# CouncilmanJeremyJamm/path_tracer

Measured on AMD Instinct MI355X. Metric: Mray/s at 1920x1080, 256 spp; achieved HBM GB/s in traversal kernel, higher is better.
Workload: dtype f32; 1 GPU; Cornell box (36 triangles, 6 BLAS) 1920x1080, 256 spp, depth 8, NEE+MIS; parallelism=rows/1, bvh_in_lds=True, scene_bytes=4208

## Files before the change

### include/pt_api.h

```cpp
#ifndef PT_API_H
#define PT_API_H
#include <stdint.h>
#ifdef __cplusplus
extern "C" {
#endif

typedef struct pt_ctx pt_ctx;

enum pt_status
{
    PT_OK = 0,
    PT_ERR_ARG = -1,
    PT_ERR_HIP = -2,
    PT_ERR_STATE = -3,
    PT_ERR_NONRIGID = -4,
    PT_ERR_LIMIT = -5,
    PT_ERR_IO = -6,
    PT_ERR_PARSE = -7,
    PT_ERR_NCCL = -8
};

enum pt_material_kind
{
    PT_LAMBERTIAN = 0,
    PT_EMISSIVE = 1,
    PT_SPECULAR = 2,
    PT_GGX_METAL = 3,
    PT_GGX_DIELECTRIC = 4,
    PT_DIELECTRIC = 5
};

typedef struct pt_material_desc
{
    int32_t kind;
    float colour[3];
    float roughness;
    float ior;
    int32_t has_volume;
    float vol_absorption[3];
    float vol_k, vol_c, vol_g;
} pt_material_desc;

typedef struct pt_config
{
    uint32_t width, height;
    uint32_t max_bounces;
    uint32_t n_sobol;
    uint32_t enable_nee;
    uint64_t seed;
    uint32_t rank, world_size, strip_rows;
    uint32_t batch_spp;
    int32_t device;
    uint32_t flags;
    uint32_t stack_lds_levels;
    uint32_t queue_slack;
    uint32_t pipelines;
    uint32_t reserved;
} pt_config;

enum
{
    PT_FLAG_TIMING = 1u,
    PT_FLAG_NO_LDS_SCENE = 2u,
    PT_FLAG_TIMING_ALL = 4u,
    PT_FLAG_NO_PRIMARY_CULL = 8u,
    PT_FLAG_GENERAL_WALK = 16u,
    PT_FLAG_ADAPTIVE = 32u
};

pt_ctx* pt_create(const pt_config* cfg);
void pt_destroy(pt_ctx* ctx);
const char* pt_last_error(pt_ctx* ctx);
int pt_set_config(pt_ctx* ctx, const pt_config* cfg);

int pt_add_material(pt_ctx* ctx, const pt_material_desc* desc);
int pt_add_model(pt_ctx* ctx, const float* positions_xyz, const float* normals_xyz, uint32_t n_tris, int material,
                 const float* affine3x4_rowmajor, uint32_t n_instances);
int pt_add_model_obj(pt_ctx* ctx, const char* path, int material, const float* affine3x4_rowmajor, uint32_t n_instances);
int pt_model_vertices(pt_ctx* ctx, int model, float* positions_xyz, float* normals_xyz, uint32_t cap_tris, uint32_t* n_tris);
int pt_build(pt_ctx* ctx);
int pt_set_instances(pt_ctx* ctx, int model, const float* affine3x4_rowmajor, uint32_t n_instances);
typedef struct pt_scene_info
{
    uint64_t blas_builds;
    uint64_t tlas_builds;
    uint64_t uploads_full;
    uint64_t uploads_patched;
    uint64_t last_upload_bytes;
    uint64_t scene_bytes;
    uint64_t reserved[2];
} pt_scene_info;
int pt_get_scene_info(pt_ctx* ctx, pt_scene_info* out);

int pt_add_texture(pt_ctx* ctx, uint32_t w, uint32_t h, const float* rgb_linear);
int pt_set_material_texture(pt_ctx* ctx, int material, int texture);
int pt_set_model_uvs(pt_ctx* ctx, int model, const float* uv, uint32_t n_tris);
int pt_model_uvs(pt_ctx* ctx, int model, float* uv, uint32_t cap_tris, uint32_t* n_tris);
int pt_surface_colour(pt_ctx* ctx, int on_device, uint32_t n, const uint32_t* instance, const uint32_t* prim, const float* u, const float* v,
                      float* rgb);

int pt_set_camera(pt_ctx* ctx, const float eye[3], const float target[3], float fov_y_deg, float aspect);
enum pt_event { PT_EV_MOUSE_MOTION = 0, PT_EV_KEY_W = 1, PT_EV_KEY_S = 2, PT_EV_KEY_A = 3, PT_EV_KEY_D = 4 };
int pt_camera_input(pt_ctx* ctx, int event, float a, float b, float dt);
int pt_camera_angles(pt_ctx* ctx, float pitch_yaw[2]);
int pt_camera_matrices(pt_ctx* ctx, float cam_to_world_3x4[12], float inv_proj_4x4_colmajor[16]);
int pt_set_environment(pt_ctx* ctx, uint32_t width, uint32_t height, const float* rgb_linear);
int pt_create_ray(pt_ctx* ctx, float s, float t, float o[3], float d[3]);

int pt_set_lens(pt_ctx* ctx, float aperture, float focus);
int pt_primary_ray(pt_ctx* ctx, uint32_t pixel, uint32_t sample, float o[3], float d[3], uint32_t* draws);

enum pt_projection_kind { PT_PROJ_PERSPECTIVE = 0, PT_PROJ_PANORAMA = 1, PT_PROJ_ORTHOGRAPHIC = 2 };
typedef struct pt_projection {
    uint32_t kind;
    float span_x_deg, span_y_deg;
    float ortho_height;
    uint32_t reserved[4];
} pt_projection;
int pt_set_projection(pt_ctx* ctx, const pt_projection* projection);
int pt_get_projection(pt_ctx* ctx, pt_projection* out);

int pt_render(pt_ctx* ctx, uint32_t first_sample, uint32_t n_samples, float* data_rgba, float* position_xyzt, uint32_t* id);
int pt_active_pixels(pt_ctx* ctx, uint32_t rect[4], float root_box[6]);
int pt_render_device(pt_ctx* ctx, uint32_t first_sample, uint32_t n_samples);
int pt_reset_accumulation(pt_ctx* ctx);
int pt_accum_device_ptr(pt_ctx* ctx, void** dev_ptr, uint64_t* n_pixels);
int pt_read_accumulation(pt_ctx* ctx, float* data_rgba);
int pt_read_frame(pt_ctx* ctx, float* data_rgba, float* position_xyzt, uint32_t* id);
int pt_write_accumulation(pt_ctx* ctx, const float* data_rgba, const float* position_xyzt, const uint32_t* id);
int pt_render_samples(pt_ctx* ctx, uint32_t first_sample, uint32_t n_samples, float* samples_rgba);
typedef struct pt_adaptive
{
    float rel_error;
    float abs_floor;
    uint32_t min_samples;
    uint32_t max_samples;
} pt_adaptive;
int pt_render_adaptive(pt_ctx* ctx, const pt_adaptive* crit, uint32_t n_samples, uint32_t* n_active);
int pt_adaptive_mask(pt_ctx* ctx, const pt_adaptive* crit, uint8_t* mask, uint32_t* n_active);
int pt_read_moments(pt_ctx* ctx, float* sumsq);
int pt_write_moments(pt_ctx* ctx, const float* sumsq);

int pt_local_rows(pt_ctx* ctx, uint32_t* n_rows, uint32_t* rows, uint32_t cap);
int pt_set_stream(pt_ctx* ctx, void* hip_stream);
int pt_synchronize(pt_ctx* ctx);

int pt_frame(pt_ctx* ctx, uint32_t frame_index, const float* last_inv_projection, float* data_rgba, float* position_xyzt, uint32_t* id);
int pt_inv_projection(pt_ctx* ctx, float out16_colmajor[16]);
int pt_frame_moving(pt_ctx* ctx, uint32_t frame_index, const float* last_inv_projection, float* data_rgba, float* position_xyzt, uint32_t* id);
int pt_present(pt_ctx* ctx, float* rgba);
int pt_present_rgb8(pt_ctx* ctx, uint8_t* rgb);
int pt_write_image(pt_ctx* ctx, const char* path);
int pt_post_velocity(pt_ctx* ctx, uint32_t w, uint32_t h, const float* position, const float* last_inv_projection, float* velocity);
int pt_post_reproject(pt_ctx* ctx, uint32_t w, uint32_t h, const float* input, const float* accum, const float* velocity, const uint32_t* id,
                      float* output);
int pt_post_motion(pt_ctx* ctx, uint32_t w, uint32_t h, const float* position_xyzt, const uint32_t* instance, uint32_t n_instances,
                   const float* matrix12, const float* inv_matrix12, const float* prev_matrix12, const uint8_t* has_prev, float* x_prev_xyzt);
int pt_post_tonemap(pt_ctx* ctx, uint32_t w, uint32_t h, const float* accum, float* out);
int pt_post_rgb8(pt_ctx* ctx, uint32_t w, uint32_t h, const float* accum, uint8_t* rgb);

int pt_render_guides(pt_ctx* ctx, uint32_t sample);
int pt_read_guides(pt_ctx* ctx, float* position_xyzt, float* normal_xyz, uint32_t* model);
int pt_read_guide_instances(pt_ctx* ctx, uint32_t* instance);
int pt_read_guide_albedo(pt_ctx* ctx, float* rgb);
typedef struct pt_denoise_params
{
    uint32_t iterations;
    float sigma_luminance;
    uint32_t sigma_normal;
    float sigma_plane;
} pt_denoise_params;
int pt_denoise(pt_ctx* ctx, const pt_denoise_params* p, float* rgba);
int pt_write_denoised_image(pt_ctx* ctx, const char* path);
int pt_post_denoise(pt_ctx* ctx, uint32_t w, uint32_t h, const pt_denoise_params* p, const float* accum_rgba, const float* position_xyzt,
                    const float* normal_xyz, const uint32_t* model, const float* sumsq, float* out_rgba);

int pt_accumulate_albedo(pt_ctx* ctx, uint32_t first_sample, uint32_t n_samples);
int pt_reset_albedo(pt_ctx* ctx);
int pt_read_albedo(pt_ctx* ctx, float* rgbn);
enum { PT_ALBEDO_GUIDE = 1, PT_ALBEDO_MEAN = 2 };
int pt_denoise_albedo(pt_ctx* ctx, const pt_denoise_params* p, uint32_t albedo_source, float* rgba);
int pt_post_denoise_albedo(pt_ctx* ctx, uint32_t w, uint32_t h, const pt_denoise_params* p, const float* accum_rgba, const float* position_xyzt,
                           const float* normal_xyz, const uint32_t* model, const float* albedo_rgb, const float* sumsq, float* out_rgba);

typedef struct pt_rays_params
{
    uint32_t draws_consumed;
    uint32_t batch_rays;
    uint32_t reserved[2];
} pt_rays_params;
int pt_integrate_rays(pt_ctx* ctx, uint64_t n, const float* o_xyz, const float* d_xyz, const uint32_t* key, const uint32_t* sample,
                      const pt_rays_params* p, float* radiance_rgba, float* position_xyzt, uint8_t* id);
int pt_integrate_rays_device(pt_ctx* ctx, uint64_t n, const float* o_xyz, const float* d_xyz, const uint32_t* key, const uint32_t* sample,
                             const pt_rays_params* p, float* radiance_rgba, float* position_xyzt, uint8_t* id);

typedef struct pt_probe_params
{
    uint32_t first_sample, n_samples;
    uint32_t key_base;
    uint32_t reserved;
} pt_probe_params;
int pt_bake_probes(pt_ctx* ctx, uint32_t n_probes, const float* position_xyz, const pt_probe_params* p, float* sh27);
int pt_probe_ray(pt_ctx* ctx, uint32_t key, uint32_t sample, float d[3], float y9[9]);

int pt_trace_closest(pt_ctx* ctx, int which, uint32_t n, const float* o_xyz, const float* d_xyz, const float* t_max, float* t,
                     float* u, float* v, uint32_t* inst, uint32_t* prim);
int pt_trace_any(pt_ctx* ctx, int which, uint32_t n, const float* o_xyz, const float* d_xyz, const float* t_max, uint8_t* hit);
int pt_ss_sobol(pt_ctx* ctx, uint32_t n_points, uint32_t n, const uint32_t* index, const uint32_t* seed, float* out_xy);
int pt_math_batch(pt_ctx* ctx, int fn, uint32_t n, const float* a, const float* b, float* out0, float* out1);
int pt_material_eval(pt_ctx* ctx, int material, uint32_t n, const float* incoming_xyz, const float* normal_xyz, const uint8_t* front,
                     const uint32_t* pixel, const uint32_t* sample, uint32_t draws_consumed, float* out9);
int pt_volume_eval(pt_ctx* ctx, int material, uint32_t n, const float* incoming_xyz, const float* t_max, const float* dist,
                   const uint32_t* pixel, const uint32_t* sample, uint32_t draws_consumed, float* out9);

int pt_blas_count(pt_ctx* ctx);
int pt_blas_dump(pt_ctx* ctx, int blas, uint32_t* n_nodes, uint32_t* root, float* boxes6, uint32_t* kind, uint32_t* a, uint32_t* b,
                 uint32_t* n_prim_ids, uint32_t* prim_ids, uint32_t cap_nodes, uint32_t cap_ids);
int pt_tlas_dump(pt_ctx* ctx, int which, uint32_t* n_nodes, uint32_t* root, float* boxes6, uint32_t* kind, uint32_t* a, uint32_t* b,
                 uint32_t cap_nodes);
int pt_tlas_instances(pt_ctx* ctx, int which, uint32_t* n, float* matrix12, float* inv_matrix12, uint32_t cap);
int pt_instance_materials(pt_ctx* ctx, int which, uint32_t* n, uint32_t* material, uint32_t* blas, uint32_t cap);
int pt_light_cdf(pt_ctx* ctx, uint32_t* n, float* pdf, float* cdf, uint32_t* blas, uint32_t* prim, float* max_weight, uint32_t cap);
int pt_triangle_dump(pt_ctx* ctx, int blas, uint32_t prim, float out36[36]);

typedef struct pt_multi pt_multi;
pt_multi* pt_multi_create(const pt_config* cfg, const int32_t* devices, uint32_t n_devices);
void pt_multi_destroy(pt_multi* m);
const char* pt_multi_last_error(pt_multi* m);
pt_ctx* pt_multi_ctx(pt_multi* m, uint32_t rank);
int pt_multi_render(pt_multi* m, uint32_t first_sample, uint32_t n_samples, float* data_rgba);
int pt_multi_framebuffer_device_ptr(pt_multi* m, void** dev_ptr);
int pt_multi_reset_accumulation(pt_multi* m);
int pt_multi_write_image(pt_multi* m, const char* path);
int pt_multi_used_rccl(pt_multi* m);

typedef struct pt_stats
{
    uint64_t rays_closest;
    uint64_t rays_any;
    uint64_t rays_light_closest;
    uint64_t paths;
    uint64_t launches_trace_closest;
    double ms_trace_closest;
    double ms_trace_any, ms_trace_light, ms_shade, ms_generate, ms_accumulate;
    double ms_total;
    uint64_t scene_bytes;
    uint32_t lds_scene;
    uint32_t stack_entries;
    uint64_t state_bytes;
    uint64_t rays_light_closest_traced;
    uint64_t rays_primary_culled;
    uint32_t ident_tlas;
    uint32_t reserved_stats;
} pt_stats;
int pt_get_stats(pt_ctx* ctx, pt_stats* out);
int pt_multi_get_stats(pt_multi* m, pt_stats* sum);
int pt_last_batch_counters(pt_ctx* ctx, uint32_t* rows16, uint32_t cap_rows, uint32_t* n_rows);
int pt_last_batch_shade_pids(pt_ctx* ctx, uint32_t qclass, uint32_t first, uint32_t count, uint32_t* pids);
int pt_last_batch_step_stats(pt_ctx* ctx, uint32_t* rows8, uint32_t cap_rows, uint32_t* n_rows);
int pt_reset_stats(pt_ctx* ctx);

#ifdef __cplusplus
}
#endif
#endif
```

### path_tracer_amd/api.py

```python
from __future__ import annotations

import ctypes as C
import os
from typing import Optional

import numpy as np

from . import build as _build
from .scene_desc import CameraDesc, SceneDesc

PT_OK = 0
FLAG_TIMING = 1
FLAG_NO_LDS_SCENE = 2
FLAG_TIMING_ALL = 4
FLAG_NO_PRIMARY_CULL = 8
FLAG_GENERAL_WALK = 16
FLAG_ADAPTIVE = 32
DEFAULT_SEED = 0x5EED5EED

EXPORTS = [
    "pt_create", "pt_destroy", "pt_last_error", "pt_set_config", "pt_add_material", "pt_add_model", "pt_add_model_obj", "pt_model_vertices", "pt_build", "pt_set_camera",
    "pt_camera_matrices", "pt_set_environment", "pt_create_ray", "pt_set_lens", "pt_primary_ray", "pt_render", "pt_render_device", "pt_reset_accumulation", "pt_accum_device_ptr",
    "pt_read_accumulation", "pt_read_frame", "pt_write_accumulation", "pt_render_samples", "pt_render_adaptive", "pt_adaptive_mask", "pt_read_moments", "pt_write_moments", "pt_active_pixels", "pt_local_rows", "pt_set_stream", "pt_synchronize", "pt_camera_input", "pt_camera_angles", "pt_frame", "pt_inv_projection", "pt_present", "pt_post_velocity", "pt_post_reproject", "pt_post_tonemap", "pt_post_rgb8", "pt_present_rgb8", "pt_write_image", "pt_trace_closest", "pt_trace_any",
    "pt_ss_sobol", "pt_math_batch", "pt_material_eval", "pt_volume_eval", "pt_blas_count", "pt_blas_dump", "pt_tlas_dump", "pt_tlas_instances", "pt_instance_materials", "pt_light_cdf",
    "pt_triangle_dump", "pt_get_stats", "pt_reset_stats", "pt_last_batch_counters", "pt_last_batch_shade_pids", "pt_last_batch_step_stats",
    "pt_multi_create", "pt_multi_destroy", "pt_multi_last_error", "pt_multi_ctx", "pt_multi_render", "pt_multi_framebuffer_device_ptr",
    "pt_multi_reset_accumulation", "pt_multi_get_stats", "pt_multi_used_rccl", "pt_multi_write_image",
    "pt_render_guides", "pt_read_guides", "pt_denoise", "pt_write_denoised_image", "pt_post_denoise",
    "pt_integrate_rays", "pt_integrate_rays_device", "pt_bake_probes", "pt_probe_ray",
    "pt_set_instances", "pt_get_scene_info", "pt_read_guide_instances", "pt_frame_moving", "pt_post_motion",
    "pt_add_texture", "pt_set_material_texture", "pt_set_model_uvs", "pt_model_uvs", "pt_surface_colour", "pt_read_guide_albedo",
    "pt_accumulate_albedo", "pt_reset_albedo", "pt_read_albedo", "pt_denoise_albedo", "pt_post_denoise_albedo",
    "pt_set_projection", "pt_get_projection",
]


ALBEDO_GUIDE, ALBEDO_MEAN = 1, 2
PROJ_PERSPECTIVE, PROJ_PANORAMA, PROJ_ORTHOGRAPHIC = range(3)
EV_MOUSE_MOTION, EV_KEY_W, EV_KEY_S, EV_KEY_A, EV_KEY_D = range(5)


class MaterialDesc(C.Structure):
    _fields_ = [("kind", C.c_int32), ("colour", C.c_float * 3), ("roughness", C.c_float), ("ior", C.c_float), ("has_volume", C.c_int32),
                ("vol_absorption", C.c_float * 3), ("vol_k", C.c_float), ("vol_c", C.c_float), ("vol_g", C.c_float)]


class Projection(C.Structure):
    _fields_ = [("kind", C.c_uint32), ("span_x_deg", C.c_float), ("span_y_deg", C.c_float), ("ortho_height", C.c_float), ("reserved", C.c_uint32 * 4)]


class Config(C.Structure):
    _fields_ = [("width", C.c_uint32), ("height", C.c_uint32), ("max_bounces", C.c_uint32), ("n_sobol", C.c_uint32),
                ("enable_nee", C.c_uint32), ("seed", C.c_uint64), ("rank", C.c_uint32), ("world_size", C.c_uint32),
                ("strip_rows", C.c_uint32), ("batch_spp", C.c_uint32), ("device", C.c_int32), ("flags", C.c_uint32),
                ("stack_lds_levels", C.c_uint32), ("queue_slack", C.c_uint32), ("pipelines", C.c_uint32), ("reserved", C.c_uint32)]


class Stats(C.Structure):
    _fields_ = [("rays_closest", C.c_uint64), ("rays_any", C.c_uint64), ("rays_light_closest", C.c_uint64), ("paths", C.c_uint64),
                ("launches_trace_closest", C.c_uint64), ("ms_trace_closest", C.c_double), ("ms_trace_any", C.c_double),
                ("ms_trace_light", C.c_double), ("ms_shade", C.c_double), ("ms_generate", C.c_double), ("ms_accumulate", C.c_double),
                ("ms_total", C.c_double), ("scene_bytes", C.c_uint64), ("lds_scene", C.c_uint32), ("stack_entries", C.c_uint32),
                ("state_bytes", C.c_uint64), ("rays_light_closest_traced", C.c_uint64), ("rays_primary_culled", C.c_uint64),
                ("ident_tlas", C.c_uint32), ("reserved_stats", C.c_uint32)]

    def as_dict(self):
        return {n: getattr(self, n) for n, _ in self._fields_}

    @property
    def rays(self):
        return self.rays_closest + self.rays_any + self.rays_light_closest


class Adaptive(C.Structure):
    _fields_ = [("rel_error", C.c_float), ("abs_floor", C.c_float), ("min_samples", C.c_uint32), ("max_samples", C.c_uint32)]


class DenoiseParams(C.Structure):
    _fields_ = [("iterations", C.c_uint32), ("sigma_luminance", C.c_float), ("sigma_normal", C.c_uint32), ("sigma_plane", C.c_float)]


class RaysParams(C.Structure):
    _fields_ = [("draws_consumed", C.c_uint32), ("batch_rays", C.c_uint32), ("reserved", C.c_uint32 * 2)]


class ProbeParams(C.Structure):
    _fields_ = [("first_sample", C.c_uint32), ("n_samples", C.c_uint32), ("key_base", C.c_uint32), ("reserved", C.c_uint32)]


class SceneInfo(C.Structure):
    _fields_ = [("blas_builds", C.c_uint64), ("tlas_builds", C.c_uint64), ("uploads_full", C.c_uint64), ("uploads_patched", C.c_uint64),
                ("last_upload_bytes", C.c_uint64), ("scene_bytes", C.c_uint64), ("reserved", C.c_uint64 * 2)]

    def as_dict(self):
        return {n: getattr(self, n) for n, _ in self._fields_ if n != "reserved"}


class PtError(RuntimeError):
    def __init__(self, code, msg):
        super().__init__(f"libptmi error {code}: {msg}")
        self.code = code


_lib = None


def lib():
    global _lib
    if _lib is None:
        path = os.environ.get("PTMI_LIB")
        if not path:
            path = _build.LIB_PATH
            if _build.is_stale():
                path = _build.build()
        try:
            import torch
        except ImportError:
            pass
        L = C.CDLL(path)
        vp, u32, f32p = C.c_void_p, C.c_uint32, C.c_void_p
        L.pt_create.restype = vp
        L.pt_create.argtypes = [C.POINTER(Config)]
        L.pt_destroy.argtypes = [vp]
        L.pt_last_error.restype = C.c_char_p
        L.pt_last_error.argtypes = [vp]
        L.pt_set_config.argtypes = [vp, C.POINTER(Config)]
        L.pt_add_material.argtypes = [vp, C.POINTER(MaterialDesc)]
        L.pt_add_model.argtypes = [vp, f32p, f32p, u32, C.c_int, f32p, u32]
        L.pt_add_model_obj.argtypes = [vp, C.c_char_p, C.c_int, f32p, u32]
        L.pt_model_vertices.argtypes = [vp, C.c_int, f32p, f32p, u32, C.POINTER(u32)]
        L.pt_build.argtypes = [vp]
        L.pt_set_camera.argtypes = [vp, C.POINTER(C.c_float), C.POINTER(C.c_float), C.c_float, C.c_float]
        L.pt_camera_matrices.argtypes = [vp, vp, vp]
        L.pt_set_environment.argtypes = [vp, u32, u32, vp]
        L.pt_create_ray.argtypes = [vp, C.c_float, C.c_float, vp, vp]
        L.pt_set_lens.argtypes = [vp, C.c_float, C.c_float]
        L.pt_primary_ray.argtypes = [vp, u32, u32, vp, vp, C.POINTER(u32)]
        L.pt_set_projection.argtypes = [vp, C.POINTER(Projection)]
        L.pt_get_projection.argtypes = [vp, C.POINTER(Projection)]
        L.pt_render.argtypes = [vp, u32, u32, vp, vp, vp]
        L.pt_render_device.argtypes = [vp, u32, u32]
        L.pt_active_pixels.argtypes = [vp, vp, vp]
        L.pt_reset_accumulation.argtypes = [vp]
        L.pt_accum_device_ptr.argtypes = [vp, C.POINTER(vp), C.POINTER(C.c_uint64)]
        L.pt_read_accumulation.argtypes = [vp, vp]
        L.pt_write_accumulation.argtypes = [vp, vp, vp, vp]
        L.pt_read_frame.argtypes = [vp, vp, vp, vp]
        L.pt_render_samples.argtypes = [vp, u32, u32, vp]
        L.pt_render_adaptive.argtypes = [vp, C.POINTER(Adaptive), u32, C.POINTER(u32)]
        L.pt_adaptive_mask.argtypes = [vp, C.POINTER(Adaptive), vp, C.POINTER(u32)]
        L.pt_read_moments.argtypes = [vp, vp]
        L.pt_write_moments.argtypes = [vp, vp]
        L.pt_local_rows.argtypes = [vp, C.POINTER(u32), vp, u32]
        L.pt_set_stream.argtypes = [vp, vp]
        L.pt_synchronize.argtypes = [vp]
        L.pt_frame.argtypes = [vp, u32, vp, vp, vp, vp]
        L.pt_camera_input.argtypes = [vp, C.c_int, C.c_float, C.c_float, C.c_float]
        L.pt_camera_angles.argtypes = [vp, vp]
        L.pt_inv_projection.argtypes = [vp, vp]
        L.pt_present.argtypes = [vp, vp]
        L.pt_multi_create.restype = vp
        L.pt_multi_create.argtypes = [C.POINTER(Config), vp, u32]
        L.pt_multi_destroy.argtypes = [vp]
        L.pt_multi_last_error.restype = C.c_char_p
        L.pt_multi_last_error.argtypes = [vp]
        L.pt_multi_ctx.restype = vp
        L.pt_multi_ctx.argtypes = [vp, u32]
        L.pt_multi_render.argtypes = [vp, u32, u32, vp]
        L.pt_multi_framebuffer_device_ptr.argtypes = [vp, C.POINTER(vp)]
        L.pt_multi_reset_accumulation.argtypes = [vp]
        L.pt_multi_get_stats.argtypes = [vp, C.POINTER(Stats)]
        L.pt_multi_used_rccl.argtypes = [vp]
        L.pt_multi_write_image.argtypes = [vp, C.c_char_p]
        L.pt_post_velocity.argtypes = [vp, u32, u32, vp, vp, vp]
        L.pt_post_reproject.argtypes = [vp, u32, u32, vp, vp, vp, vp, vp]
        L.pt_post_tonemap.argtypes = [vp, u32, u32, vp, vp]
        L.pt_post_rgb8.argtypes = [vp, u32, u32, vp, vp]
        L.pt_present_rgb8.argtypes = [vp, vp]
        L.pt_write_image.argtypes = [vp, C.c_char_p]
        L.pt_trace_closest.argtypes = [vp, C.c_int, u32] + [vp] * 8
        L.pt_trace_any.argtypes = [vp, C.c_int, u32] + [vp] * 4
        L.pt_ss_sobol.argtypes = [vp, u32, u32, vp, vp, vp]
        L.pt_math_batch.argtypes = [vp, C.c_int, u32, vp, vp, vp, vp]
        L.pt_material_eval.argtypes = [vp, C.c_int, u32, vp, vp, vp, vp, vp, u32, vp]
        L.pt_volume_eval.argtypes = [vp, C.c_int, u32, vp, vp, vp, vp, vp, u32, vp]
        L.pt_blas_count.argtypes = [vp]
        L.pt_blas_dump.argtypes = [vp, C.c_int] + [vp] * 8 + [u32, u32]
        L.pt_tlas_dump.argtypes = [vp, C.c_int] + [vp] * 6 + [u32]
        L.pt_tlas_instances.argtypes = [vp, C.c_int, vp, vp, vp, u32]
        L.pt_instance_materials.argtypes = [vp, C.c_int, vp, vp, vp, u32]
        L.pt_light_cdf.argtypes = [vp] + [vp] * 6 + [u32]
        L.pt_triangle_dump.argtypes = [vp, C.c_int, u32, vp]
        L.pt_get_stats.argtypes = [vp, C.POINTER(Stats)]
        L.pt_reset_stats.argtypes = [vp]
        L.pt_last_batch_counters.argtypes = [vp, vp, u32, C.POINTER(u32)]
        L.pt_last_batch_shade_pids.argtypes = [vp, u32, u32, u32, vp]
        L.pt_render_guides.argtypes = [vp, u32]
        L.pt_read_guides.argtypes = [vp, vp, vp, vp]
        L.pt_denoise.argtypes = [vp, C.POINTER(DenoiseParams), vp]
        L.pt_write_denoised_image.argtypes = [vp, C.c_char_p]
        L.pt_post_denoise.argtypes = [vp, u32, u32, C.POINTER(DenoiseParams), vp, vp, vp, vp, vp, vp]
        L.pt_integrate_rays.argtypes = [vp, C.c_uint64, vp, vp, vp, vp, C.POINTER(RaysParams), vp, vp, vp]
        L.pt_integrate_rays_device.argtypes = [vp, C.c_uint64, vp, vp, vp, vp, C.POINTER(RaysParams), vp, vp, vp]
        L.pt_bake_probes.argtypes = [vp, u32, vp, C.POINTER(ProbeParams), vp]
        L.pt_probe_ray.argtypes = [vp, u32, u32, vp, vp]
        L.pt_set_instances.argtypes = [vp, C.c_int, f32p, u32]
        L.pt_get_scene_info.argtypes = [vp, C.POINTER(SceneInfo)]
        L.pt_read_guide_instances.argtypes = [vp, vp]
        L.pt_frame_moving.argtypes = [vp, u32, vp, vp, vp, vp]
        L.pt_post_motion.argtypes = [vp, u32, u32, vp, vp, u32, vp, vp, vp, vp, vp]
        L.pt_add_texture.argtypes = [vp, u32, u32, vp]
        L.pt_set_material_texture.argtypes = [vp, C.c_int, C.c_int]
        L.pt_set_model_uvs.argtypes = [vp, C.c_int, vp, u32]
        L.pt_model_uvs.argtypes = [vp, C.c_int, vp, u32, C.POINTER(u32)]
        L.pt_surface_colour.argtypes = [vp, C.c_int, u32, vp, vp, vp, vp, vp]
        L.pt_read_guide_albedo.argtypes = [vp, vp]
        L.pt_accumulate_albedo.argtypes = [vp, u32, u32]
        L.pt_reset_albedo.argtypes = [vp]
        L.pt_read_albedo.argtypes = [vp, vp]
        L.pt_denoise_albedo.argtypes = [vp, C.POINTER(DenoiseParams), u32, vp]
        L.pt_post_denoise_albedo.argtypes = [vp, u32, u32, C.POINTER(DenoiseParams), vp, vp, vp, vp, vp, vp, vp]
        _lib = L
    return _lib


def _p(a):
    return a.ctypes.data_as(C.c_void_p) if a is not None else None


def _f3(v):
    return (C.c_float * 3)(*[float(x) for x in v])


class Renderer:

    def __init__(self, scene: SceneDesc, width: int, height: int, max_bounces: int = 8, n_sobol: int = 512, enable_nee: bool = True,
                 seed: int = DEFAULT_SEED, rank: int = 0, world_size: int = 1, strip_rows: int = 4, batch_spp: int = 0, device: int = -1,
                 flags: int = 0, stack_lds_levels: int = 0, queue_slack: int = 0, pipelines: int = 0):
        self.L = lib()
        self.cfg = Config(width, height, max_bounces, n_sobol, int(enable_nee), seed, rank, world_size, strip_rows, batch_spp, device, flags,
                          stack_lds_levels, queue_slack, pipelines, 0)
        self.ctx = C.c_void_p(self.L.pt_create(C.byref(self.cfg)))
        if not self.ctx:
            raise PtError(-1, "pt_create failed (bad configuration)")
        self.desc = scene
        self._materials = []
        self._textures = []
        for mod in scene.models:
            self.add_model(mod)
        self.rebuild()
        if scene.camera is not None:
            self.set_camera(scene.camera)

    def _material_index(self, m) -> int:
        if m not in self._materials:
            d = MaterialDesc()
            d.kind = m.kind
            d.colour[:] = m.colour
            d.roughness, d.ior = m.roughness, m.ior
            if m.volume is not None:
                d.has_volume = 1
                d.vol_absorption[:] = m.volume.absorption
                d.vol_k, d.vol_c, d.vol_g = m.volume.k, m.volume.c, m.volume.g
            mi = self._chk(self.L.pt_add_material(self.ctx, C.byref(d)), allow_positive=True)
            self._materials.append(m)
            if getattr(m, "texture", None) is not None:
                self.set_material_texture(mi, self._texture_index(m.texture))
        return self._materials.index(m)

    def _texture_index(self, t) -> int:
        for i, have in enumerate(self._textures):
            if have is t:
                return i
        self.add_texture(t.data)
        self._textures[-1] = t
        return len(self._textures) - 1

    def add_model(self, mod) -> int:
        mi = self._material_index(mod.material)
        if getattr(mod, "obj_path", None):
            r = self._chk(self.L.pt_add_model_obj(self.ctx, mod.obj_path.encode(), mi, _p(mod.matrices), mod.matrices.shape[0]), allow_positive=True)
        else:
            r = self._chk(self.L.pt_add_model(self.ctx, _p(mod.positions), _p(mod.normals), mod.positions.shape[0], mi, _p(mod.matrices),
                                              mod.matrices.shape[0]), allow_positive=True)
        if getattr(mod, "uvs", None) is not None:
            self.set_model_uvs(r, mod.uvs)
        return r

# ... 380 lines not shown
                                                _p(out)))
        return out

    def integrate_rays(self, o, d, key, sample, draws_consumed=1, batch_rays=0):
        if type(o).__module__.startswith("torch"):
            return self._integrate_rays_device(o, d, key, sample, draws_consumed, batch_rays)
        o = np.ascontiguousarray(o, np.float32).reshape(-1, 3)
        d = np.ascontiguousarray(d, np.float32).reshape(-1, 3)
        key = np.ascontiguousarray(key, np.uint32).reshape(-1)
        sample = np.ascontiguousarray(sample, np.uint32).reshape(-1)
        n = o.shape[0]
        if d.shape[0] != n or key.size != n or sample.size != n:
            raise PtError(-1, "integrate_rays: o, d, key and sample do not describe the same number of rays")
        rad = np.zeros((n, 4), np.float32); pos = np.zeros((n, 4), np.float32); idb = np.zeros(n, np.uint8)
        prm = RaysParams(draws_consumed, batch_rays)
        self._chk(self.L.pt_integrate_rays(self.ctx, n, _p(o), _p(d), _p(key), _p(sample), C.byref(prm), _p(rad), _p(pos), _p(idb)))
        return rad, pos, idb

    def _integrate_rays_device(self, o, d, key, sample, draws_consumed, batch_rays):
        import torch
        n = o.shape[0]
        ts = (o, d, key, sample)
        if not all(t.is_cuda and t.is_contiguous() for t in ts) or o.dtype != torch.float32 or d.dtype != torch.float32 or \
                key.dtype not in (torch.int32, torch.uint32) or sample.dtype not in (torch.int32, torch.uint32):
            raise PtError(-1, "integrate_rays: device rays are contiguous GPU tensors, o and d float32, key and sample 32-bit integers")
        if o.numel() != 3 * n or d.numel() != 3 * n or key.numel() != n or sample.numel() != n:
            raise PtError(-1, "integrate_rays: o, d, key and sample do not describe the same number of rays")
        rad = torch.zeros((n, 4), dtype=torch.float32, device=o.device); pos = torch.zeros((n, 4), dtype=torch.float32, device=o.device)
        idb = torch.zeros(n, dtype=torch.uint8, device=o.device)
        torch.cuda.synchronize(o.device)
        prm = RaysParams(draws_consumed, batch_rays)
        ptr = lambda t: C.c_void_p(t.data_ptr())
        self._chk(self.L.pt_integrate_rays_device(self.ctx, n, ptr(o), ptr(d), ptr(key), ptr(sample), C.byref(prm), ptr(rad), ptr(pos), ptr(idb)))
        return rad, pos, idb

    def bake_probes(self, positions, n_samples, first_sample=0, key_base=0, sh=None):
        pos = np.ascontiguousarray(positions, np.float32).reshape(-1, 3)
        n = pos.shape[0]
        out = np.zeros((n, 9, 3), np.float32) if sh is None else np.ascontiguousarray(sh, np.float32)
        if out.size != n * 27:
            raise PtError(-1, "bake_probes: sh does not hold 27 values per probe")
        prm = ProbeParams(first_sample, n_samples, key_base, 0)
        self._chk(self.L.pt_bake_probes(self.ctx, n, _p(pos), C.byref(prm), _p(out)))
        return out.reshape(n, 9, 3)

    def probe_ray(self, key: int, sample: int):
        d = np.zeros(3, np.float32); y = np.zeros(9, np.float32)
        self._chk(self.L.pt_probe_ray(self.ctx, key, sample, _p(d), _p(y)))
        return d, y

    def trace_closest(self, o, d, tmax=None, which=0):
        o = np.ascontiguousarray(o, np.float32)
        d = np.ascontiguousarray(d, np.float32)
        n = o.shape[0]
        tm = None if tmax is None else np.ascontiguousarray(tmax, np.float32)
        t = np.zeros(n, np.float32); u = np.zeros(n, np.float32); v = np.zeros(n, np.float32)
        inst = np.zeros(n, np.uint32); prim = np.zeros(n, np.uint32)
        self._chk(self.L.pt_trace_closest(self.ctx, which, n, _p(o), _p(d), _p(tm), _p(t), _p(u), _p(v), _p(inst), _p(prim)))
        return dict(t=t, u=u, v=v, inst=inst, prim=prim)

    def trace_any(self, o, d, tmax, which=0):
        o = np.ascontiguousarray(o, np.float32)
        d = np.ascontiguousarray(d, np.float32)
        tm = np.ascontiguousarray(tmax, np.float32)
        hit = np.zeros(o.shape[0], np.uint8)
        self._chk(self.L.pt_trace_any(self.ctx, which, o.shape[0], _p(o), _p(d), _p(tm), _p(hit)))
        return hit

    def ss_sobol(self, n_points, index, seed):
        index = np.ascontiguousarray(index, np.uint32)
        seed = np.ascontiguousarray(seed, np.uint32)
        out = np.zeros((index.size, 2), np.float32)
        self._chk(self.L.pt_ss_sobol(self.ctx, n_points, index.size, _p(index), _p(seed), _p(out)))
        return out

    def math_batch(self, fn, a, b=None):
        a = np.ascontiguousarray(a, np.float32)
        b = None if b is None else np.ascontiguousarray(b, np.float32)
        o0 = np.zeros_like(a)
        o1 = np.zeros_like(a)
        self._chk(self.L.pt_math_batch(self.ctx, fn, a.size, _p(a), _p(b), _p(o0), _p(o1)))
        return o0, o1

    def material_eval(self, material, incoming, normal, front, pixel, sample, draws_consumed=0):
        i = np.ascontiguousarray(incoming, np.float32); n = np.ascontiguousarray(normal, np.float32)
        f = np.ascontiguousarray(front, np.uint8); px = np.ascontiguousarray(pixel, np.uint32); sm = np.ascontiguousarray(sample, np.uint32)
        out = np.zeros((i.shape[0], 9), np.float32)
        self._chk(self.L.pt_material_eval(self.ctx, material, i.shape[0], _p(i), _p(n), _p(f), _p(px), _p(sm), draws_consumed, _p(out)))
        return out

    def volume_eval(self, material, incoming, t_max, dist, pixel, sample, draws_consumed=0):
        i = np.ascontiguousarray(incoming, np.float32); tm = np.ascontiguousarray(t_max, np.float32); d = np.ascontiguousarray(dist, np.float32)
        px = np.ascontiguousarray(pixel, np.uint32); sm = np.ascontiguousarray(sample, np.uint32)
        out = np.zeros((i.shape[0], 9), np.float32)
        self._chk(self.L.pt_volume_eval(self.ctx, material, i.shape[0], _p(i), _p(tm), _p(d), _p(px), _p(sm), draws_consumed, _p(out)))
        return out

    def model_vertices(self, model):
        n = C.c_uint32()
        self._chk(self.L.pt_model_vertices(self.ctx, model, None, None, 0, C.byref(n)))
        p = np.zeros((n.value, 3, 3), np.float32)
        nr = np.zeros((n.value, 3, 3), np.float32)
        self._chk(self.L.pt_model_vertices(self.ctx, model, _p(p), _p(nr), n.value, C.byref(n)))
        return p, nr

    def blas_count(self):
        return self._chk(self.L.pt_blas_count(self.ctx), allow_positive=True)

    def blas_dump(self, blas, cap=1 << 20):
        nn = C.c_uint32(); root = C.c_uint32(); nids = C.c_uint32()
        boxes = np.zeros((cap, 6), np.float32); kind = np.zeros(cap, np.uint32); a = np.zeros(cap, np.uint32); b = np.zeros(cap, np.uint32)
        ids = np.zeros(cap, np.uint32)
        self._chk(self.L.pt_blas_dump(self.ctx, blas, C.byref(nn), C.byref(root), _p(boxes), _p(kind), _p(a), _p(b), C.byref(nids), _p(ids), cap, cap))
        n = nn.value
        return dict(root=root.value, boxes=boxes[:n].copy(), kind=kind[:n].copy(), a=a[:n].copy(), b=b[:n].copy(), prim_ids=ids[:nids.value].copy())

    def tlas_dump(self, which=0, cap=1 << 16):
        nn = C.c_uint32(); root = C.c_uint32()
        boxes = np.zeros((cap, 6), np.float32); kind = np.zeros(cap, np.uint32); a = np.zeros(cap, np.uint32); b = np.zeros(cap, np.uint32)
        self._chk(self.L.pt_tlas_dump(self.ctx, which, C.byref(nn), C.byref(root), _p(boxes), _p(kind), _p(a), _p(b), cap))
        n = nn.value
        return dict(root=root.value, boxes=boxes[:n].copy(), kind=kind[:n].copy(), a=a[:n].copy(), b=b[:n].copy())

    def tlas_instances(self, which=0, cap=1 << 16):
        n = C.c_uint32()
        m = np.zeros((cap, 3, 4), np.float32); inv = np.zeros((cap, 3, 4), np.float32)
        self._chk(self.L.pt_tlas_instances(self.ctx, which, C.byref(n), _p(m), _p(inv), cap))
        return dict(matrix=m[:n.value].copy(), inv_matrix=inv[:n.value].copy())

    def instance_materials(self, which=0, cap=1 << 16):
        n = C.c_uint32()
        mat = np.zeros(cap, np.uint32); bl = np.zeros(cap, np.uint32)
        self._chk(self.L.pt_instance_materials(self.ctx, which, C.byref(n), _p(mat), _p(bl), cap))
        return dict(material=mat[:n.value].copy(), blas=bl[:n.value].copy())

    def light_cdf(self, cap=1 << 20):
        n = C.c_uint32(); mx = C.c_float()
        pdf = np.zeros(cap, np.float32); cdf = np.zeros(cap, np.float32); bl = np.zeros(cap, np.uint32); pr = np.zeros(cap, np.uint32)
        self._chk(self.L.pt_light_cdf(self.ctx, C.byref(n), _p(pdf), _p(cdf), _p(bl), _p(pr), C.byref(mx), cap))
        k = n.value
        return dict(pdf=pdf[:k].copy(), cdf=cdf[:k].copy(), blas=bl[:k].copy(), prim=pr[:k].copy(), max=mx.value)

    def triangle(self, blas, prim):
        out = np.zeros(36, np.float32)
        self._chk(self.L.pt_triangle_dump(self.ctx, blas, prim, _p(out)))
        return out

    def stats(self) -> Stats:
        s = Stats()
        self._chk(self.L.pt_get_stats(self.ctx, C.byref(s)))
        return s

    def last_batch_counters(self):
        rows = np.zeros((self.cfg.max_bounces + 2, 16), np.uint32)
        n = C.c_uint32()
        self._chk(self.L.pt_last_batch_counters(self.ctx, _p(rows), rows.shape[0], C.byref(n)))
        return rows[: n.value]

    def last_batch_shade_pids(self, qclass, first, count):
        out = np.zeros(count, np.uint32)
        self._chk(self.L.pt_last_batch_shade_pids(self.ctx, qclass, first, count, _p(out)))
        return out

    def last_batch_step_stats(self):
        rows = np.zeros((self.cfg.max_bounces + 2, 8), np.uint32)
        n = C.c_uint32()
        self._chk(self.L.pt_last_batch_step_stats(self.ctx, _p(rows), rows.shape[0], C.byref(n)))
        return rows[: n.value]

    def reset_stats(self):
        self._chk(self.L.pt_reset_stats(self.ctx))


class MultiRenderer:

    def __init__(self, scene: SceneDesc, width: int, height: int, devices, **kw):
        self.L = lib()
        devices = [int(d) for d in devices]
        kw.setdefault("strip_rows", 4)
        cfg = Config(width, height, kw.get("max_bounces", 8), kw.get("n_sobol", 512), int(kw.get("enable_nee", True)), kw.get("seed", DEFAULT_SEED), 0, 1,
                     kw["strip_rows"], kw.get("batch_spp", 0), -1, kw.get("flags", 0), 0, 0, kw.get("pipelines", 0), 0)
        arr = (C.c_int32 * len(devices))(*devices)
        self.m = C.c_void_p(self.L.pt_multi_create(C.byref(cfg), arr, len(devices)))
        if not self.m:
            raise PtError(-1, "pt_multi_create failed")
        self.width, self.height, self.n = width, height, len(devices)
        self.rank0 = Renderer.attach(self.L.pt_multi_ctx(self.m, 0), cfg)
        for mod in scene.models:
            self.rank0.add_model(mod)
        self.rank0.rebuild()
        if scene.camera is not None:
            self.rank0.set_camera(scene.camera)

    def _chk(self, r):
        if r != 0:
            raise PtError(r, self.L.pt_multi_last_error(self.m).decode())

    def render(self, first_sample: int, n_samples: int, download=True):
        out = np.zeros((self.height, self.width, 4), np.float32) if download else None
        self._chk(self.L.pt_multi_render(self.m, first_sample, n_samples, _p(out)))
        return out

    def reset_accumulation(self):
        self._chk(self.L.pt_multi_reset_accumulation(self.m))

    def write_image(self, path):
        self._chk(self.L.pt_multi_write_image(self.m, str(path).encode()))

    def used_rccl(self) -> bool:
        return bool(self.L.pt_multi_used_rccl(self.m))

    def stats(self) -> Stats:
        s = Stats()
        self._chk(self.L.pt_multi_get_stats(self.m, C.byref(s)))
        return s

    def close(self):
# ... 11 lines not shown
```

### path_tracer_amd/csrc/pt_api.cpp

```cpp
#include "../../include/pt_api.h"

#include <hip/hip_runtime.h>

#include <algorithm>
#include <chrono>
#include <cmath>
#include <cstdio>
#include <cstdlib>
#include <cstring>
#include <mutex>
#include <string>
#include <utility>
#include <vector>

#include "pt_batch_plan.h"
#include "pt_kernels.h"
#include "pt_png.h"
#include "pt_probe.h"
#include "pt_scene.h"

using namespace pt;

#ifndef PT_SHADE_BLOCKS_PER_CU
#define PT_SHADE_BLOCKS_PER_CU 16
// ... 24 lines not shown
#endif

namespace {

enum TimeCat { T_GEN = 0, T_WORLD, T_ANY, T_LIGHT, T_SHADE, T_ACCUM, T_COUNT };

template <class T, auto Release>
struct Owned
{
    T p{};
    Owned() = default;
    Owned(Owned&& o) noexcept : p(std::exchange(o.p, T{})) {}
    ~Owned() { reset(); }
    void reset() { if (p) (void)Release(p); p = T{}; }
    T* out() { reset(); return &p; }
    operator T() const { return p; }
};
using StreamHandle = Owned<hipStream_t, hipStreamDestroy>;
using EventHandle = Owned<hipEvent_t, hipEventDestroy>;
template <class T> using Pinned = Owned<T*, hipHostFree>;

struct DevBuf : Owned<void*, hipFree>
{
    size_t bytes = 0;
    DevBuf() = default;
    DevBuf(DevBuf&& o) noexcept : Owned(std::move(o)), bytes(std::exchange(o.bytes, 0)) {}
    void reset() { Owned::reset(); bytes = 0; }
};

}

struct pt_ctx
{
    pt_config cfg{};
    HostScene scene;
    std::string err;
    std::mutex mu;

    bool dev_ready = false;
    int device = 0;
    int n_cus = 256;
    StreamHandle own_stream;
    hipStream_t stream = nullptr;
    EventHandle ev_start;

    struct Pipe
    {
        StreamHandle own_stream, side_stream;
        EventHandle ev_fork, ev_join, ev_done;
        size_t cap_paths = 0, cap_slots = 0, cap_slots_term = 0;
        uint32_t cap_rows = 0;
        std::vector<DevBuf> pool;
        WavefrontBuffers wb{};
        Pinned<Counters> h_counters;
        Pinned<uint32_t> h_heads;
        struct Ev { EventHandle a, b; int cat; };
        std::vector<Ev> ev_pool;
        size_t ev_used = 0;
        uint32_t slack_cfg = 0;
        uint32_t pixels_cfg = 0;
        size_t state_bytes = 0;
        DevBuf ray_pos, ray_id;
        bool busy = false;
        uint32_t busy_rows = 0;
        uint64_t busy_paths = 0, busy_culled = 0;
    };
    static constexpr int kMaxPipes = (int)kMaxPipelines;
    Pipe pipe[kMaxPipes];
    hipStream_t pipe_stream(int i) const { return i == 0 ? stream : pipe[i].own_stream; }

    bool scene_uploaded = false;
    DevBuf d_spill;
    size_t spill_region_words = 0;
    DevBuf d_blob, d_tri_shade, d_tri_pos, d_tri_orig, d_materials, d_lights, d_env;
    DevBuf d_tri_uv, d_tex_table, d_tex_texels;
    TexView tex{};
    bool textured = false;
    std::vector<f4> h_env;
    uint32_t env_w = 0, env_h = 0;
    bool env_uploaded = false;
    SceneView sv{};
    bool lds_scene = false;
    uint32_t ident_tlas = 0;
    uint32_t block_threads = 256, trace_blocks = 1024;
    bool class_present[Q_COUNT] = {true, false, false, false, false};
    bool resident_valid = false;
    uint64_t resident_epoch = 0;
    size_t resident_blob_bytes = 0;
    std::vector<uint8_t> h_patch;
    EventHandle ev_patch;
    uint64_t uploads_full = 0, uploads_patched = 0, last_upload_bytes = 0;

    std::vector<uint32_t> rows;
    uint32_t local_pixels = 0;
    uint32_t pad_rows = 0;
    uint64_t scene_version = 0;
    DevBuf d_accum, d_position, d_id;
    DevBuf d_input, d_velocity, d_output;

    DevBuf d_moments, d_list, d_select;
    bool moments_valid = true;
    const uint2* cur_list = nullptr;
    uint32_t cur_list_n = 0;

    DevBuf d_gpos, d_gnrm, d_gmodel, d_ginst, d_galbedo, d_gray_a, d_gray_b, d_ghits, d_ghead;
    bool guides_valid = false;
    uint64_t guides_scene_version = 0, guides_config_version = 0;
    uint32_t guides_sample = 0;
    uint64_t config_version = 0;
    DevBuf d_dn_a, d_dn_b, d_dn_nv, d_dn_out;
    DevBuf d_albedo_sum, d_dn_k;
    bool albedo_valid = false;
    uint64_t albedo_scene_version = 0, albedo_config_version = 0;

    std::vector<std::vector<xf34>> snap;
    bool snap_valid = false;
    uint64_t snap_build = 0;
    DevBuf d_motion, d_xprev;
    bool denoised_valid = false;

    DevBuf d_ray_keys;

    pt_stats stats{};
    int last_pipe = 0;
};

namespace {

int fail(pt_ctx* c, int code, const std::string& msg)
{
    c->err = msg;
    return code;
}

#define HIPCHK(c, call)                                                                                       \
    do {                                                                                                      \
        hipError_t e__ = (call);                                                                              \
        if (e__ != hipSuccess) return fail((c), PT_ERR_HIP, std::string(#call) + ": " + hipGetErrorString(e__)); \
    } while (0)

int dev_alloc(pt_ctx* c, DevBuf& b, size_t bytes)
{
    if (b.bytes >= bytes && b.p) return PT_OK;
    b.reset();
    bytes = std::max<size_t>(bytes, 16);
    HIPCHK(c, hipMalloc(&b.p, bytes));
    b.bytes = bytes;
    return PT_OK;
}

struct Staging
{
    pt_ctx* c;
    int err = PT_OK;
    std::vector<DevBuf> bufs;
    explicit Staging(pt_ctx* c_) : c(c_) {}
    void* in(const void* src, size_t bytes)
    {
        DevBuf b;
        if (err || (err = dev_alloc(c, b, bytes))) return nullptr;
        const hipError_t e = src ? hipMemcpy(b.p, src, bytes, hipMemcpyHostToDevice) : hipSuccess;
        if (e != hipSuccess) { err = fail(c, PT_ERR_HIP, hipGetErrorString(e)); return nullptr; }
        bufs.push_back(std::move(b));
        return bufs.back().p;
    }
    void* out(size_t bytes) { return in(nullptr, bytes); }
// ... 10 lines not shown
    const pt_config& g = c->cfg;
    c->rows.clear();
    const uint32_t world = std::max(1u, g.world_size), strip = std::max(1u, g.strip_rows);
    for (uint32_t y = 0; y < g.height; ++y)
        if ((y / strip) % world == g.rank) c->rows.push_back(y);
    c->local_pixels = (uint32_t)c->rows.size() * g.width;
    uint32_t r0 = 0;
    for (uint32_t y = 0; y < g.height; ++y) r0 += ((y / strip) % world == 0u) ? 1u : 0u;
    c->pad_rows = r0;
}

int normalise_config(pt_ctx* c, const pt_config* in)
{
    pt_config g = *in;
    if (g.width == 0 || g.height == 0) return fail(c, PT_ERR_ARG, "width/height must be non-zero");
    if (g.n_sobol == 0) g.n_sobol = 512;
    if (g.world_size == 0) g.world_size = 1;
    if (g.strip_rows == 0) g.strip_rows = 4;
    if (g.rank >= g.world_size) return fail(c, PT_ERR_ARG, "rank >= world_size");
    if ((uint64_t)g.width * g.height > 0x7fffffffull) return fail(c, PT_ERR_ARG, "image too large");
    c->cfg = g;
    compute_rows(c);
    return PT_OK;
}

int ensure_device(pt_ctx* c)
{
    if (c->dev_ready)
    {
        HIPCHK(c, hipSetDevice(c->device));
        return PT_OK;
    }
    int n = 0;
    hipError_t e = hipGetDeviceCount(&n);
    if (e != hipSuccess || n == 0) return fail(c, PT_ERR_HIP, "no HIP device available (libptmi has no CPU path)");
    if (c->cfg.device >= 0) HIPCHK(c, hipSetDevice(c->cfg.device));
    HIPCHK(c, hipGetDevice(&c->device));
    hipDeviceProp_t prop;
    HIPCHK(c, hipGetDeviceProperties(&prop, c->device));
    c->n_cus = prop.multiProcessorCount > 0 ? prop.multiProcessorCount : 256;
    HIPCHK(c, hipStreamCreateWithFlags(c->own_stream.out(), hipStreamNonBlocking));
    HIPCHK(c, hipEventCreateWithFlags(c->ev_start.out(), hipEventDisableTiming));
    for (int i = 0; i < pt_ctx::kMaxPipes; ++i)
    {
        pt_ctx::Pipe& pp = c->pipe[i];
        if (i > 0) HIPCHK(c, hipStreamCreateWithFlags(pp.own_stream.out(), hipStreamNonBlocking));
        HIPCHK(c, hipStreamCreateWithFlags(pp.side_stream.out(), hipStreamNonBlocking));
        HIPCHK(c, hipEventCreateWithFlags(pp.ev_fork.out(), hipEventDisableTiming));
        HIPCHK(c, hipEventCreateWithFlags(pp.ev_join.out(), hipEventDisableTiming));
        HIPCHK(c, hipEventCreateWithFlags(pp.ev_done.out(), hipEventDisableTiming));
    }
    if (!c->stream) c->stream = c->own_stream;
    c->dev_ready = true;
    return PT_OK;
}

int derive_scene_view(pt_ctx* c, const FlatScene& f, size_t blob_bytes)
{
    int r;
    const size_t nb = f.nodes.size() * sizeof(DNode), tb = f.tri_isect.size() * sizeof(DTriIsect);
    SceneView& sv = c->sv;
    uint8_t* base = (uint8_t*)c->d_blob.p;
    sv.nodes = (const DNode*)base;
    sv.tri_isect = (const DTriIsect*)(base + nb);
    sv.instances = (const DInstance*)(base + nb + tb);
    sv.tri_shade = (const DTriVerts*)c->d_tri_shade.p;
    sv.tri_pos = (const DTriVerts*)c->d_tri_pos.p;
    sv.tri_orig = (const uint32_t*)c->d_tri_orig.p;
    sv.materials = (const DMaterial*)c->d_materials.p;
    sv.lights = (const DLight*)c->d_lights.p;
    sv.n_nodes = (uint32_t)f.nodes.size();
    sv.n_tris = (uint32_t)f.tri_isect.size();
    sv.n_instances = (uint32_t)f.instances.size();
    sv.n_materials = (uint32_t)f.materials.size();
    sv.n_lights = (uint32_t)f.lights.size();
    sv.world_root = f.world_root;
    sv.lights_root = f.lights_root;
    sv.prim_bits = f.prim_bits;
    sv.light_weight_sum = f.light_weight_sum;
    sv.blob_bytes = (uint32_t)blob_bytes;
    sv.stack_entries = f.stack_entries;
    sv.has_volumes = f.has_volumes ? 1u : 0u;
    c->ident_tlas = f.ident_tlas;

    c->lds_scene = blob_bytes <= 48 * 1024 && !(c->cfg.flags & PT_FLAG_NO_LDS_SCENE);
    uint32_t threads = 256;
#ifndef PT_STACK_LDS_LEVELS
#define PT_STACK_LDS_LEVELS 14
#endif
    sv.stack_lds = std::min<uint32_t>(sv.stack_entries, c->cfg.stack_lds_levels ? c->cfg.stack_lds_levels : PT_STACK_LDS_LEVELS);
    auto lds_need = [&](uint32_t t) { return trace_lds_bytes(c->lds_scene, sv.blob_bytes, sv.stack_lds, t); };
    while (threads > 64 && lds_need(threads) > 64 * 1024) threads >>= 1;
    if (lds_need(threads) > 160 * 1024) return fail(c, PT_ERR_LIMIT, "BVH too deep for the LDS traversal stack");
    c->block_threads = threads;
    const size_t lds = lds_need(threads);
    uint32_t per_cu = (uint32_t)std::min<size_t>((160 * 1024) / std::max<size_t>(lds, 1), 2048 / threads);
    per_cu = std::max(1u, std::min(per_cu, (uint32_t)PT_TRACE_BLOCKS_PER_CU_MAX));
    c->trace_blocks = (uint32_t)c->n_cus * per_cu;
    sv.stack_spill = nullptr;
    if (sv.stack_entries > sv.stack_lds)
    {
        const size_t lanes = (size_t)c->trace_blocks * threads;
        c->spill_region_words = (size_t)(sv.stack_entries - sv.stack_lds) * lanes;
        if ((r = dev_alloc(c, c->d_spill, 2 * pt_ctx::kMaxPipes * c->spill_region_words * 8))) return r;
        sv.stack_spill = (uint64_t*)c->d_spill.p;
    }

    for (uint32_t q = 0; q < Q_COUNT; ++q) c->class_present[q] = (q == Q_TERMINAL);
    for (const DInstance& in : f.instances) c->class_present[in.qclass & 0xffu] = true;
    c->stats.scene_bytes = blob_bytes;
    c->stats.lds_scene = c->lds_scene;
    c->stats.stack_entries = sv.stack_entries;
    return PT_OK;
}

int upload_scene(pt_ctx* c)
{
    if (c->scene_uploaded) return ensure_device(c);
    if (!c->scene.built) return fail(c, PT_ERR_STATE, "pt_build has not been called");
    int r = ensure_device(c);
    if (r) return r;
    const FlatScene& f = c->scene.flat;
    const size_t nb = f.nodes.size() * sizeof(DNode), tb = f.tri_isect.size() * sizeof(DTriIsect), ib = f.instances.size() * sizeof(DInstance);
    const size_t lb = (f.big_leaves.size() * 4 + 15) / 16 * 16;
    const size_t blob_bytes = nb + tb + ib + lb;

    if (c->resident_valid && c->resident_epoch == c->scene.layout_epoch && c->resident_blob_bytes == blob_bytes && c->d_blob.p)
    {
        const size_t tlas_nodes = c->scene.world.nodes.size() + c->scene.lights.nodes.size();
        const size_t pn = tlas_nodes * sizeof(DNode);
        if (pn > nb) return fail(c, PT_ERR_STATE, "internal: TLAS nodes exceed the node array");
        HIPCHK(c, hipStreamSynchronize(c->stream));
        if (!c->ev_patch.p) HIPCHK(c, hipEventCreateWithFlags(c->ev_patch.out(), hipEventDisableTiming));
        for (int i = 1; i < pt_ctx::kMaxPipes; ++i)
        {
            HIPCHK(c, hipEventRecord(c->ev_patch, c->pipe_stream(i)));
            HIPCHK(c, hipStreamWaitEvent(c->stream, c->ev_patch, 0));
        }
        c->h_patch.resize(pn + ib);
        if (pn) std::memcpy(c->h_patch.data(), f.nodes.data(), pn);
        if (ib) std::memcpy(c->h_patch.data() + pn, f.instances.data(), ib);
        uint8_t* base = (uint8_t*)c->d_blob.p;
        if (pn) HIPCHK(c, hipMemcpyAsync(base, c->h_patch.data(), pn, hipMemcpyHostToDevice, c->stream));
        if (ib) HIPCHK(c, hipMemcpyAsync(base + nb + tb, c->h_patch.data() + pn, ib, hipMemcpyHostToDevice, c->stream));
        if ((r = derive_scene_view(c, f, blob_bytes))) { c->resident_valid = false; return r; }
        c->scene_uploaded = true;
        c->uploads_patched++;
        c->last_upload_bytes = pn + ib;
        return PT_OK;
    }

    c->resident_valid = false;
    std::vector<uint8_t> blob(blob_bytes);
    std::memcpy(blob.data(), f.nodes.data(), nb);
    std::memcpy(blob.data() + nb, f.tri_isect.data(), tb);
    std::memcpy(blob.data() + nb + tb, f.instances.data(), ib);
    if (lb) std::memcpy(blob.data() + nb + tb + ib, f.big_leaves.data(), f.big_leaves.size() * 4);
    if ((r = dev_alloc(c, c->d_blob, blob.size()))) return r;
    HIPCHK(c, hipMemcpy(c->d_blob.p, blob.data(), blob.size(), hipMemcpyHostToDevice));
    uint64_t copied = blob.size();
    auto up = [&](DevBuf& b, const void* src, size_t bytes) -> int {
        int rr = dev_alloc(c, b, bytes);
        if (rr) return rr;
        if (bytes) HIPCHK(c, hipMemcpy(b.p, src, bytes, hipMemcpyHostToDevice));
        copied += bytes;
        return PT_OK;
    };
    if ((r = up(c->d_tri_shade, f.tri_shade.data(), f.tri_shade.size() * sizeof(DTriVerts)))) return r;
    if ((r = up(c->d_tri_pos, f.tri_pos.data(), f.tri_pos.size() * sizeof(DTriVerts)))) return r;
    if ((r = up(c->d_tri_orig, f.tri_orig.data(), f.tri_orig.size() * 4))) return r;
    if ((r = up(c->d_materials, f.materials.data(), f.materials.size() * sizeof(DMaterial)))) return r;
    if ((r = up(c->d_lights, f.lights.data(), f.lights.size() * sizeof(DLight)))) return r;
    c->textured = f.has_textures;
    c->tex = TexView{};
    if (f.has_textures)
    {
        if ((r = up(c->d_tri_uv, f.tri_uv.data(), f.tri_uv.size() * sizeof(DTriUV)))) return r;
        if ((r = up(c->d_tex_table, f.tex_table.data(), f.tex_table.size() * sizeof(DTexture)))) return r;
        if ((r = up(c->d_tex_texels, f.tex_texels.data(), f.tex_texels.size() * sizeof(f4)))) return r;
        c->tex = TexView{(const f4*)c->d_tex_texels.p, (const DTexture*)c->d_tex_table.p, (const DTriUV*)c->d_tri_uv.p};
    }
    if ((r = derive_scene_view(c, f, blob_bytes))) return r;
    c->scene_uploaded = true;
    c->resident_valid = true;
    c->resident_epoch = c->scene.layout_epoch;
    c->resident_blob_bytes = blob_bytes;
    c->uploads_full++;
    c->last_upload_bytes = copied;
    return PT_OK;
}

TraceLaunch trace_launch(pt_ctx* c, int pipe = 0, bool side_stream = false)
{
    TraceLaunch tl;
    tl.scene = c->sv;
    if (tl.scene.stack_spill) tl.scene.stack_spill += (size_t)(2 * pipe + (side_stream ? 1 : 0)) * c->spill_region_words;
    tl.blob = c->d_blob.p;
    tl.lds_scene = c->lds_scene;
    tl.ident_tlas = (c->cfg.flags & PT_FLAG_GENERAL_WALK) ? 0u : c->ident_tlas;
    tl.grid_blocks = c->trace_blocks;
    tl.n_cus = (uint32_t)c->n_cus;
    tl.block_threads = c->block_threads;
    tl.tex = c->textured ? &c->tex : nullptr;
    return tl;
}

struct ActiveRect { uint32_t x0, w, ly0, rows; };
ActiveRect active_rect(pt_ctx* c)
{
    const uint32_t W = c->cfg.width, H = c->cfg.height, local_rows = (uint32_t)c->rows.size();
    const ActiveRect full{0u, W, 0u, local_rows};
    if ((c->cfg.flags & PT_FLAG_NO_PRIMARY_CULL) || c->env_w || !c->scene.built || !c->scene.camera.set) return full;
    if (c->scene.camera.proj_kind != PROJ_PERSPECTIVE) return full;
    const FlatScene& f = c->scene.flat;
    if (f.world_root == MISS_ID || f.world_root >= f.nodes.size()) return full;
    const DNode& root = f.nodes[f.world_root];
    double m[16], inv[16];
    for (int i = 0; i < 16; ++i) m[i] = c->scene.camera.ray_matrix[i];
    {
        double a[4][8];
        for (int r = 0; r < 4; ++r)
            for (int k = 0; k < 4; ++k) { a[r][k] = m[k * 4 + r]; a[r][4 + k] = r == k ? 1.0 : 0.0; }
        for (int col = 0; col < 4; ++col)
        {
            int piv = col;
            for (int r = col + 1; r < 4; ++r)
                if (std::fabs(a[r][col]) > std::fabs(a[piv][col])) piv = r;
            if (std::fabs(a[piv][col]) < 1e-300) return full;
            for (int k = 0; k < 8; ++k) std::swap(a[col][k], a[piv][k]);
            const double d = a[col][col];
            for (int k = 0; k < 8; ++k) a[col][k] /= d;
            for (int r = 0; r < 4; ++r)
                if (r != col)
                {
                    const double fct = a[r][col];
                    for (int k = 0; k < 8; ++k) a[r][k] -= fct * a[col][k];
                }
        }
        for (int r = 0; r < 4; ++r)
            for (int k = 0; k < 4; ++k) inv[k * 4 + r] = a[r][4 + k];
    }
    const double eye[3] = {c->scene.camera.matrix.t.x, c->scene.camera.matrix.t.y, c->scene.camera.matrix.t.z};
    double ctr[4];
    for (int r = 0; r < 4; ++r) ctr[r] = m[12 + r];
    if (!(std::fabs(ctr[3]) > 1e-300)) return full;
    double fwd[3] = {ctr[0] / ctr[3] - eye[0], ctr[1] / ctr[3] - eye[1], ctr[2] / ctr[3] - eye[2]};
    const double fl = std::sqrt(fwd[0] * fwd[0] + fwd[1] * fwd[1] + fwd[2] * fwd[2]);
    if (!(fl > 0.0) || !std::isfinite(fl)) return full;
    double ext = 0.0;
    for (int k = 0; k < 3; ++k) { fwd[k] /= fl; ext = std::max(ext, std::fabs((double)root.mx[k] - (double)root.mn[k])); }
    const LensView lens = c->scene.lens_view();
    const double lens_r = lens.radius;
    double px_lo = 1e300, px_hi = -1e300, py_lo = 1e300, py_hi = -1e300;
    for (int corner = 0; corner < 8; ++corner)
    {
        const double X[3] = {corner & 1 ? root.mx[0] : root.mn[0], corner & 2 ? root.mx[1] : root.mn[1], corner & 4 ? root.mx[2] : root.mn[2]};
        if (!std::isfinite(X[0]) || !std::isfinite(X[1]) || !std::isfinite(X[2])) return full;
        const double depth = (X[0] - eye[0]) * fwd[0] + (X[1] - eye[1]) * fwd[1] + (X[2] - eye[2]) * fwd[2];
        if (!(depth > 1e-3 * ext + 1e-6)) return full;
        for (int lc = 0; lc < (lens_r > 0.0 ? 4 : 1); ++lc)
        {
            double P[3] = {X[0], X[1], X[2]};
            if (lens_r > 0.0)
            {
                const double sa = lc & 1 ? lens_r : -lens_r, sb = lc & 2 ? lens_r : -lens_r;
                double L[3], z = 0.0;
                for (int k = 0; k < 3; ++k) { L[k] = eye[k] + sa * lens.c0[k] + sb * lens.c1[k]; z += (X[k] - L[k]) * fwd[k]; }
                if (!(z > 1e-3 * ext + 1e-6)) return full;
                for (int k = 0; k < 3; ++k) P[k] = L[k] + (X[k] - L[k]) * ((double)lens.focus / z);
            }
            double q[4];
            for (int r = 0; r < 4; ++r) q[r] = inv[r] * P[0] + inv[4 + r] * P[1] + inv[8 + r] * P[2] + inv[12 + r];
            if (!(std::fabs(q[3]) > 1e-300)) return full;
            const double nx = q[0] / q[3], ny = q[1] / q[3];
            if (!std::isfinite(nx) || !std::isfinite(ny)) return full;
            const double px = (nx + 1.0) * 0.5 * W, py = (ny + 1.0) * 0.5 * H;
            px_lo = std::min(px_lo, px); px_hi = std::max(px_hi, px);
            py_lo = std::min(py_lo, py); py_hi = std::max(py_hi, py);
        }
    }
    const double margin = 3.0;
    const double gx0 = std::floor(px_lo - 0.5 - margin), gx1 = std::ceil(px_hi + 0.5 + margin) + 1.0;
// ... 2056 lines not shown
    {
        for (uint32_t i = 0; i < n; ++i) { t[i] = __builtin_inff(); u[i] = v[i] = 0; inst[i] = prim[i] = MISS_ID; }
        return PT_OK;
    }
    Staging st(c);
    RayQueue q;
    uint32_t* dh = upload_rays(st, n, o, d, tmax, q);
    f4* dhit = (f4*)st.out((size_t)n * 16);
    if (st.err) return st.err;
    launch_trace_rays_closest(c->stream, trace_launch(c), root, q, n, dh, dhit);
    std::vector<f4> h(n);
    if ((r = st.download(h.data(), dhit, (size_t)n * 16))) return r;
    const FlatScene& f = c->scene.flat;
    const uint32_t mask = (1u << f.prim_bits) - 1u;
    for (uint32_t i = 0; i < n; ++i)
    {
        const uint32_t id = bits(h[i].w);
        t[i] = h[i].x; u[i] = h[i].y; v[i] = h[i].z;
        if (id == MISS_ID) { inst[i] = prim[i] = MISS_ID; t[i] = __builtin_inff(); u[i] = v[i] = 0; }
        else
        {
            inst[i] = (id >> f.prim_bits) - f.inst_base[which ? 1 : 0];
            prim[i] = f.tri_orig[id & mask];
        }
    }
    return PT_OK;
}

int pt_trace_any(pt_ctx* c, int which, uint32_t n, const float* o, const float* d, const float* tmax, uint8_t* hit)
{
    if (!c || !o || !d || !tmax || !hit) return PT_ERR_ARG;
    std::lock_guard<std::mutex> lk(c->mu);
    int r;
    if ((r = upload_scene(c))) return r;
    if (n == 0) return PT_OK;
    const uint32_t root = which ? c->sv.lights_root : c->sv.world_root;
    if (root == MISS_ID) { std::memset(hit, 0, n); return PT_OK; }
    Staging st(c);
    RayQueue q;
    uint32_t* dh = upload_rays(st, n, o, d, tmax, q);
    uint32_t* docc = (uint32_t*)st.out((size_t)n * 4);
    if (st.err) return st.err;
    launch_trace_rays_any(c->stream, trace_launch(c), root, q, n, dh, docc);
    std::vector<uint32_t> h(n);
    if ((r = st.download(h.data(), docc, (size_t)n * 4))) return r;
    for (uint32_t i = 0; i < n; ++i) hit[i] = h[i] ? 1 : 0;
    return PT_OK;
}

int pt_ss_sobol(pt_ctx* c, uint32_t n_points, uint32_t n, const uint32_t* index, const uint32_t* seed, float* out)
{
    if (!c || !index || !seed || !out || n_points == 0) return PT_ERR_ARG;
    std::lock_guard<std::mutex> lk(c->mu);
    int r;
    if ((r = ensure_device(c))) return r;
    Staging t(c);
    const uint32_t* di = (const uint32_t*)t.in(index, (size_t)n * 4);
    const uint32_t* ds = (const uint32_t*)t.in(seed, (size_t)n * 4);
    float* dout = (float*)t.out((size_t)n * 8);
    if (t.err) return t.err;
    launch_sobol_probe(c->stream, n_points, n, di, ds, dout);
    return t.download(out, dout, (size_t)n * 8);
}

int pt_math_batch(pt_ctx* c, int fn, uint32_t n, const float* a, const float* b, float* o0, float* o1)
{
    if (!c || !a || !o0) return PT_ERR_ARG;
    std::lock_guard<std::mutex> lk(c->mu);
    int r;
    if ((r = ensure_device(c))) return r;
    Staging t(c);
    const float* da = (const float*)t.in(a, (size_t)n * 4);
    float* db = (float*)t.in(b, (size_t)n * 4);
    float* d0 = (float*)t.out((size_t)n * 4);
    float* d1 = (float*)t.out((size_t)n * 4);
    if (t.err) return t.err;
    if (!b) HIPCHK(c, hipMemsetAsync(db, 0, (size_t)n * 4, c->stream));
    HIPCHK(c, hipMemsetAsync(d1, 0, (size_t)n * 4, c->stream));
    launch_math_probe(c->stream, fn, n, da, db, d0, d1, c->cfg.seed);
    if ((r = t.download(o0, d0, (size_t)n * 4))) return r;
    return o1 ? t.download(o1, d1, (size_t)n * 4) : PT_OK;
}

int pt_material_eval(pt_ctx* c, int material, uint32_t n, const float* incoming, const float* normal, const uint8_t* front, const uint32_t* pixel,
                     const uint32_t* sample, uint32_t draws, float* out9)
{
    if (!c || !incoming || !normal || !front || !pixel || !sample || !out9) return PT_ERR_ARG;
    std::lock_guard<std::mutex> lk(c->mu);
    if (material < 0 || material >= (int)c->scene.materials.size()) return fail(c, PT_ERR_ARG, "material index");
    int r;
    if ((r = upload_scene(c))) return r;
    Staging t(c);
    const float* di = (const float*)t.in(incoming, (size_t)n * 12);
    const float* dn = (const float*)t.in(normal, (size_t)n * 12);
    const uint8_t* df = (const uint8_t*)t.in(front, n);
    const uint32_t* dp = (const uint32_t*)t.in(pixel, (size_t)n * 4);
    const uint32_t* ds = (const uint32_t*)t.in(sample, (size_t)n * 4);
    float* dout = (float*)t.out((size_t)n * 36);
    if (t.err) return t.err;
    launch_material_probe(c->stream, c->sv, material, n, di, dn, df, dp, ds, draws, c->cfg.seed, dout);
    return t.download(out9, dout, (size_t)n * 36);
}

int pt_volume_eval(pt_ctx* c, int material, uint32_t n, const float* incoming, const float* t_max, const float* dist, const uint32_t* pixel,
                   const uint32_t* sample, uint32_t draws, float* out9)
{
    if (!c || !incoming || !t_max || !dist || !pixel || !sample || !out9) return PT_ERR_ARG;
    std::lock_guard<std::mutex> lk(c->mu);
    if (material < 0 || material >= (int)c->scene.materials.size()) return fail(c, PT_ERR_ARG, "material index");
    if (n == 0) return PT_OK;
    int r;
    if ((r = upload_scene(c))) return r;
    Staging t(c);
    const float* di = (const float*)t.in(incoming, (size_t)n * 12);
    const float* dt = (const float*)t.in(t_max, (size_t)n * 4);
    const float* dd = (const float*)t.in(dist, (size_t)n * 4);
    const uint32_t* dp = (const uint32_t*)t.in(pixel, (size_t)n * 4);
    const uint32_t* ds = (const uint32_t*)t.in(sample, (size_t)n * 4);
    float* dout = (float*)t.out((size_t)n * 36);
    if (t.err) return t.err;
    launch_volume_probe(c->stream, c->sv, material, n, di, dt, dd, dp, ds, draws, c->cfg.seed, dout);
    return t.download(out9, dout, (size_t)n * 36);
}

int pt_blas_count(pt_ctx* c) { return (c && c->scene.built) ? (int)c->scene.blas.size() : PT_ERR_STATE; }

int pt_blas_dump(pt_ctx* c, int blas, uint32_t* n_nodes, uint32_t* root, float* boxes6, uint32_t* kind, uint32_t* a, uint32_t* b,
                 uint32_t* n_prim_ids, uint32_t* prim_ids, uint32_t cap_nodes, uint32_t cap_ids)
{
    if (!c || !c->scene.built) return PT_ERR_STATE;
    if (blas < 0 || blas >= (int)c->scene.blas.size()) return PT_ERR_ARG;
    const HostBlas& bl = c->scene.blas[blas];
    *n_nodes = (uint32_t)bl.nodes.size();
    *root = bl.root;
    *n_prim_ids = (uint32_t)bl.prim_ids.size();
    if (bl.nodes.size() > cap_nodes || bl.prim_ids.size() > cap_ids) return PT_ERR_ARG;
    for (size_t i = 0; i < bl.nodes.size(); ++i)
    {
        std::memcpy(boxes6 + i * 6, &bl.nodes[i].box, 24);
        kind[i] = bl.nodes[i].kind == NODE_BRANCH ? 0 : 1;
        a[i] = bl.nodes[i].a;
        b[i] = bl.nodes[i].b;
    }
    std::memcpy(prim_ids, bl.prim_ids.data(), bl.prim_ids.size() * 4);
    return PT_OK;
}

int pt_tlas_dump(pt_ctx* c, int which, uint32_t* n_nodes, uint32_t* root, float* boxes6, uint32_t* kind, uint32_t* a, uint32_t* b, uint32_t cap)
{
    if (!c || !c->scene.built) return PT_ERR_STATE;
    const HostTlas& t = which ? c->scene.lights : c->scene.world;
    *n_nodes = (uint32_t)t.nodes.size();
    *root = t.root;
    if (t.nodes.size() > cap) return PT_ERR_ARG;
    for (size_t i = 0; i < t.nodes.size(); ++i)
    {
        std::memcpy(boxes6 + i * 6, &t.nodes[i].box, 24);
        kind[i] = t.nodes[i].kind == NODE_BRANCH ? 0 : 1;
        a[i] = t.nodes[i].a;
        b[i] = t.nodes[i].b;
    }
    return PT_OK;
}

int pt_tlas_instances(pt_ctx* c, int which, uint32_t* n, float* matrix12, float* inv_matrix12, uint32_t cap)
{
    if (!c || !c->scene.built || !n) return PT_ERR_STATE;
    const HostTlas& t = which ? c->scene.lights : c->scene.world;
    *n = (uint32_t)t.instances.size();
    if (t.instances.size() > cap || !matrix12 || !inv_matrix12) return PT_ERR_ARG;
    for (size_t i = 0; i < t.instances.size(); ++i) { xf_rows(t.instances[i].fwd, matrix12 + 12 * i); xf_rows(t.instances[i].inv, inv_matrix12 + 12 * i); }
    return PT_OK;
}

int pt_instance_materials(pt_ctx* c, int which, uint32_t* n, uint32_t* material, uint32_t* blas, uint32_t cap)
{
    if (!c || !c->scene.built || !n) return PT_ERR_STATE;
    const FlatScene& f = c->scene.flat;
    const uint32_t b = f.inst_base[which ? 1 : 0], e = which ? (uint32_t)f.instances.size() : f.inst_base[1];
    *n = e - b;
    if (e - b > cap || !material || !blas) return PT_ERR_ARG;
    for (uint32_t i = b; i < e; ++i) { material[i - b] = f.instances[i].material; blas[i - b] = f.instances[i].blas; }
    return PT_OK;
}

int pt_light_cdf(pt_ctx* c, uint32_t* n, float* pdf, float* cdf, uint32_t* blas, uint32_t* prim, float* max_weight, uint32_t cap)
{
    if (!c || !c->scene.built) return PT_ERR_STATE;
    const auto& L = c->scene.light_items;
    *n = (uint32_t)L.size();
    *max_weight = c->scene.light_weight_sum;
    if (L.size() > cap) return PT_ERR_ARG;
    for (size_t i = 0; i < L.size(); ++i) { pdf[i] = L[i].pdf; cdf[i] = L[i].cdf; blas[i] = L[i].blas; prim[i] = L[i].prim; }
    return PT_OK;
}

int pt_triangle_dump(pt_ctx* c, int blas, uint32_t prim, float out36[36])
{
    if (!c || !c->scene.built) return PT_ERR_STATE;
    if (blas < 0 || blas >= (int)c->scene.blas.size() || prim >= c->scene.blas[blas].tris.size()) return PT_ERR_ARG;
    const HostTriangle& t = c->scene.blas[blas].tris[prim];
    std::memcpy(out36, &t.n0, 16);
    std::memcpy(out36 + 4, &t.n1, 16);
    std::memcpy(out36 + 8, &t.n2, 16);
    std::memcpy(out36 + 12, t.p, 36);
    std::memcpy(out36 + 21, t.n, 36);
    for (int i = 30; i < 36; ++i) out36[i] = 0;
    return PT_OK;
}

}

#include <dlfcn.h>
#include <rccl/rccl.h>
#include <thread>

namespace {
struct Rccl
{
    void* lib = nullptr;
    ncclResult_t (*CommInitAll)(ncclComm_t*, int, const int*) = nullptr;
    ncclResult_t (*CommDestroy)(ncclComm_t) = nullptr;
    ncclResult_t (*GroupStart)() = nullptr;
    ncclResult_t (*GroupEnd)() = nullptr;
    ncclResult_t (*Gather)(const void*, void*, size_t, ncclDataType_t, int, ncclComm_t, hipStream_t) = nullptr;
    const char* (*GetErrorString)(ncclResult_t) = nullptr;
    bool load(std::string* err)
    {
        if (lib) return true;
        for (const char* name : {"librccl.so", "librccl.so.1", "/opt/rocm/lib/librccl.so"})
            if ((lib = dlopen(name, RTLD_NOW | RTLD_LOCAL))) break;
        if (!lib) { *err = std::string("librccl.so cannot be loaded: ") + dlerror(); return false; }
        CommInitAll = (decltype(CommInitAll))dlsym(lib, "ncclCommInitAll");
        CommDestroy = (decltype(CommDestroy))dlsym(lib, "ncclCommDestroy");
        GroupStart = (decltype(GroupStart))dlsym(lib, "ncclGroupStart");
        GroupEnd = (decltype(GroupEnd))dlsym(lib, "ncclGroupEnd");
        Gather = (decltype(Gather))dlsym(lib, "ncclGather");
        GetErrorString = (decltype(GetErrorString))dlsym(lib, "ncclGetErrorString");
        if (!CommInitAll || !CommDestroy || !GroupStart || !GroupEnd || !Gather || !GetErrorString) { *err = "librccl.so lacks an expected symbol"; return false; }
        return true;
    }
};
Rccl g_rccl;
std::mutex g_rccl_mu;
}

struct pt_multi
{
    std::vector<pt_ctx*> ctx;
    std::vector<int> devices;
    std::string err;
    bool distinct = true;
    std::vector<ncclComm_t> comms;
    uint64_t replicated_version = ~0ull;
    DevBuf d_parts, d_full;
    bool used_rccl = false;
};

namespace {
int mfail(pt_multi* m, int code, const std::string& msg)
{
    m->err = msg;
    return code;
}
#define MHIPCHK(m, call)                                                                                      \
// ... 324 lines not shown
```

### path_tracer_amd/csrc/pt_kernels.hip

```cpp
#include "pt_kernels.h"
#include "pt_camera.h"
#include "pt_probe.h"
#include "pt_materials.h"

#include <algorithm>
#include <mutex>
#include <type_traits>
#include <vector>

namespace pt {
namespace {

#ifndef PT_STEPS_PER_ROUND
#define PT_STEPS_PER_ROUND 8
#endif
#ifndef PT_REFILL_BELOW
#define PT_REFILL_BELOW 40
#endif
#ifndef PT_STEPS_PER_ROUND_GLOBAL_BVH
#define PT_STEPS_PER_ROUND_GLOBAL_BVH 4
#endif
#ifndef PT_REFILL_BELOW_GLOBAL_BVH
#define PT_REFILL_BELOW_GLOBAL_BVH 56
#endif
// ... 5 lines not shown
#endif
#ifndef PT_WAVES_LDS_BVH
#define PT_WAVES_LDS_BVH 5
#endif
#ifndef PT_WAVES_LDS_BVH_ANY
#define PT_WAVES_LDS_BVH_ANY 5
#endif
#ifndef PT_WAVES_GLOBAL_BVH
#define PT_WAVES_GLOBAL_BVH 5
#endif
#ifndef PT_WAVES_GLOBAL_BVH_ANY
#define PT_WAVES_GLOBAL_BVH_ANY 5
#endif
#ifndef PT_TRACE_WAVES_LDS_IDENT
#define PT_TRACE_WAVES_LDS_IDENT 6
#endif
constexpr uint32_t trace_waves_cap(bool lds, bool ident) { return lds && ident ? PT_TRACE_WAVES_LDS_IDENT : 0; }
#ifndef PT_BRANCH_LEVELS
#define PT_BRANCH_LEVELS 4
#endif
#ifndef PT_BRANCH_LEVELS_ANY
#define PT_BRANCH_LEVELS_ANY 4
#endif
#ifndef PT_BRANCH_LEVELS_INLINE
#define PT_BRANCH_LEVELS_INLINE 6
#endif
#ifndef PT_ACC_QUAD_BELOW
#define PT_ACC_QUAD_BELOW (1u << 30)
#endif
#ifndef PT_STEP_STATS
#define PT_STEP_STATS 0
#endif
#ifndef PT_WAVE_TIMES
#define PT_WAVE_TIMES 0
#endif
#ifndef PT_MIN_GENERATIONS
#define PT_MIN_GENERATIONS 1
#endif
#ifndef PT_STRIPE_DIV
#define PT_STRIPE_DIV 64
#endif
#ifndef PT_REGIONS_PER_STRIPE
#define PT_REGIONS_PER_STRIPE 256
#endif
#ifndef PT_REGION_DIV
#define PT_REGION_DIV 16
#endif
#ifndef PT_TAPER
#define PT_TAPER 2
#endif
#ifndef PT_TAPER_ANY
#define PT_TAPER_ANY 0
#endif
#ifndef PT_RESERVICE
#define PT_RESERVICE 1
#endif
#ifndef PT_CLAIM_AHEAD
#define PT_CLAIM_AHEAD 0
#endif
#ifndef PT_SHADE_WAVES
#define PT_SHADE_WAVES 5
#endif
#ifndef PT_SHADE_WAVES_DIEL
#define PT_SHADE_WAVES_DIEL 5
#endif
#ifndef PT_SHADE_WAVES_GGX
#define PT_SHADE_WAVES_GGX 5
#endif
#ifndef PT_SHADE_WAVES_VOLUMES
#define PT_SHADE_WAVES_VOLUMES 4
#endif
constexpr int shade_waves(uint32_t qclass, bool volumes)
{
    return volumes ? PT_SHADE_WAVES_VOLUMES : (qclass == Q_GGX ? PT_SHADE_WAVES_GGX : (qclass == Q_DIELECTRIC ? PT_SHADE_WAVES_DIEL : PT_SHADE_WAVES));
}
#ifndef PT_INLINE_SHADOW
#define PT_INLINE_SHADOW 1
#endif
#ifndef PT_IDENT_SHADE
#define PT_IDENT_SHADE 1
#endif
#ifndef PT_SHADE_WAVES_INLINE
#define PT_SHADE_WAVES_INLINE 5
#endif
#ifndef PT_SHADE_THREADS
#define PT_SHADE_THREADS 256
#endif
#ifndef PT_CHUNK_MAX
#define PT_CHUNK_MAX 1024
#endif
#ifndef PT_CHUNK_DIV
#define PT_CHUNK_DIV 4
#endif
#ifndef PT_CHUNK_DIV_GLOBAL_BVH
#define PT_CHUNK_DIV_GLOBAL_BVH 16
#endif
template <bool LDS_SCENE> struct Refill
{
    static constexpr int kSteps = LDS_SCENE ? PT_STEPS_PER_ROUND : PT_STEPS_PER_ROUND_GLOBAL_BVH;
    static constexpr int kStepsAny = LDS_SCENE ? PT_STEPS_ANY : PT_STEPS_PER_ROUND_GLOBAL_BVH;
    static constexpr int kBelow = LDS_SCENE ? PT_REFILL_BELOW : PT_REFILL_BELOW_GLOBAL_BVH;
    static constexpr int kBelowAny = LDS_SCENE ? PT_REFILL_BELOW_ANY : PT_REFILL_BELOW_GLOBAL_BVH;
};

__device__ __forceinline__ uint32_t fastdiv(uint32_t n, const FastDiv& f)
{
    const uint32_t q = __umulhi(f.magic, n);
    const uint32_t t = ((n - q) >> 1) + q;
    return f.one ? n : (t >> f.shift);
}
__device__ __forceinline__ uint32_t lane_id() { return threadIdx.x & 63u; }
__device__ __forceinline__ uint32_t mbcnt64(uint64_t m)
{
    return __builtin_amdgcn_mbcnt_hi((uint32_t)(m >> 32), __builtin_amdgcn_mbcnt_lo((uint32_t)m, 0u));
}
struct FetchPlan
{
    uint32_t n;
    uint32_t chunk;
    uint32_t n_static;
    uint32_t psize;
    uint32_t lvl;
    uint32_t blocks;
};
__device__ __forceinline__ bool chunk_of(const FetchPlan& pl, uint32_t i, uint32_t& start, uint32_t& len)
{
    uint32_t rem = pl.psize, base = 0u;
    const uint32_t e64 = min(rem, pl.lvl); rem -= e64;
    const uint32_t e128 = min(rem, 2u * pl.lvl); rem -= e128;
    const uint32_t e256 = min(rem, 4u * pl.lvl); rem -= e256;
    const uint32_t e512 = min(rem, 8u * pl.lvl); rem -= e512;
    const uint32_t e1024 = rem;
#define PT_LEVEL(E, C)                                                                                     \
    {                                                                                                      \
        const uint32_t c = min((uint32_t)(C), pl.chunk), cnt = ((E) + c - 1u) / c;                          \
        if (i < cnt) { start = base + i * c; len = min(c, (E) - i * c); return true; }                      \
        i -= cnt;                                                                                          \
        base += (E);                                                                                       \
    }
    PT_LEVEL(e1024, 1024u) PT_LEVEL(e512, 512u) PT_LEVEL(e256, 256u) PT_LEVEL(e128, 128u) PT_LEVEL(e64, 64u)
#undef PT_LEVEL
    return false;
}
__device__ __forceinline__ FetchPlan fetch_plan(uint32_t n, uint32_t chunk_div, uint32_t taper)
{
    FetchPlan pl;
    const uint32_t wpb = blockDim.x >> 6;
    const uint32_t need_waves = (n + 63u) >> 6;
    pl.blocks = min(gridDim.x, (need_waves + wpb * (uint32_t)PT_MIN_GENERATIONS - 1u) / (wpb * (uint32_t)PT_MIN_GENERATIONS));
    const uint32_t waves = max(pl.blocks, 1u) * wpb;
    uint32_t c = n / (waves * chunk_div);
    c = c < 64u ? 64u : (c > (uint32_t)PT_CHUNK_MAX ? (uint32_t)PT_CHUNK_MAX : c);
    pl.chunk = (c + 63u) & ~63u;
    pl.n = n;
    const uint64_t st = (uint64_t)waves * pl.chunk;
    pl.n_static = st >= n ? n : (uint32_t)st;
    const uint32_t units = (n - pl.n_static + 63u) >> 6;
    pl.psize = ((units + kQueueHeads - 1u) / kQueueHeads) << 6;
    pl.lvl = taper ? ((taper * waves * 64u / kQueueHeads + 63u) & ~63u) : 0u;
    return pl;
}
struct WaveRange
{
    uint32_t cur, end;
    uint32_t home;
    bool drained;
// ... 274 lines not shown
__device__ __forceinline__ bool tri_in_range(const TriEval& e, float t_min, float t_mx) { return !sign_differs(e.td - e.det * t_min, e.det * t_mx - e.td); }

struct Blob
{
    const uint4* nodes;
    const uint4* tris;
    const uint4* inst;
    const uint2* leaves;
};
__device__ __forceinline__ void leaf_range(const Blob& bl, uint32_t kind, uint32_t payload, uint32_t& first, uint32_t& count)
{
    if (kind == NODE_TRIS) { first = payload & LEAF_FIRST_MASK; count = (payload >> LEAF_FIRST_BITS) + 1u; }
    else { const uint2 lf = bl.leaves[payload]; first = lf.x; count = lf.y; }
}

struct LaneRay { f3 o, d, inv; };

__device__ __forceinline__ void pin(uint4& v) { asm volatile("" : "+v"(v.x), "+v"(v.y), "+v"(v.z), "+v"(v.w)); }
template <bool EAGER, bool ROOT_BOX>
__device__ __forceinline__ LaneRay to_object(const Blob& bl, uint32_t inst, const LaneRay& w, bool ray_finite, uint4& root0, uint4& root1)
{
    const uint4* ip = bl.inst + INST_WORDS * inst;
    uint4 r0, r1, r2;
    if (EAGER)
    {
        r0 = ip[0]; r1 = ip[1]; r2 = ip[2];
    }
    const uint4 meta = ip[INST_META_WORD];
    if (ROOT_BOX) { root0 = ip[INST_ROOT_WORD]; root1 = ip[INST_ROOT_WORD + 1u]; }
    else root0.w = reinterpret_cast<const uint32_t*>(ip + INST_ROOT_WORD)[3];
    if (EAGER) { pin(r0); pin(r1); pin(r2); }
    LaneRay r;
    if ((meta.w & INSTANCE_IDENTITY) != 0u && ray_finite)
    {
        const uint32_t so = asu(w.o.x) & asu(w.o.y) & asu(w.o.z) & 0x80000000u;
        const uint32_t sd = asu(w.d.x) & asu(w.d.y) & asu(w.d.z) & 0x80000000u;
        r.o.x = w.o.x != 0.0f ? w.o.x : asf(so);
        r.o.y = w.o.y != 0.0f ? w.o.y : asf(so);
        r.o.z = w.o.z != 0.0f ? w.o.z : asf(so);
        r.d.x = w.d.x != 0.0f ? w.d.x : asf(sd);
        r.d.y = w.d.y != 0.0f ? w.d.y : asf(sd);
        r.d.z = w.d.z != 0.0f ? w.d.z : asf(sd);
        r.inv.x = w.d.x != 0.0f ? w.inv.x : asf(sd | 0x7f800000u);
        r.inv.y = w.d.y != 0.0f ? w.inv.y : asf(sd | 0x7f800000u);
        r.inv.z = w.d.z != 0.0f ? w.inv.z : asf(sd | 0x7f800000u);
        return r;
    }
    if (!EAGER) { r0 = ip[0]; r1 = ip[1]; r2 = ip[2]; }
    r.o.x = ((asf(r0.x) * w.o.x + asf(r0.y) * w.o.y) + asf(r0.z) * w.o.z) + asf(r0.w);
    r.o.y = ((asf(r1.x) * w.o.x + asf(r1.y) * w.o.y) + asf(r1.z) * w.o.z) + asf(r1.w);
    r.o.z = ((asf(r2.x) * w.o.x + asf(r2.y) * w.o.y) + asf(r2.z) * w.o.z) + asf(r2.w);
    r.d.x = (asf(r0.x) * w.d.x + asf(r0.y) * w.d.y) + asf(r0.z) * w.d.z;
    r.d.y = (asf(r1.x) * w.d.x + asf(r1.y) * w.d.y) + asf(r1.z) * w.d.z;
    r.d.z = (asf(r2.x) * w.d.x + asf(r2.y) * w.d.y) + asf(r2.z) * w.d.z;
    r.inv = rcp3(r.d);
    return r;
}

__device__ __forceinline__ LaneRay ident_ray(const LaneRay& w)
{
    const uint32_t so = asu(w.o.x) & asu(w.o.y) & asu(w.o.z) & 0x80000000u;
    const uint32_t sd = asu(w.d.x) & asu(w.d.y) & asu(w.d.z) & 0x80000000u;
    LaneRay r;
    r.o.x = w.o.x != 0.0f ? w.o.x : asf(so);
    r.o.y = w.o.y != 0.0f ? w.o.y : asf(so);
    r.o.z = w.o.z != 0.0f ? w.o.z : asf(so);
    r.d.x = w.d.x != 0.0f ? w.d.x : asf(sd);
    r.d.y = w.d.y != 0.0f ? w.d.y : asf(sd);
    r.d.z = w.d.z != 0.0f ? w.d.z : asf(sd);
    r.inv = w.inv;
    return r;
}
__device__ __forceinline__ uint32_t ray_signs(const LaneRay& w)
{
    return (asu(w.o.x) >> 31) | ((asu(w.o.y) >> 31) << 1) | ((asu(w.o.z) >> 31) << 2) |
           ((asu(w.d.x) >> 31) << 3) | ((asu(w.d.y) >> 31) << 4) | ((asu(w.d.z) >> 31) << 5);
}
__device__ __forceinline__ f3 with_signs(const f3 v, uint32_t bits)
{
    return f3{asf((asu(v.x) & 0x7fffffffu) | ((bits & 1u) << 31)), asf((asu(v.y) & 0x7fffffffu) | (((bits >> 1) & 1u) << 31)),
              asf((asu(v.z) & 0x7fffffffu) | (((bits >> 2) & 1u) << 31))};
}

__device__ __forceinline__ Blob blob_at(const SceneView& sv, const uint4* base)
{
    Blob b;
    b.nodes = base;
    b.tris = base + 2u * sv.n_nodes;
    b.inst = base + 2u * sv.n_nodes + 3u * sv.n_tris;
    b.leaves = reinterpret_cast<const uint2*>(base + 2u * sv.n_nodes + 3u * sv.n_tris + INST_WORDS * sv.n_instances);
    return b;
}
template <bool LDS_SCENE>
__device__ __forceinline__ Blob stage_scene(const SceneView& sv, const uint4* __restrict__ gblob, uint4* smem, uint32_t& words)
{
    const uint4* base = gblob;
    words = 0;
    if (LDS_SCENE)
    {
        words = sv.blob_bytes >> 4;
        for (uint32_t i = threadIdx.x; i < words; i += blockDim.x) smem[i] = gblob[i];
        __syncthreads();
        base = smem;
    }
    return blob_at(sv, base);
}

enum { CLOSEST_WORLD = 0, CLOSEST_LIGHTS = 1, CLOSEST_HOOK = 2, CLOSEST_PRIMARY = 3, CLOSEST_PRIMARY_LENS = 4 };
constexpr bool closest_is_primary(int mode) { return mode == CLOSEST_PRIMARY || mode == CLOSEST_PRIMARY_LENS; }

struct ClosestOut
{
    f4* hits;
    f4* q_base;
    uint32_t q_stride, q_class_slot;
    uint2* q_term;
    uint32_t* n_shade;
    uint4* wave_times;
    uint32_t* tails;
    uint32_t cap_shade, cap_term;
    uint32_t class_mask;
    uint32_t* overflow;
    uint32_t world_root;
    uint8_t* occl;
    f3 eye;
    f4* radiance;
    f4* first_pos;
    uint32_t* first_id;
    uint32_t keep_s_id, keep_s_pos, blk_log, n_blk, blk_last, act_pixels;
    FastDiv div_blk_paths, div_blk_last;
    uint32_t finalize_miss;
    const DPathRec* rec;
    uint32_t enable_nee;
};

template <bool SPILL>
struct Stack8;
template <>
struct Stack8<false>
{
    char* base;
    uint32_t bottom, step;
    __device__ __forceinline__ static Stack8 make(uint4* smem, uint32_t blob_words, const SceneView&)
    {
        return Stack8{reinterpret_cast<char*>(smem), blob_words * 16u + threadIdx.x * 8u, blockDim.x * 8u};
    }
    __device__ __forceinline__ uint32_t empty() const { return bottom; }
    __device__ __forceinline__ uint32_t up(uint32_t sp) const { return sp + step; }
    __device__ __forceinline__ uint32_t down(uint32_t sp) const { return sp - step; }
    __device__ __forceinline__ uint2 get(uint32_t sp) const { return *reinterpret_cast<const uint2*>(base + sp); }
    __device__ __forceinline__ void put(uint32_t sp, uint2 v) const { *reinterpret_cast<uint2*>(base + sp) = v; }
};
template <>
struct Stack8<true>
{
    uint2* lds;
    uint2* spill;
    uint32_t stride, lds_levels, spill_stride;
    __device__ __forceinline__ static Stack8 make(uint4* smem, uint32_t blob_words, const SceneView& sv)
    {
        return Stack8{reinterpret_cast<uint2*>(smem + blob_words) + threadIdx.x,
                      reinterpret_cast<uint2*>(sv.stack_spill) + (blockIdx.x * blockDim.x + threadIdx.x), blockDim.x, sv.stack_lds, gridDim.x * blockDim.x};
    }
    __device__ __forceinline__ uint32_t empty() const { return 0u; }
    __device__ __forceinline__ uint32_t up(uint32_t sp) const { return sp + 1u; }
    __device__ __forceinline__ uint32_t down(uint32_t sp) const { return sp - 1u; }
// ... 48 lines not shown
    }
};
struct WaveTimes
{
#if PT_WAVE_TIMES
    uint32_t start = (uint32_t)wall_clock64(), first = 0u, drained = 0u;
#endif
    __device__ __forceinline__ void check_drained(bool no_more)
    {
#if PT_WAVE_TIMES
        if (no_more && drained == 0u) drained = (uint32_t)wall_clock64() | 1u;
#endif
    }
    __device__ __forceinline__ void check_first(uint32_t take)
    {
#if PT_WAVE_TIMES
        if (first == 0u && take != 0u) first = (uint32_t)wall_clock64() | 1u;
#endif
    }
    __device__ __forceinline__ void write(uint4* times)
    {
#if PT_WAVE_TIMES
        if (lane_id() == 0u && times)
        {
            const uint32_t end = (uint32_t)wall_clock64();
            if (drained == 0u) drained = end;
            if (first == 0u) first = start;
            const uint32_t w = blockIdx.x * (blockDim.x >> 6) + (threadIdx.x >> 6);
            if (w < kWaveTimeSlots) times[w] = make_uint4(start, first, drained, end | 1u);
        }
#endif
    }
};
#if PT_WAVE_TIMES
__device__ uint4* g_any_times = nullptr;
#else
constexpr uint4* g_any_times = nullptr;
#endif

template <typename Radiance>
__device__ __forceinline__ void apply_shadow(DPathRec* rec, bool ends, bool blocked, Radiance&& radiance)
{
    if (ends)
    {
        const f3 e = blocked ? f3{0.0f, 0.0f, 0.0f} : xyz(rec->nee_e);
        const f3 acc = xyz(rec->acc) + xyz(rec->nee_pw) * (e + f3{0.0f, 0.0f, 0.0f});
        radiance() = f4{acc.x, acc.y, acc.z, 0.0f};
    }
    else if (blocked)
    {
        float* e = reinterpret_cast<float*>(&rec->nee_e);
        e[0] = 0.0f; e[1] = 0.0f; e[2] = 0.0f;
    }
}

struct ClosestKArgs
{
    SceneView sv;
    const uint4* gblob;
    const f4* ra;
    const f4* rb;
    const uint32_t* n_ptr;
    uint32_t* heads;
    uint32_t root, cap_in;
    ClosestOut out;
};
typedef const __attribute__((address_space(4))) ClosestKArgs* ClosestKArgsPtr;
typedef const __attribute__((address_space(4))) ClosestOut* ClosestOutPtr;
__device__ __forceinline__ ClosestOutPtr launder_args(ClosestOutPtr p)
{
    asm volatile("" : "+s"(p));
    return p;
}
template <int BVH, int MODE, bool SPILL, bool IDENT>
__device__ __forceinline__ void closest_body(const SceneView& sv, const Blob& bl, const uint32_t blob_words, uint4* smem, const uint32_t root, const f4* __restrict__ ra,
                                             const f4* __restrict__ rb, const uint32_t* __restrict__ n_ptr, const uint32_t cap_in,
                                             uint32_t* __restrict__ heads, const ClosestOutPtr outp)
{
    constexpr bool LDS_SCENE = BVH != 0;
    const FetchPlan plan = fetch_plan(min(*n_ptr, cap_in), LDS_SCENE ? (uint32_t)PT_CHUNK_DIV : (uint32_t)PT_CHUNK_DIV_GLOBAL_BVH, (uint32_t)PT_TAPER);
    if (blockIdx.x >= plan.blocks) return;
    const Stack8<SPILL> stk = Stack8<SPILL>::make(smem, blob_words, sv);
    const uint32_t prim_bits = sv.prim_bits;

    bool active = false, pending = false, ray_finite = false;
    uint32_t ray_idx = 0, pid = 0;
    LaneRay w{}, ob{};
    uint32_t w_signs = 0u;
    float t_max = 0.0f, bt = 0.0f;
    float hud = 0.0f, hvd = 0.0f, hdet = 1.0f;
    uint32_t bid = MISS_ID, sp = stk.empty(), blas_base = 0, inst = 0;
    bool in_blas = false;
    bool any_phase = false;
    uint32_t chain_code = 0u;
    WaveRange wr = first_range(plan, heads);
    uint32_t light_hits = 0, valid_rays = 0;
    StepStats ss;
    WaveTimes wt;
    Region bin_region[Q_COUNT];
#pragma unroll
    for (uint32_t c = 0; c < Q_COUNT; ++c) bin_region[c] = Region{0u, 0u};
    const uint32_t lights_world_root = MODE == CLOSEST_LIGHTS ? outp->world_root : 0u;
    const uint32_t rsize = outp->finalize_miss != 0u ? 64u : region_size(plan.n, plan.blocks * (blockDim.x >> 6), 64u);
    const Stripes stripes = stripes_for(plan.n);
    uint32_t stripe_rot = blockIdx.x * (blockDim.x >> 6) + __builtin_amdgcn_readfirstlane(threadIdx.x >> 6);

    for (;;)
    {
        uint64_t act = __ballot(active);
        const bool no_more = wr.drained && wr.cur >= wr.end;
        wt.check_drained(no_more);
        const bool service = no_more ? (act == 0ull) : (__popcll(act) <= Refill<LDS_SCENE>::kBelow);
        if (service)
        {
            const ClosestOutPtr out = launder_args(outp);
            const uint64_t pm = __ballot(pending);
            if (pm != 0ull)
            {
                if (MODE == CLOSEST_WORLD || closest_is_primary(MODE))
                {
                    if (IDENT && pending) { w.o = with_signs(ob.o, w_signs); w.d = with_signs(ob.d, w_signs >> 3); }
                    uint64_t qm = pm;
                    if (closest_is_primary(MODE))
                    {
                        const bool missed = pending && bid == MISS_ID && out->finalize_miss != 0u;
                        if (pending) out->occl[ray_idx] = missed ? (uint8_t)PRIMARY_MISS : (uint8_t)0u;
                        if (!missed && pending && bid == MISS_ID)
                        {
                            const FastDiv dbp{out->div_blk_paths.magic, out->div_blk_paths.shift, out->div_blk_paths.one, out->div_blk_paths.d};
                            const FastDiv dbl{out->div_blk_last.magic, out->div_blk_last.shift, out->div_blk_last.one, out->div_blk_last.d};
                            const uint32_t b = fastdiv(ray_idx, dbp), rem = ray_idx - b * (out->act_pixels << out->blk_log);
                            const bool short_blk = b + 1u == out->n_blk;
                            const uint32_t k = short_blk ? fastdiv(rem, dbl) : (rem >> out->blk_log);
                            const uint32_t sl = (b << out->blk_log) + (rem - k * (short_blk ? out->blk_last : (1u << out->blk_log)));
                            if (sl >= out->keep_s_id) out->first_id[(sl - out->keep_s_id) * out->act_pixels + k] = 255u;
                            if (sl == out->keep_s_pos)
                            {
                                const f3 far = fma3(w.d, bc3(1e5f), w.o);
                                out->first_pos[k] = f4{far.x, far.y, far.z, 1e5f};
                            }
                        }
                        qm = __ballot(pending && !missed);
                        pending = pending && !missed;
                    }
                    if (MODE == CLOSEST_WORLD)
                    {
                        bool ends = false, emissive = false;
                        uint32_t mat_id = 0;
                        if (pending)
                        {
                            if (bid == MISS_ID) ends = out->finalize_miss != 0u;
                            else
                            {
                                const uint4 meta = bl.inst[INST_WORDS * (bid >> prim_bits) + INST_META_WORD];
                                emissive = ends = (meta.w & 0xffu) == (uint32_t)Q_TERMINAL;
                                mat_id = meta.z;
                            }
                        }
                        if (ends)
                        {
                            const DPathRec& rec = out->rec[pid];
                            const f4 acc4 = rec.acc;
                            const uint32_t flags = asu(acc4.w);
                            if (!(flags & FLAG_BSDF_CAST))
                            {
                                f3 acc = xyz(acc4);
// ... 49 lines not shown
                    if (pending)
                    {
                        out->occl[pid] = (uint8_t)chain_code;
                        if (chain_code == 0u) out->hits[ray_idx] = f4{bt, hud / hdet, hvd / hdet, asf(bid)};
                    }
                }
                else
                {
                    if (pending) out->hits[ray_idx] = f4{bt, hud / hdet, hvd / hdet, asf(bid)};
                }
                pending = false;
            }
            if (no_more) break;
            const uint64_t idle = ~act;
            uint32_t first;
            const uint32_t take = claim_rays(wr, heads, plan, (uint32_t)__popcll(idle), first);
            const uint32_t rank = mbcnt64(idle);
            if (!active && rank < take)
            {
                const uint32_t mine = first + rank;
                const f4 b = rb[mine];
                ray_idx = mine;
                pid = asu(b.w);
                if (pid != HOLE) {
                valid_rays += 1u;
                if (MODE == CLOSEST_PRIMARY)
                {
                    w.o = f3{out->eye.x, out->eye.y, out->eye.z};
                    t_max = asf(0x7f800000u);
                }
                else
                {
                    const f4 a = ra[mine];
                    w.o = xyz(a);
                    t_max = a.w;
                }
                w.d = xyz(b);
                w.inv = rcp3(w.d);
                ray_finite = finite3(w.o) && finite3(w.d);
                if (IDENT) { ob = ident_ray(w); w_signs = ray_signs(w); }
                bid = MISS_ID;
                any_phase = false;
                chain_code = 2u;
                bt = asf(0x7f800000u);
                hud = 0.0f;
                hvd = 0.0f;
                hdet = 1.0f;
                in_blas = false;
                sp = stk.empty();
                float te;
                const uint4 root0 = bl.nodes[2u * root];
                const bool ok = (t_max == t_max) && (!IDENT || ray_finite) && slab(root0, bl.nodes[2u * root + 1u], IDENT ? ob.o : w.o, w.inv, t_max, te);
                if (ok)
                {
                    stk.put(sp, make_uint2(root0.w, 0u));
                    sp = stk.up(sp);
                    active = true;
                }
                else { pending = true; }
                }
            }
            wt.check_first(take);
            act = __ballot(active);
            if (act == 0ull) continue;
            if (PT_RESERVICE && take < (uint32_t)__popcll(idle) && !wr.drained && (uint32_t)__popcll(act) <= (uint32_t)Refill<LDS_SCENE>::kBelow) continue;
        }

#pragma unroll 1
        for (int it = 0; it < Refill<LDS_SCENE>::kSteps; ++it)
        {
            ss.step(active);
            if (!active) continue;
            if (!IDENT && in_blas && sp == blas_base) in_blas = false;
            if (MODE == CLOSEST_LIGHTS && any_phase)
            {
                if (sp == stk.empty()) { active = false; pending = true; chain_code = 0u; continue; }
                sp = stk.down(sp);
                const uint2 e = stk.get(sp);
                uint32_t link = e.x;
                float t_enter = asf(e.y);
                if ((link >> NODE_KIND_SHIFT) == NODE_INSTANCE)
                {
                    uint4 r0, r1;
                    if (IDENT)
                    {
                        const uint4* ip = bl.inst + INST_WORDS * (link & NODE_PAYLOAD_MASK) + INST_ROOT_WORD;
                        r0 = ip[0]; r1 = ip[1];
                    }
                    else
                    {
                        ob = to_object<!LDS_SCENE, true>(bl, link & NODE_PAYLOAD_MASK, w, ray_finite, r0, r1);
                        in_blas = true;
                        blas_base = sp;
                    }
                    if (!slab(r0, r1, ob.o, ob.inv, t_max, t_enter)) continue;
                    link = r0.w;
                }
                const uint32_t kkind = link >> NODE_KIND_SHIFT, kpay = link & NODE_PAYLOAD_MASK;
                if (kkind == NODE_BRANCH)
                {
                    const uint4* cp = bl.nodes + 2u * kpay;
                    const uint4 l0 = cp[0], l1 = cp[1], r0 = cp[2], r1 = cp[3];
                    const f3 so = (IDENT || in_blas) ? ob.o : w.o, sinv = (IDENT || in_blas) ? ob.inv : w.inv;
                    float tl, tr;
                    const bool hl = slab(l0, l1, so, sinv, t_max, tl);
                    const bool hr = slab(r0, r1, so, sinv, t_max, tr);
                    if (hl) { stk.put(sp, make_uint2(l0.w, asu(tl))); sp = stk.up(sp); }
                    if (hr) { stk.put(sp, make_uint2(r0.w, asu(tr))); sp = stk.up(sp); }
                }
                else
                {
                    uint32_t first, count;
                    leaf_range(bl, kkind, kpay, first, count);
                    for (uint32_t k = 0; k < count; ++k)
                    {
                        const uint4* tp = bl.tris + 3u * (first + k);
                        float td, ud, vd, det;
                        if (tri_planes(tp[0], tp[1], tp[2], ob.o, ob.d, t_max, t_enter, td, ud, vd, det))
                        {
                            active = false;
                            pending = true;
                            chain_code = 1u;
                            break;
                        }
                    }
                }
                continue;
            }
            if (sp == stk.empty())
            {
                if (MODE == CLOSEST_LIGHTS && bid != MISS_ID)
                {
                    light_hits += 1u;
                    any_phase = true;
                    in_blas = false;
                    t_max = bt * (1.0f - PT_EPSILON);
                    float te = 0.0f;
                    const uint4 wr0 = bl.nodes[2u * lights_world_root];
                    if (t_max == t_max && slab(wr0, bl.nodes[2u * lights_world_root + 1u], IDENT ? ob.o : w.o, IDENT ? ob.inv : w.inv, t_max, te)) { stk.put(sp, make_uint2(wr0.w, asu(te))); sp = stk.up(sp); }
                    else { active = false; pending = true; chain_code = 0u; }
                    continue;
                }
                active = false;
                pending = true;
                continue;
            }
            sp = stk.down(sp);
            const uint2 e = stk.get(sp);
            if (asf(e.y) > t_max) continue;
            uint32_t link = e.x;
            float t_est = asf(e.y);
            ss.section(StepStats::INST, (link >> NODE_KIND_SHIFT) == NODE_INSTANCE);
            if ((link >> NODE_KIND_SHIFT) == NODE_INSTANCE)
            {
                uint4 root0, root1;
                inst = link & NODE_PAYLOAD_MASK;
                if (IDENT) root0.w = reinterpret_cast<const uint32_t*>(bl.inst + INST_WORDS * inst + INST_ROOT_WORD)[3];
                else
                {
                    ob = to_object<!LDS_SCENE, false>(bl, inst, w, ray_finite, root0, root1);
                    in_blas = true;
                    blas_base = sp;
                }
                if (0.0f > t_max) continue;
                link = root0.w;
                t_est = 0.0f;
            }
            uint32_t kind = link >> NODE_KIND_SHIFT, payload = link & NODE_PAYLOAD_MASK;
            ss.section(StepStats::BRANCH, kind == NODE_BRANCH);
#pragma unroll 1
            for (int lvl = 0; lvl < PT_BRANCH_LEVELS && kind == NODE_BRANCH; ++lvl)
            {
                const uint4* cp = bl.nodes + 2u * payload;
                const uint4 l0 = cp[0], l1 = cp[1], r0 = cp[2], r1 = cp[3];
                const f3 o = (IDENT || in_blas) ? ob.o : w.o, inv = (IDENT || in_blas) ? ob.inv : w.inv;
                float tl, tr;
                const bool hl = slab(l0, l1, o, inv, t_max, tl);
                const bool hr = slab(r0, r1, o, inv, t_max, tr);
                const bool left_near = tl < tr;
                const uint2 le = make_uint2(l0.w, asu(tl)), re = make_uint2(r0.w, asu(tr));
                if (hl && hr) { stk.put(sp, left_near ? re : le); sp = stk.up(sp); }
                kind = NODE_INSTANCE;
                if (hl || hr)
                {
                    const uint2 near = (hl && (left_near || !hr)) ? le : re;
                    const uint32_t nk = near.x >> NODE_KIND_SHIFT;
                    if ((nk & 1u) != 0u || (nk == NODE_BRANCH && lvl + 1 < PT_BRANCH_LEVELS))
                    {
                        kind = nk;
                        payload = near.x & NODE_PAYLOAD_MASK;
                        t_est = asf(near.y);
                    }
                    else { stk.put(sp, near); sp = stk.up(sp); }
                }
            }
            ss.section(StepStats::LEAF, (kind & 1u) != 0u);
            if (kind & 1u)
            {
                uint32_t first, count;
                leaf_range(bl, kind, payload, first, count);
                const f3 mo = fma3(ob.d, bc3(t_est), ob.o);
                const float t_min = PT_EPSILON - t_est;
                auto accept = [&](const TriEval& e, uint32_t tri) {
                    if (e.uv_ok && tri_in_range(e, t_min, t_max - t_est))
                    {
                        bt = e.td / e.det + t_est;
                        hud = e.ud;
                        hvd = e.vd;
                        hdet = e.det;
                        t_max = bt;
                        bid = (inst << prim_bits) | tri;
                    }
                };
                for (uint32_t k = 0; k < count; ++k) accept(tri_eval(bl.tris + 3u * (first + k), mo, ob.d), first + k);
                if (bt != bt) { sp = stk.empty(); in_blas = false; }
            }
        }
    }
    if (MODE == CLOSEST_WORLD || closest_is_primary(MODE))
    {
        const ClosestOutPtr out = launder_args(outp);
        const f4 hole{0.0f, 0.0f, 0.0f, asf(HOLE)};
        for (uint32_t i = bin_region[Q_TERMINAL].cur + lane_id(); i < bin_region[Q_TERMINAL].end; i += 64u) out->q_term[i] = make_uint2(HOLE, 0u);
#pragma unroll
        for (uint32_t c = 1; c < Q_COUNT; ++c)
        {
            f4* const qa = out->q_base + (size_t)(3u * ((out->q_class_slot >> (4u * c)) & 0xfu)) * out->q_stride;
            for (uint32_t i = bin_region[c].cur + lane_id(); i < bin_region[c].end; i += 64u) qa[i] = hole;
        }
    }
    wt.write(outp->wave_times);
    ss.flush(heads);
    if (MODE != CLOSEST_HOOK) add_tally(heads, valid_rays, HEAD_TALLY0);
    if (MODE == CLOSEST_LIGHTS) add_tally(heads, light_hits, HEAD_TALLY1);
}
template <int BVH, int MODE, bool SPILL, bool IDENT = false>
__global__ void __launch_bounds__(256, BVH != 0 ? PT_WAVES_LDS_BVH : PT_WAVES_GLOBAL_BVH) k_closest(const ClosestKArgs a)
{
    constexpr bool LDS_SCENE = BVH != 0;
    extern __shared__ uint4 smem[];
    if (blockIdx.x >= fetch_plan(min(*a.n_ptr, a.cap_in), LDS_SCENE ? (uint32_t)PT_CHUNK_DIV : (uint32_t)PT_CHUNK_DIV_GLOBAL_BVH, (uint32_t)PT_TAPER).blocks) return;
    uint32_t blob_words;
    const Blob bl = stage_scene<LDS_SCENE>(a.sv, a.gblob, smem, blob_words);
    const ClosestOutPtr outp = &((ClosestKArgsPtr)__builtin_amdgcn_kernarg_segment_ptr())->out;
    closest_body<BVH, MODE, SPILL, IDENT>(a.sv, bl, blob_words, smem, a.root, a.ra, a.rb, a.n_ptr, a.cap_in, a.heads, outp);
}

enum { ANY_SHADOW = 0, ANY_HOOK = 2 };

template <int BVH, int MODE, bool SPILL, bool IDENT>
__device__ __forceinline__ void any_body(const SceneView& sv, const Blob& bl, const uint32_t blob_words, uint4* smem, const uint32_t root, const f4* __restrict__ ra,
                                         const f4* __restrict__ rb, const uint32_t* __restrict__ n_ptr, const uint32_t cap_in,
                                         uint32_t* __restrict__ heads, uint32_t* __restrict__ occluded,
                                         f4* __restrict__ radiance)
{
    constexpr bool LDS_SCENE = BVH != 0;
    const FetchPlan plan = fetch_plan(min(*n_ptr, cap_in), LDS_SCENE ? (uint32_t)PT_CHUNK_DIV : (uint32_t)PT_CHUNK_DIV_GLOBAL_BVH, (uint32_t)PT_TAPER_ANY);
    if (blockIdx.x >= plan.blocks) return;
    const Stack8<SPILL> stk = Stack8<SPILL>::make(smem, blob_words, sv);

    bool active = false, ray_finite = false;
    uint32_t out_idx = 0, valid_rays = 0;
    LaneRay w{}, ob{};
    float t_max = 0.0f;
    uint32_t sp = stk.empty(), blas_base = 0;
    bool path_ends = false;
    auto put_result_at = [&](uint32_t idx, bool ends, uint32_t v) {
        if (MODE == ANY_SHADOW) apply_shadow(reinterpret_cast<DPathRec*>(occluded) + idx, ends, v != 0u, [&]() -> f4& { return radiance[idx]; });
        else occluded[idx] = v;
    };
    auto put_result = [&](uint32_t v) { put_result_at(out_idx, path_ends, v); };
    bool in_blas = false;
    WaveTimes wt;
    StepStats ss;
    WaveRange wr = first_range(plan, heads);

    for (;;)
    {
        uint64_t act = __ballot(active);
        const bool no_more = wr.drained && wr.cur >= wr.end;
        wt.check_drained(no_more);
        const bool service = no_more ? (act == 0ull) : (__popcll(act) <= Refill<LDS_SCENE>::kBelowAny);
        if (service)
        {
            if (no_more) break;
            const uint64_t idle = ~act;
            uint32_t first;
            const uint32_t take = claim_rays(wr, heads, plan, (uint32_t)__popcll(idle), first);
            const uint32_t rank = mbcnt64(idle);
            if (!active && rank < take)
            {
                const uint32_t mine = first + rank;
                const f4 a = ra[mine], b = rb[mine];
                const uint32_t tag = asu(b.w);
                if (tag != HOLE) {
                valid_rays += 1u;
                path_ends = MODE == ANY_SHADOW && (tag & PATH_ENDS) != 0u;
                out_idx = (MODE == ANY_HOOK) ? mine : (tag & ~PATH_ENDS);
                w.o = xyz(a);
                w.d = xyz(b);
                w.inv = rcp3(w.d);
                ray_finite = finite3(w.o) && finite3(w.d);
                if (IDENT) ob = ident_ray(w);
                t_max = a.w;
                in_blas = false;
                sp = stk.empty();
                float te;
                const uint4 root0 = bl.nodes[2u * root];
                const bool ok = (t_max == t_max) && (!IDENT || ray_finite) && slab(root0, bl.nodes[2u * root + 1u], IDENT ? ob.o : w.o, w.inv, t_max, te);
                if (ok)
                {
                    stk.put(sp, make_uint2(root0.w, asu(te)));
                    sp = stk.up(sp);
                    active = true;
                }
                else put_result(0u);
                }
            }
            act = __ballot(active);
            if (act == 0ull) continue;
            if (PT_RESERVICE && take < (uint32_t)__popcll(idle) && !wr.drained && (uint32_t)__popcll(act) <= (uint32_t)Refill<LDS_SCENE>::kBelowAny) continue;
        }

#pragma unroll 1
        for (int it = 0; it < Refill<LDS_SCENE>::kStepsAny; ++it)
        {
            ss.step(active);
            if (!active) continue;
            if (!IDENT && in_blas && sp == blas_base) in_blas = false;
            if (sp == stk.empty())
            {
                active = false;
                put_result(0u);
                continue;
            }
            sp = stk.down(sp);
            const uint2 e = stk.get(sp);
            uint32_t link = e.x;
            float t_enter = asf(e.y);
            ss.section(StepStats::INST, (link >> NODE_KIND_SHIFT) == NODE_INSTANCE);
            if ((link >> NODE_KIND_SHIFT) == NODE_INSTANCE)
            {
                uint4 r0, r1;
                if (IDENT)
                {
                    const uint4* ip = bl.inst + INST_WORDS * (link & NODE_PAYLOAD_MASK) + INST_ROOT_WORD;
                    r0 = ip[0]; r1 = ip[1];
                }
                else
                {
                    ob = to_object<!LDS_SCENE, true>(bl, link & NODE_PAYLOAD_MASK, w, ray_finite, r0, r1);
                    in_blas = true;
                    blas_base = sp;
                }
                if (!slab(r0, r1, ob.o, ob.inv, t_max, t_enter)) continue;
                link = r0.w;
            }
            uint32_t kind = link >> NODE_KIND_SHIFT, payload = link & NODE_PAYLOAD_MASK;
            ss.section(StepStats::BRANCH, kind == NODE_BRANCH);
#pragma unroll 1
            for (int lvl = 0; lvl < PT_BRANCH_LEVELS_ANY && kind == NODE_BRANCH; ++lvl)
            {
                const uint4* cp = bl.nodes + 2u * payload;
                const uint4 l0 = cp[0], l1 = cp[1], r0 = cp[2], r1 = cp[3];
                const f3 o = (IDENT || in_blas) ? ob.o : w.o, inv = (IDENT || in_blas) ? ob.inv : w.inv;
                float tl, tr;
                const bool hl = slab(l0, l1, o, inv, t_max, tl);
                const bool hr = slab(r0, r1, o, inv, t_max, tr);
                if (hl && hr) { stk.put(sp, make_uint2(l0.w, asu(tl))); sp = stk.up(sp); }
                kind = NODE_INSTANCE;
                if (hl || hr)
                {
                    const uint2 next = hr ? make_uint2(r0.w, asu(tr)) : make_uint2(l0.w, asu(tl));
                    const uint32_t nk = next.x >> NODE_KIND_SHIFT;
                    if ((nk & 1u) != 0u || (nk == NODE_BRANCH && lvl + 1 < PT_BRANCH_LEVELS_ANY))
                    {
                        kind = nk;
                        payload = next.x & NODE_PAYLOAD_MASK;
                        t_enter = asf(next.y);
                    }
                    else { stk.put(sp, next); sp = stk.up(sp); }
                }
            }
            ss.section(StepStats::LEAF, (kind & 1u) != 0u);
            if (kind & 1u)
            {
                uint32_t first, count;
                leaf_range(bl, kind, payload, first, count);
                for (uint32_t k = 0; k < count; ++k)
                {
                    const uint4* tp = bl.tris + 3u * (first + k);
                    float td, ud, vd, det;
                    if (tri_planes(tp[0], tp[1], tp[2], ob.o, ob.d, t_max, t_enter, td, ud, vd, det))
                    {
                        active = false;
                        put_result(1u);
                        break;
                    }
                }
            }
        }
    }
    if (MODE == ANY_SHADOW)
    {
        ss.flush(heads);
        add_tally(heads, valid_rays, HEAD_TALLY0);
        wt.write(g_any_times);
    }
}
template <int BVH, int MODE, bool SPILL, bool IDENT = false>
__global__ void __launch_bounds__(256, BVH != 0 ? PT_WAVES_LDS_BVH_ANY : PT_WAVES_GLOBAL_BVH_ANY) k_any(const SceneView sv, const uint4* __restrict__ gblob, const uint32_t root, const f4* __restrict__ ra,
                                              const f4* __restrict__ rb, const uint32_t* __restrict__ n_ptr, const uint32_t cap_in,
                                              uint32_t* __restrict__ heads, uint32_t* __restrict__ occluded,
                                              f4* __restrict__ radiance)
{
    constexpr bool LDS_SCENE = BVH != 0;
    extern __shared__ uint4 smem[];
    if (blockIdx.x >= fetch_plan(min(*n_ptr, cap_in), LDS_SCENE ? (uint32_t)PT_CHUNK_DIV : (uint32_t)PT_CHUNK_DIV_GLOBAL_BVH, (uint32_t)PT_TAPER_ANY).blocks) return;
    uint32_t blob_words;
    const Blob bl = stage_scene<LDS_SCENE>(sv, gblob, smem, blob_words);
    any_body<BVH, MODE, SPILL, IDENT>(sv, bl, blob_words, smem, root, ra, rb, n_ptr, cap_in, heads, occluded, radiance);
}

struct FusedArgs
{
    const f4 *wa, *wb;
    const uint32_t* wn;
    uint32_t* wheads;
    const f4 *la, *lb;
    const uint32_t* ln;
    uint32_t* lheads;
    uint32_t world_root, lights_root, cap_in;
};
struct FusedKArgs
{
    SceneView sv;
    const uint4* gblob;
    FusedArgs fa;
    ClosestOut wout, lout;
// ... 187 lines not shown
            const DInstance& in = sv.instances[inst];
            const DMaterial& lm = sv.materials[in.material];
            const f3 emitted{lm.colour[0], lm.colour[1], lm.colour[2]};
            const DTriIsect ti = sv.tri_isect[tri];
            const float area = 0.5f * len3(xyz(ti.n0));
            const float sample_pdf = (area * len3(emitted) / sv.light_weight_sum) / area;
            const f3 dir = xyz(io.rq_lchain_prev.b[slot]);
            bool ff;
            const f3 ln = hit_normal(sv, inst, tri, lh.y, lh.z, dir, ff);
            const float cosine = fabsf(dot3(dir, ln));
            const float light_pdf = sample_pdf * (lh.x * lh.x / cosine);
            const float weight = mis2(pw4.w, light_pdf);
            s = emitted * weight * b4.w * xyz(b4) / pw4.w;
        }
    }
    acc = acc + xyz(pw4) * (e + s);
    flags &= ~(FLAG_NEE_PENDING | FLAG_BSDF_CAST);
}

template <bool LENS = false>
__global__ void __launch_bounds__(256) k_shade_terminal(const SceneView sv, const RenderParams rp, const ShadeIO io, const uint32_t bounce)
{
    const uint32_t n = min(io.ctr->n_shade[Q_TERMINAL], io.cap_slots_term);
    for (uint32_t idx = blockIdx.x * blockDim.x + threadIdx.x; idx < n; idx += gridDim.x * blockDim.x)
    {
        const uint2 e2 = io.entries[idx];
        const uint32_t entry = e2.x, pid = e2.y;
        if (entry == HOLE) continue;
        const bool dead = (entry & ENTRY_DEAD) != 0u;
        f4 ra{}, rb{}, hit{};
        if (!dead)
        {
            hit = io.hits[entry];
            if (asu(hit.w) != MISS_ID)
            {
                ra = (!LENS && bounce == 0u) ? io.primary_a : io.rq_in.a[entry];
                rb = io.rq_in.b[entry];
            }
            else if (io.env.w != 0u) rb = io.rq_in.b[entry];
        }
        f3 acc{0.0f, 0.0f, 0.0f};
        uint32_t flags = 0u;
        if (bounce != 0u)
        {
            const DPathRec& rec = io.st.rec[pid];
            const f4 acc4 = rec.acc;
            acc = xyz(acc4);
            flags = asu(acc4.w);
            resolve_nee(sv, io, pid, rec, acc, flags);
        }
        if (!dead)
        {
            const f3 pw = bounce == 0u ? f3{1.0f, 1.0f, 1.0f} : xyz(io.st.rec[pid].pw);
            const uint32_t hid = asu(hit.w);
            if (hid == MISS_ID)
            {
                if (io.env.w != 0u) acc = acc + env_lookup(io.env, xyz(rb)) * pw;
                else acc = acc + f3{0.006f, 0.006f, 0.006f} * pw;
            }
            else
            {
                const uint32_t inst = hid >> sv.prim_bits;
                const DInstance& in = sv.instances[inst];
                if (bounce == 0u)
                {
                    const PidParts pp = pid_split(rp, pid);
                    if (pp.s == rp.keep_s_pos)
                    {
                        const f3 p = fma3(xyz(rb), bc3(hit.x), xyz(ra));
                        io.st.first_pos[pp.k] = f4{p.x, p.y, p.z, hit.x};
                    }
                    if (pp.s >= rp.keep_s_id) io.st.first_id[(pp.s - rp.keep_s_id) * rp.act_pixels + pp.k] = in.blas & 0xffu;
                }
                const DMaterial& m = sv.materials[in.material];
                if (!rp.enable_nee || (flags & FLAG_LAST_DELTA) || bounce == 0u)
                    acc = fma3(f3{m.colour[0], m.colour[1], m.colour[2]}, pw, acc);
            }
        }
        io.st.radiance[pid] = f4{acc.x, acc.y, acc.z, 0.0f};
    }
}

template <bool IDENT>
__device__ __forceinline__ bool inline_any(const Blob& bl, const Stack8<false>& stk, const uint32_t root, const f4 ra, const f4 rb, const bool want)
{
    bool active = false, blocked = false, in_blas = false, ray_finite = false;
    LaneRay w{}, ob{};
    const float t_max = ra.w;
    uint32_t sp = stk.empty(), blas_base = 0u;
    if (want)
    {
        w.o = xyz(ra);
        w.d = xyz(rb);
        w.inv = rcp3(w.d);
        ray_finite = finite3(w.o) && finite3(w.d);
        if (IDENT) ob = ident_ray(w);
        float te;
        const uint4 root0 = bl.nodes[2u * root];
        if ((t_max == t_max) && (!IDENT || ray_finite) && slab(root0, bl.nodes[2u * root + 1u], IDENT ? ob.o : w.o, w.inv, t_max, te))
        {
            stk.put(sp, make_uint2(root0.w, asu(te)));
            sp = stk.up(sp);
            active = true;
        }
    }
    while (__ballot(active) != 0ull)
    {
        if (!active) continue;
        if (!IDENT && in_blas && sp == blas_base) in_blas = false;
        if (sp == stk.empty()) { active = false; continue; }
        sp = stk.down(sp);
        const uint2 e = stk.get(sp);
        uint32_t link = e.x;
        float t_enter = asf(e.y);
        if ((link >> NODE_KIND_SHIFT) == NODE_INSTANCE)
        {
            uint4 r0, r1;
            if (IDENT)
            {
                const uint4* ip = bl.inst + INST_WORDS * (link & NODE_PAYLOAD_MASK) + INST_ROOT_WORD;
                r0 = ip[0]; r1 = ip[1];
            }
            else
            {
                ob = to_object<false, true>(bl, link & NODE_PAYLOAD_MASK, w, ray_finite, r0, r1);
                in_blas = true;
                blas_base = sp;
            }
            if (!slab(r0, r1, ob.o, ob.inv, t_max, t_enter)) continue;
            link = r0.w;
        }
        uint32_t kind = link >> NODE_KIND_SHIFT, payload = link & NODE_PAYLOAD_MASK;
#pragma unroll 1
        for (int lvl = 0; lvl < PT_BRANCH_LEVELS_INLINE && kind == NODE_BRANCH; ++lvl)
        {
            const uint4* cp = bl.nodes + 2u * payload;
            const uint4 l0 = cp[0], l1 = cp[1], r0 = cp[2], r1 = cp[3];
            const f3 o = (IDENT || in_blas) ? ob.o : w.o, inv = (IDENT || in_blas) ? ob.inv : w.inv;
            float tl, tr;
            const bool hl = slab(l0, l1, o, inv, t_max, tl);
            const bool hr = slab(r0, r1, o, inv, t_max, tr);
            if (hl && hr) { stk.put(sp, make_uint2(l0.w, asu(tl))); sp = stk.up(sp); }
            kind = NODE_INSTANCE;
            if (hl || hr)
            {
                const uint2 next = hr ? make_uint2(r0.w, asu(tr)) : make_uint2(l0.w, asu(tl));
                const uint32_t nk = next.x >> NODE_KIND_SHIFT;
                if ((nk & 1u) != 0u || (nk == NODE_BRANCH && lvl + 1 < PT_BRANCH_LEVELS_INLINE))
                {
                    kind = nk;
                    payload = next.x & NODE_PAYLOAD_MASK;
                    t_enter = asf(next.y);
                }
                else { stk.put(sp, next); sp = stk.up(sp); }
            }
        }
        if (kind & 1u)
        {
            uint32_t first, count;
            leaf_range(bl, kind, payload, first, count);
            for (uint32_t k = 0; k < count; ++k)
            {
                const uint4* tp = bl.tris + 3u * (first + k);
                float td, ud, vd, det;
                if (tri_planes(tp[0], tp[1], tp[2], ob.o, ob.d, t_max, t_enter, td, ud, vd, det))
                {
                    active = false;
                    blocked = true;
                    break;
                }
            }
        }
    }
    return blocked;
}

struct ShadeKArgs { SceneView sv; RenderParams rp; ShadeIO io; uint32_t bounce; const uint4* gblob; uint32_t world_root; };
typedef const __attribute__((address_space(4))) ShadeKArgs* ShadeKArgsPtr;
__device__ __forceinline__ const ShadeKArgs& shade_args()
{
    ShadeKArgsPtr p = (ShadeKArgsPtr)__builtin_amdgcn_kernarg_segment_ptr();
    asm volatile("" : "+s"(p));
    return *(const ShadeKArgs*)p;
}
struct ShadeKArgsTex : ShadeKArgs { TexView tex; };
typedef const __attribute__((address_space(4))) ShadeKArgsTex* ShadeKArgsTexPtr;
__device__ __forceinline__ const TexView& shade_args_tex()
{
    ShadeKArgsTexPtr p = (ShadeKArgsTexPtr)__builtin_amdgcn_kernarg_segment_ptr();
    asm volatile("" : "+s"(p));
    return ((const ShadeKArgsTex*)p)->tex;
}
#define PT_SHADE_ARGS                                                                                                              \
    const ShadeKArgs& ka_ = shade_args();                                                                                          \
    [[maybe_unused]] const SceneView& sv = ka_.sv;                                                                                 \
    [[maybe_unused]] const RenderParams& rp = ka_.rp;                                                                              \
    [[maybe_unused]] const ShadeIO& io = ka_.io;
#ifndef PT_TEX_EARLY
#define PT_TEX_EARLY 0
#endif
template <uint32_t QCLASS, bool VOLUMES, bool INLINE = false, bool IDENT = false, bool LIST = false, bool LENS = false, bool RAYS = false, bool TEX = false,
          bool ONE_DRAW = false>
__global__ void __launch_bounds__(PT_SHADE_THREADS, INLINE ? PT_SHADE_WAVES_INLINE : shade_waves(QCLASS, VOLUMES))
k_shade_surface(const std::conditional_t<TEX, ShadeKArgsTex, ShadeKArgs> kargs)
{
    static_assert(!(TEX && INLINE), "textured scenes queue their shadow rays");
    extern __shared__ uint4 smem_dyn[];
    const ShadeIO& io = kargs.io;
    const uint32_t bounce = kargs.bounce;
    __shared__ BlockAppend sh_append;
    __shared__ uint32_t sh_tail[kTailStripes];
    __shared__ uint32_t sh_extent;
    const Stripes stripes = stripes_for(min(io.ctr->n_closest, io.cap_slots));
// ... 202 lines not shown
                        sh_a = f4{p.x, p.y, p.z, (1.0f - PT_EPSILON) * dist};
                        sh_b = f4{dir.x, dir.y, dir.z, asf(pid)};
                    }
                    nee_e = f4{ce.x, ce.y, ce.z, 0.0f};
                }
                {
                    PT_SHADE_ARGS
                    const f3 dir = mat_scatter(mat, rng, rd, normal, front);
                    if (dot3(dir, normal) > 0.0f)
                    {
                        const BsdfSample bp = mat_bsdf_pdf(mat, wi, dir, normal, front);
                        float te;
                        const uint4* const lr = reinterpret_cast<const uint4*>(sv.nodes + sv.lights_root);
                        const bool may_hit = slab(lr[0], lr[1], p, rcp3(dir), asf(0x7f800000u), te);
                        if (may_hit)
                        {
                            nee_b = f4{bp.bsdf.x, bp.bsdf.y, bp.bsdf.z, mat_weakening(mat.kind, dir, normal)};
                            nee_pw.w = bp.pdf;
                            want_lchain = true;
                            lc_a = f4{p.x, p.y, p.z, asf(0x7f800000u)};
                            lc_b = f4{dir.x, dir.y, dir.z, asf(pid)};
                            flags |= FLAG_BSDF_CAST;
                        }
                        else if (!INLINE) culled += 1u;
                        else cull_now = true;
                    }
                }
                nee_pw.x = pw.x; nee_pw.y = pw.y; nee_pw.z = pw.z;
                flags |= FLAG_NEE_PENDING;
            }

            ndir = mat_scatter(mat, rng, rd, normal, front);
            const BsdfSample info = mat_bsdf_pdf(mat, wi, ndir, normal, front);
            alive = !(info.pdf < 0.0f);
            if (alive)
            {
                pw = pw * (mat_weakening(mat.kind, ndir, normal) * info.bsdf / info.pdf);
                flags = is_delta ? (flags | FLAG_LAST_DELTA) : (flags & ~FLAG_LAST_DELTA);
            }
            }
            if (alive)
            {
                {
                const uint32_t nb = bounce + 1u;
                if (nb > rp.max_bounces) alive = false;
                else if (nb > 3u)
                {
                    const float survive = min_num(hmax3(pw), 0.9999f);
                    if (rng.f32() > survive) alive = false;
                    else pw = pw / survive;
                }
                }
            }
            if (alive && VOLUMES && (vst != vst_in || bounce == 0u)) io.st.vstack[pid] = vst;
            draws = rng.k;
            if (alive)
            {
                want_next = true;
                nx_a = f4{next_o.x, next_o.y, next_o.z, asf(0x7f800000u)};
                nx_b = f4{ndir.x, ndir.y, ndir.z, asf(pid)};
            }
            else if (flags & FLAG_NEE_PENDING)
            {
                if (flags & FLAG_BSDF_CAST) want_dead = true;
                else if (want_shadow) { ends_with_shadow = true; sh_b.w = asf(pid | PATH_ENDS); }
                else acc = acc + xyz(nee_pw) * (xyz(nee_e) + f3{0.0f, 0.0f, 0.0f});
            }
        }
        PT_SHADE_ARGS
        uint32_t* const ctrs[4] = {&io.ctr->n_shadow, &io.ctr->n_lchain, &io.ctr_next->n_closest, &io.ctr_next->n_shade[Q_TERMINAL]};
        const bool preds[4] = {want_shadow && !INLINE, want_lchain, want_next, want_dead};
        const uint32_t caps[4] = {io.cap_slots, io.cap_slots, io.cap_slots, io.cap_slots_term};
        uint32_t pos[4];
        block_append4(sh_append, ctrs, preds, caps, &io.ctr->overflow, pos);
        if (want_shadow && !INLINE) { nt_store(io.rq_shadow.a + pos[0], sh_a); nt_store(io.rq_shadow.b + pos[0], sh_b); }
        if (want_lchain) { io.rq_lchain.a[pos[1]] = lc_a; io.rq_lchain.b[pos[1]] = lc_b; io.lchain_nb[pos[1]] = nee_b; nee_e.w = asf(pos[1]); }
        if (want_next) { nt_store(io.rq_out.a + pos[2], nx_a); nt_store(io.rq_out.b + pos[2], nx_b); }
        if (want_dead) io.q_term_next[pos[3]] = make_uint2(pid | ENTRY_DEAD, pid);
        const bool write_rec = valid && (want_next || want_dead || ends_with_shadow);
        if (valid && !write_rec) io.st.radiance[pid] = f4{acc.x, acc.y, acc.z, 0.0f};
        {
            float m[4][4] = {{pw.x, pw.y, pw.z, asf(draws)}, {acc.x, acc.y, acc.z, asf(flags)}, {nee_e.x, nee_e.y, nee_e.z, nee_e.w}, {nee_pw.x, nee_pw.y, nee_pw.z, nee_pw.w}};
            const uint32_t q = threadIdx.x & 3u;
#pragma unroll
            for (int c = 0; c < 4; ++c)
            {
                float a0 = m[0][c], a1 = m[1][c], a2 = m[2][c], a3 = m[3][c];
                { const float t = (q & 1u) ? a0 : a1; const float r = asf(__builtin_amdgcn_mov_dpp(asu(t), 0xB1, 0xF, 0xF, true)); if (q & 1u) a0 = r; else a1 = r; }
                { const float t = (q & 1u) ? a2 : a3; const float r = asf(__builtin_amdgcn_mov_dpp(asu(t), 0xB1, 0xF, 0xF, true)); if (q & 1u) a2 = r; else a3 = r; }
                { const float t = (q & 2u) ? a0 : a2; const float r = asf(__builtin_amdgcn_mov_dpp(asu(t), 0x4E, 0xF, 0xF, true)); if (q & 2u) a0 = r; else a2 = r; }
                { const float t = (q & 2u) ? a1 : a3; const float r = asf(__builtin_amdgcn_mov_dpp(asu(t), 0x4E, 0xF, 0xF, true)); if (q & 2u) a1 = r; else a3 = r; }
                m[0][c] = a0; m[1][c] = a1; m[2][c] = a2; m[3][c] = a3;
            }
            const uint32_t wr = write_rec ? 1u : 0u;
#define PT_QUAD_STORE(K, SEL)                                                                                                   \
            {                                                                                                                      \
                const uint32_t pid_k = __builtin_amdgcn_mov_dpp(pid, SEL, 0xF, 0xF, true);                \
                const uint32_t wr_k = __builtin_amdgcn_mov_dpp(wr, SEL, 0xF, 0xF, true);                                           \
                if (wr_k != 0u) reinterpret_cast<f4*>(io.st.rec + pid_k)[q] = f4{m[K][0], m[K][1], m[K][2], m[K][3]};             \
            }
            PT_QUAD_STORE(0, 0x00) PT_QUAD_STORE(1, 0x55) PT_QUAD_STORE(2, 0xAA) PT_QUAD_STORE(3, 0xFF)
#undef PT_QUAD_STORE
        }
        if (INLINE)
        {
            uint32_t tid = threadIdx.x;
            asm volatile("" : "+v"(tid));
            const ShadeKArgs& ka2 = shade_args();
            const uint32_t blob_words = ka2.sv.blob_bytes >> 4;
            const Blob bl = blob_at(ka2.sv, smem_dyn);
            const Stack8<false> stk{reinterpret_cast<char*>(smem_dyn), blob_words * 16u + tid * 8u, blockDim.x * 8u};
            traced += (uint32_t)__popcll(__ballot(want_shadow));
            culled += (uint32_t)__popcll(__ballot(cull_now));
            const bool blocked = inline_any<IDENT>(bl, stk, ka2.world_root, sh_a, sh_b, want_shadow);
            if (want_shadow) apply_shadow(shade_args().io.st.rec + pid, ends_with_shadow, blocked, [&]() -> f4& { return shade_args().io.st.radiance[pid]; });
            a_next = (idx + stride) < n ? nt_load(shade_args().io.q_in.a + idx + stride) : hole_a;
        }
    }
    if (!INLINE) add_tally(io.lchain_heads, culled, HEAD_TALLY2);
    else if (lane_id() == 0u)
    {
        const uint32_t wave = blockIdx.x * (blockDim.x >> 6) + (threadIdx.x >> 6);
        const uint32_t line = ((wave * 7u) & (kQueueHeads - 1u)) * kHeadStrideWords;
        if (culled != 0u) atomicAdd(io.lchain_heads + line + HEAD_TALLY2, culled);
        if (traced != 0u) atomicAdd(io.shadow_heads + line + HEAD_TALLY0, traced);
    }
}

#undef PT_SHADE_ARGS

struct CameraLensView : CameraView { LensView lens; };
struct CameraProjView : CameraView { ProjView proj; };
__device__ __forceinline__ f3 miss_position(const RenderParams& rp, const CameraView& cam, uint32_t gx, uint32_t gy, uint32_t sample)
{
    const f3 d = camera_ray_dir(rp, cam, gx, gy, sample);
    return fma3(d, bc3(1e5f), f3{cam.eye[0], cam.eye[1], cam.eye[2]});
}
__device__ __forceinline__ f3 miss_position(const RenderParams& rp, const CameraLensView& cam, uint32_t gx, uint32_t gy, uint32_t sample)
{
    f3 o;
    const f3 d = camera_ray(rp, cam, cam.lens, gx, gy, sample, &o);
    return fma3(d, bc3(1e5f), o);
}
__device__ __forceinline__ f3 miss_position(const RenderParams& rp, const CameraProjView& cam, uint32_t gx, uint32_t gy, uint32_t sample)
{
    f3 o;
    const f3 d = camera_ray_projected(rp, cam, cam.proj, gx, gy, sample, &o);
    return fma3(d, bc3(1e5f), o);
}

__device__ __forceinline__ f3 finalise(f3 acc)
{
    if (!finite3(acc)) return f3{0.0f, 0.0f, 0.0f};
    return clamp_len_max(acc, 100.0f);
}

__device__ __forceinline__ float luminance(float r, float g, float b) { return (0.2126f * r + 0.7152f * g) + 0.0722f * b; }

template <bool FEW_PIXELS, bool MOMENTS = false, bool LIST = false, bool LENS = false, bool PROJ = false>
__global__ void __launch_bounds__(256) k_accumulate(const RenderParams rp,
                                                     const std::conditional_t<PROJ, CameraProjView, std::conditional_t<LENS, CameraLensView, CameraView>> cam, const PathState st,
                                                     f4* accum, f4* position, uint32_t* id, const uint32_t write_position, const uint32_t add_to_accum,
                                                     float* moments, const uint2* list)
{
    const uint32_t tid = blockIdx.x * blockDim.x + threadIdx.x;
    const uint32_t t = FEW_PIXELS ? tid >> 2 : tid, q = FEW_PIXELS ? (tid & 3u) : 0u;
    if (t >= (LIST ? rp.act_pixels : rp.local_pixels)) return;
    uint2 entry{t, 0u};
    if (LIST) entry = list[t];
    const uint32_t lp = entry.x;
    f4 a = accum[lp];
    float qv = 0.0f;
    if (MOMENTS) qv = moments[lp];
    uint32_t idv = id[lp];
    const uint32_t ly = fastdiv(lp, rp.div_width), x = lp - ly * rp.width;
    if (!LIST && (x - rp.act_x0 >= rp.act_w || ly - rp.act_ly0 >= rp.act_rows))
    {
        for (uint32_t s = 0; s < rp.batch_samples; ++s)
        {
            a = f4{a.x + 0.006f, a.y + 0.006f, a.z + 0.006f, a.w + 1.0f};
            if (MOMENTS) { const float l = luminance(0.006f, 0.006f, 0.006f); qv = qv + l * l; }
        }
        for (uint32_t s = rp.batch_samples >= 2u ? rp.batch_samples - 2u : 0u; s < rp.batch_samples; ++s) idv = (idv << 16) | 255u;
        if (q != 0u) return;
        if (add_to_accum) accum[lp] = a;
        if (MOMENTS && add_to_accum) moments[lp] = qv;
        id[lp] = idv;
        if (write_position)
        {
            const f3 far = miss_position(rp, cam, x, global_row(rp, ly), rp.first_sample + rp.batch_samples - 1u);
            position[lp] = f4{far.x, far.y, far.z, 1e5f};
        }
        return;
    }
    const uint32_t k = LIST ? t : (ly - rp.act_ly0) * rp.act_w + (x - rp.act_x0);
    if (FEW_PIXELS)
    {
// ... 179 lines not shown
    const uint32_t base = blockIdx.x * kSelectPerBlock;
    uint32_t mine = 0u;
    bool any_bad = false;
#pragma unroll
    for (uint32_t j = 0; j < kSelectPerBlock / 256u; ++j)
    {
        const uint32_t p = base + j * 256u + threadIdx.x;
        if (p >= n_pixels) break;
        uint32_t n_p;
        bool bad;
        mine += adaptive_active(accum[p], moments[p], cr, n_p, bad) ? 1u : 0u;
        any_bad |= bad;
    }
    if (any_bad) atomicOr(header + 1, 1u);
    uint32_t w = mine;
    for (int off = 32; off > 0; off >>= 1) w += (uint32_t)__shfl_xor((int)w, off);
    if (lane_id() == 0u) sh_cnt[threadIdx.x >> 6] = w;
    __syncthreads();
    if (threadIdx.x == 0u) counts[blockIdx.x] = sh_cnt[0] + sh_cnt[1] + sh_cnt[2] + sh_cnt[3];
}
__global__ void __launch_bounds__(256) k_adaptive_write(const f4* __restrict__ accum, const float* __restrict__ moments, const uint32_t n_pixels,
                                                        const AdaptiveCrit cr, const uint32_t* __restrict__ counts, uint2* list, uint32_t* header)
{
    __shared__ uint32_t sh_sum[4];
    __shared__ uint32_t sh_wave[kSelectPerBlock / 256u][4];
    const uint32_t wid = threadIdx.x >> 6;
    uint32_t before = 0u;
    for (uint32_t b = threadIdx.x; b < blockIdx.x; b += 256u) before += counts[b];
    for (int off = 32; off > 0; off >>= 1) before += (uint32_t)__shfl_xor((int)before, off);
    if (lane_id() == 0u) sh_sum[wid] = before;
    const uint32_t base = blockIdx.x * kSelectPerBlock;
    bool act[kSelectPerBlock / 256u];
    uint32_t np[kSelectPerBlock / 256u];
    uint64_t m[kSelectPerBlock / 256u];
#pragma unroll
    for (uint32_t j = 0; j < kSelectPerBlock / 256u; ++j)
    {
        const uint32_t p = base + j * 256u + threadIdx.x;
        bool bad;
        np[j] = 0u;
        act[j] = p < n_pixels && adaptive_active(accum[p], moments[p], cr, np[j], bad);
        m[j] = __ballot(act[j]);
        if (lane_id() == 0u) sh_wave[j][wid] = (uint32_t)__popcll(m[j]);
    }
    __syncthreads();
    uint32_t off = sh_sum[0] + sh_sum[1] + sh_sum[2] + sh_sum[3];
#pragma unroll
    for (uint32_t j = 0; j < kSelectPerBlock / 256u; ++j)
    {
        uint32_t pos = off;
        for (uint32_t w2 = 0; w2 < wid; ++w2) pos += sh_wave[j][w2];
        if (act[j]) list[pos + mbcnt64(m[j])] = uint2{base + j * 256u + threadIdx.x, np[j]};
        off += sh_wave[j][0] + sh_wave[j][1] + sh_wave[j][2] + sh_wave[j][3];
    }
    if (blockIdx.x + 1u == gridDim.x && threadIdx.x == 0u) header[0] = off;
}

__global__ void k_sobol_probe(uint32_t n_points, uint32_t n, const uint32_t* index, const uint32_t* seed, float* out)
{
    const uint32_t i = blockIdx.x * blockDim.x + threadIdx.x;
    if (i >= n) return;
    ss_sobol(n_points, index[i], seed[i], &out[2 * i], &out[2 * i + 1]);
}
__global__ void k_math_probe(int fn, uint32_t n, const float* a, const float* b, float* o0, float* o1, uint64_t seed)
{
    const uint32_t i = blockIdx.x * blockDim.x + threadIdx.x;
    if (i >= n) return;
    switch (fn)
    {
    case 0: sincos_det(a[i], &o0[i], &o1[i]); break;
    case 1: o0[i] = exp_det(a[i]); break;
    case 2: o0[i] = ln_det(a[i]); break;
    case 3: o0[i] = hypot_det(a[i], b[i]); break;
    case 4: o0[i] = a[i] / b[i]; break;
    case 5: o0[i] = sqrtf(a[i]); break;
    case 6: o0[i] = tan_det(a[i]); break;
    case 8: o0[i] = atan2_det(a[i], b[i]); break;
    case 9: o0[i] = asin_det(a[i]); break;
    case 7:
    {
        Stream r{stream_key(seed, asu(a[i]), asu(b[i])), 0u};
        o0[i] = asf(r.u32());
        o1[i] = r.f32();
        break;
    }
    }
}
__global__ void k_material_probe(const SceneView sv, int material, uint32_t n, const float* incoming, const float* normal, const uint8_t* front,
                                 const uint32_t* pixel, const uint32_t* sample, uint32_t draws, uint64_t seed, float* out9)
{
    const uint32_t i = blockIdx.x * blockDim.x + threadIdx.x;
    if (i >= n) return;
    const MatView m = load_material(sv.materials, (uint32_t)material);
    Stream rng{stream_key(seed, pixel[i], sample[i]), draws};
    const f3 in{incoming[3 * i], incoming[3 * i + 1], incoming[3 * i + 2]}, nn{normal[3 * i], normal[3 * i + 1], normal[3 * i + 2]};
    const bool ff = front[i] != 0;
    const f3 wo = mat_scatter(m, rng, in, nn, ff);
    const BsdfSample bp = mat_bsdf_pdf(m, -in, wo, nn, ff);
    float* o = out9 + 9 * i;
    o[0] = wo.x; o[1] = wo.y; o[2] = wo.z;
    o[3] = bp.bsdf.x; o[4] = bp.bsdf.y; o[5] = bp.bsdf.z;
    o[6] = bp.pdf;
    o[7] = mat_weakening(m.kind, wo, nn);
    o[8] = (float)(rng.k - draws);
}

__global__ void k_volume_probe(const SceneView sv, int material, uint32_t n, const float* incoming, const float* t_max, const float* dist,
                               const uint32_t* pixel, const uint32_t* sample, uint32_t draws, uint64_t seed, float* out9)
{
    const uint32_t i = blockIdx.x * blockDim.x + threadIdx.x;
    if (i >= n) return;
    const DMaterial& dm = sv.materials[material];
    Stream rng{stream_key(seed, pixel[i], sample[i]), draws};
    const f3 rd{incoming[3 * i], incoming[3 * i + 1], incoming[3 * i + 2]};
    float* o = out9 + 9 * i;
    o[0] = 0.0f; o[1] = 0.0f; o[2] = 0.0f; o[3] = 0.0f; o[4] = 0.0f;
    if (dm.vol_flags & 2u)
    {
        const float t = -ln_det(rng.f32()) / dm.vol_c;
        if (!(t > t_max[i]))
        {
            const f3 d = hg_direction(dm.vol_g, rng, rd);
            o[0] = 1.0f; o[1] = t; o[2] = d.x; o[3] = d.y; o[4] = d.z;
        }
    }
    f3 w{1.0f, 1.0f, 1.0f};
    if (dm.vol_flags & 1u) w = beer_lambert(f3{dm.vol_abs[0], dm.vol_abs[1], dm.vol_abs[2]}, dist[i]);
    o[5] = w.x; o[6] = w.y; o[7] = w.z;
    o[8] = (float)(rng.k - draws);
}

__global__ void __launch_bounds__(256) k_guide_rays(const RenderParams rp, const CameraView cam, const RayQueue rq, uint32_t* __restrict__ n_and_heads)
{
    const uint32_t i = blockIdx.x * blockDim.x + threadIdx.x;
    if (i == 0u) n_and_heads[0] = rp.local_pixels;
    if (i >= rp.local_pixels) return;
    const uint32_t ly = fastdiv(i, rp.div_width), x = i - ly * rp.width;
    const f3 dir = camera_ray_dir(rp, cam, x, global_row(rp, ly), rp.first_sample);
    rq.a[i] = f4{cam.eye[0], cam.eye[1], cam.eye[2], __builtin_inff()};
    rq.b[i] = f4{dir.x, dir.y, dir.z, asf(i)};
}
__global__ void __launch_bounds__(256) k_guide_rays_lens(const RenderParams rp, const CameraView cam, const LensView lens, const RayQueue rq,
                                                          uint32_t* __restrict__ n_and_heads)
{
    const uint32_t i = blockIdx.x * blockDim.x + threadIdx.x;
    if (i == 0u) n_and_heads[0] = rp.local_pixels;
    if (i >= rp.local_pixels) return;
    const uint32_t ly = fastdiv(i, rp.div_width), x = i - ly * rp.width;
    f3 o;
    const f3 dir = camera_ray(rp, cam, lens, x, global_row(rp, ly), rp.first_sample, &o);
    rq.a[i] = f4{o.x, o.y, o.z, __builtin_inff()};
    rq.b[i] = f4{dir.x, dir.y, dir.z, asf(i)};
}
template <uint32_t KIND>
__global__ void __launch_bounds__(256) k_guide_rays_proj(const RenderParams rp, const CameraView cam, const ProjView proj, const RayQueue rq,
                                                          uint32_t* __restrict__ n_and_heads)
{
    const uint32_t i = blockIdx.x * blockDim.x + threadIdx.x;
    if (i == 0u) n_and_heads[0] = rp.local_pixels;
    if (i >= rp.local_pixels) return;
    const uint32_t ly = fastdiv(i, rp.div_width), x = i - ly * rp.width;
    f3 o;
    const f3 dir = KIND == PROJ_PANORAMA ? camera_ray_panorama(rp, cam, proj, x, global_row(rp, ly), rp.first_sample, &o)
                                         : camera_ray_orthographic(rp, cam, proj, x, global_row(rp, ly), rp.first_sample, &o);
    rq.a[i] = f4{o.x, o.y, o.z, __builtin_inff()};
    rq.b[i] = f4{dir.x, dir.y, dir.z, asf(i)};
// ... 226 lines not shown
{
    Counters* row = wb.counters + b;
    Counters* prev = wb.counters + (b - 1u);
    const ClosestOut wout = world_out(wb, b, rp, env);
    ClosestOut lout{};
    lout.hits = wb.lchain_hit;
    lout.world_root = tl.scene.world_root;
    lout.occl = wb.st.occl;
    FusedArgs fa{};
    fa.wa = wb.rq[b & 1u].a; fa.wb = wb.rq[b & 1u].b; fa.wn = &row->n_closest; fa.wheads = row_heads(wb, b, HEADS_CLOSEST);
    fa.la = wb.rq_lchain[(b - 1u) & 1u].a; fa.lb = wb.rq_lchain[(b - 1u) & 1u].b; fa.ln = &prev->n_lchain; fa.lheads = row_heads(wb, b - 1u, HEADS_LCHAIN);
    fa.world_root = tl.scene.world_root; fa.lights_root = tl.scene.lights_root; fa.cap_in = wb.cap_slots;
    const FusedKArgs ka{tl.scene, (const uint4*)tl.blob, fa, wout, lout};
    with_trace_variant(tl, ident_walk(tl, IDENT_TLAS_WORLD | IDENT_TLAS_LIGHTS), [&](auto bvh, auto spill, auto ident) {
        launch_resident(k_trace_fused<bvh, spill, ident>, trace_waves_cap(bvh != 0, ident), tl, s, ka);
    });
}
void launch_trace_shadow(hipStream_t s, const TraceLaunch& tl, const WavefrontBuffers& wb, uint32_t b)
{
    Counters* row = wb.counters + b;
#if PT_WAVE_TIMES
    {
        uint4* where = wb.wave_times_any ? wb.wave_times_any + (size_t)b * kWaveTimeSlots : nullptr;
        (void)hipMemcpyToSymbolAsync(HIP_SYMBOL(g_any_times), &where, sizeof(where), 0, hipMemcpyHostToDevice, s);
    }
#endif
    launch_any_impl<ANY_SHADOW>(s, tl, tl.scene.world_root, wb.rq_shadow, &row->n_shadow, wb.cap_slots, row_heads(wb, b, HEADS_SHADOW),
                                reinterpret_cast<uint32_t*>(wb.st.rec), wb.st.radiance);
}
void launch_trace_lchain(hipStream_t s, const TraceLaunch& tl, const WavefrontBuffers& wb, uint32_t b)
{
    Counters* row = wb.counters + b;
    ClosestOut out{};
    out.hits = wb.lchain_hit;
    out.n_shade = nullptr;
    out.world_root = tl.scene.world_root;
    out.occl = wb.st.occl;
    launch_closest_impl<CLOSEST_LIGHTS>(s, tl, tl.scene.lights_root, wb.rq_lchain[b & 1u], &row->n_lchain, wb.cap_slots, row_heads(wb, b, HEADS_LCHAIN), out);
}
bool shade_traces_shadow(const TraceLaunch& tl)
{
    return PT_INLINE_SHADOW != 0 && !tl.tex && tl.lds_scene && tl.scene.stack_entries <= tl.scene.stack_lds && !tl.scene.has_volumes && tl.block_threads == PT_SHADE_THREADS &&
           trace_lds_bytes(tl) + 1024 <= 32 * 1024;
}
void launch_shade(hipStream_t s, uint32_t qclass, const SceneView& sv, const RenderParams& rp, const WavefrontBuffers& wb, uint32_t b,
                  uint32_t grid_blocks, const CameraView& cam, const CameraOptics& opt, const EnvView& env, const TraceLaunch* tl, const uint2* list,
                  const uint2* ray_keys)
{
    const TexView* const tex = tl ? tl->tex : nullptr;
    if (ray_keys) list = nullptr;
    const bool proj0 = b == 0u && proj_set(opt.proj) && ray_keys == nullptr;
    const bool lens0 = proj0 || (b == 0u && (lens_set(opt.lens) || ray_keys != nullptr));
    ShadeIO io{};
    io.env = env;
    io.primary_a = f4{cam.eye[0], cam.eye[1], cam.eye[2], __builtin_inff()};
    io.st = wb.st;
    io.rq_in = wb.rq[b & 1u];
    io.rq_out = wb.rq[(b + 1u) & 1u];
    io.rq_shadow = wb.rq_shadow;
    io.rq_lchain = wb.rq_lchain[b & 1u];
    io.rq_lchain_prev = wb.rq_lchain[(b + 1u) & 1u];
    io.lchain_nb = wb.lchain_nb[b & 1u];
    io.lchain_nb_prev = wb.lchain_nb[(b + 1u) & 1u];
    io.lchain_hit = wb.lchain_hit;
    io.hits = wb.hits;
    io.entries = wb.q_term[b & 1u];
    if (qclass != Q_TERMINAL)
    {
        io.q_in = shade_queue(wb, qclass);
        io.tails_in = wb.tails + ((size_t)b * Q_COUNT + qclass) * kTailWordsPerQueue;
    }
    io.q_term_next = wb.q_term[(b + 1u) & 1u];
    io.cap_slots = wb.cap_slots;
    io.cap_slots_term = wb.cap_slots_term;
    io.cap_slots_shade = wb.cap_slots_shade;
    io.ctr = wb.counters + b;
    io.lchain_heads = row_heads(wb, b, HEADS_LCHAIN);
    io.shadow_heads = row_heads(wb, b, HEADS_SHADOW);
    io.ctr_next = wb.counters + b + 1u;
    const uint32_t surface_blocks = (grid_blocks * 256u + PT_SHADE_THREADS - 1u) / PT_SHADE_THREADS;
    const bool inl = tl && shade_traces_shadow(*tl);
    if (list && qclass != Q_TERMINAL) io.list = list;
    if (ray_keys && qclass != Q_TERMINAL) io.list = ray_keys;
    const ShadeKArgs ka{sv, rp, io, b, inl ? (const uint4*)tl->blob : nullptr, inl ? tl->scene.world_root : 0u};
    const size_t lds = inl ? trace_lds_bytes(*tl) : 0;
    ShadeKArgsTex kat{};
    static_cast<ShadeKArgs&>(kat) = ka;
    if (tex) kat.tex = *tex;
#define PT_SURF_L(LENS, Q, V, ...)                                                                                                      \
    do {                                                                                                                                 \
        if (ray_keys) hipLaunchKernelGGL((k_shade_surface<Q, V, __VA_ARGS__, false, LENS, true>), dim3(surface_blocks), dim3(PT_SHADE_THREADS), lds, s, ka); \
        else if (list) hipLaunchKernelGGL((k_shade_surface<Q, V, __VA_ARGS__, true, LENS>), dim3(surface_blocks), dim3(PT_SHADE_THREADS), lds, s, ka);  \
        else hipLaunchKernelGGL((k_shade_surface<Q, V, __VA_ARGS__, false, LENS>), dim3(surface_blocks), dim3(PT_SHADE_THREADS), lds, s, ka);      \
    } while (0)
#define PT_SURF_P(Q, V, ...)                                                                                                            \
    do {                                                                                                                                 \
        if (list) hipLaunchKernelGGL((k_shade_surface<Q, V, __VA_ARGS__, true, true, false, false, true>), dim3(surface_blocks), dim3(PT_SHADE_THREADS), lds, s, ka); \
        else hipLaunchKernelGGL((k_shade_surface<Q, V, __VA_ARGS__, false, true, false, false, true>), dim3(surface_blocks), dim3(PT_SHADE_THREADS), lds, s, ka); \
    } while (0)
#define PT_SURF(Q, V, ...)                                                                                                              \
    do {                                                                                                                                 \
        if (proj0) PT_SURF_P(Q, V, __VA_ARGS__);                                                                                         \
        else if (lens0) PT_SURF_L(true, Q, V, __VA_ARGS__);                                                                              \
        else PT_SURF_L(false, Q, V, __VA_ARGS__);                                                                                        \
    } while (0)
#define PT_SURF_TEX_L(LENS, Q, V)                                                                                                       \
    do {                                                                                                                                 \
        if (ray_keys) hipLaunchKernelGGL((k_shade_surface<Q, V, false, false, false, LENS, true, true>), dim3(surface_blocks), dim3(PT_SHADE_THREADS), 0, s, kat); \
        else if (list) hipLaunchKernelGGL((k_shade_surface<Q, V, false, false, true, LENS, false, true>), dim3(surface_blocks), dim3(PT_SHADE_THREADS), 0, s, kat); \
        else hipLaunchKernelGGL((k_shade_surface<Q, V, false, false, false, LENS, false, true>), dim3(surface_blocks), dim3(PT_SHADE_THREADS), 0, s, kat); \
    } while (0)
#define PT_SURF_TEX_P(Q, V)                                                                                                            \
    do {                                                                                                                                 \
        if (list) hipLaunchKernelGGL((k_shade_surface<Q, V, false, false, true, true, false, true, true>), dim3(surface_blocks), dim3(PT_SHADE_THREADS), 0, s, kat); \
        else hipLaunchKernelGGL((k_shade_surface<Q, V, false, false, false, true, false, true, true>), dim3(surface_blocks), dim3(PT_SHADE_THREADS), 0, s, kat); \
    } while (0)
#define PT_SURF_TEX(Q)                                                                                                                  \
    do {                                                                                                                                 \
        if (proj0) { if (sv.has_volumes) PT_SURF_TEX_P(Q, true); else PT_SURF_TEX_P(Q, false); }                                        \
        else if (lens0) { if (sv.has_volumes) PT_SURF_TEX_L(true, Q, true); else PT_SURF_TEX_L(true, Q, false); }                             \
        else { if (sv.has_volumes) PT_SURF_TEX_L(false, Q, true); else PT_SURF_TEX_L(false, Q, false); }                                 \
    } while (0)
    if (tex && qclass != Q_TERMINAL)
    {
        switch (qclass)
        {
        case Q_LAMBERT: PT_SURF_TEX(Q_LAMBERT); break;
        case Q_SPECULAR: PT_SURF_TEX(Q_SPECULAR); break;
        case Q_DIELECTRIC: PT_SURF_TEX(Q_DIELECTRIC); break;
        case Q_GGX: PT_SURF_TEX(Q_GGX); break;
        default: break;
        }
        return;
    }
#undef PT_SURF_TEX
#undef PT_SURF_TEX_L
#undef PT_SURF_TEX_P
    switch (qclass)
    {
    case Q_TERMINAL:
        if (lens0) hipLaunchKernelGGL(k_shade_terminal<true>, dim3(grid_blocks), dim3(256), 0, s, sv, rp, io, b);
        else hipLaunchKernelGGL(k_shade_terminal<false>, dim3(grid_blocks), dim3(256), 0, s, sv, rp, io, b);
        break;
    case Q_LAMBERT:
        if (inl && PT_IDENT_SHADE && ident_walk(*tl, IDENT_TLAS_WORLD)) PT_SURF(Q_LAMBERT, false, true, true);
        else if (inl) PT_SURF(Q_LAMBERT, false, true, false);
        else if (sv.has_volumes) PT_SURF(Q_LAMBERT, true, false, false);
        else PT_SURF(Q_LAMBERT, false, false, false);
        break;
    case Q_SPECULAR:
        if (sv.has_volumes) PT_SURF(Q_SPECULAR, true, false, false);
        else PT_SURF(Q_SPECULAR, false, false, false);
        break;
    case Q_DIELECTRIC:
        if (sv.has_volumes) PT_SURF(Q_DIELECTRIC, true, false, false);
        else PT_SURF(Q_DIELECTRIC, false, false, false);
        break;
    case Q_GGX:
        if (sv.has_volumes) PT_SURF(Q_GGX, true, false, false);
        else PT_SURF(Q_GGX, false, false, false);
        break;
    default: break;
    }
#undef PT_SURF
#undef PT_SURF_L
#undef PT_SURF_P
}
// ... 138 lines not shown
```

### path_tracer_amd/csrc/pt_scene.cpp

```cpp
#include "pt_scene.h"
#include "pt_camera.h"

#include <algorithm>
#include <chrono>
#include <cctype>
#include <cstdio>
#include <cstdlib>
#include <cstring>
#include <exception>
#include <numeric>
#include <system_error>
#include <thread>
#include <utility>

namespace pt {

namespace {

const float kInf = __builtin_inff();

HostBox box_empty() { return HostBox{bc3(kInf), bc3(-kInf)}; }
HostBox box_join(const HostBox& a, const HostBox& b) { return HostBox{min3(a.mn, b.mn), max3(a.mx, b.mx)}; }
float box_area(const HostBox& b)
{
// ... 776 lines not shown
        }
        return true;
    };
    if (!put_tlas(world, world_base, f.inst_base[0]) || !put_tlas(lights, lights_base, f.inst_base[1]))
    {
        if (err) *err = "internal: TLAS arena holds nodes outside the tree";
        return -5;
    }
    f.world_root = world.root == MISS_ID ? MISS_ID : world_base;
    f.lights_root = lights.root == MISS_ID ? MISS_ID : lights_base;

    uint32_t max_blas_depth = 0;
    std::vector<uint32_t> blas_root_at(blas.size(), MISS_ID);
    if (!keep_blas)
    {
        f.tri_isect.reserve(tri_cursor);
        f.tri_shade.reserve(tri_cursor);
        f.tri_pos.reserve(tri_cursor);
        f.tri_orig.reserve(tri_cursor);
        if (f.has_textures)
        {
            f.tri_uv.reserve(tri_cursor);
            uint32_t at = 0;
            for (const HostTexture& t : textures)
            {
                f.tex_table.push_back(DTexture{at, t.w, t.h, 0u});
                at += t.w * t.h;
            }
            f.tex_texels.resize(at);
            for (size_t i = 0; i < textures.size(); ++i)
            {
                const HostTexture& t = textures[i];
                f4* dst = f.tex_texels.data() + f.tex_table[i].offset;
                parallel_slices((size_t)t.w * t.h, [&](size_t lo, size_t hi) {
                    for (size_t k = lo; k < hi; ++k) dst[k] = f4{t.rgb[3 * k], t.rgb[3 * k + 1], t.rgb[3 * k + 2], 0.0f};
                });
            }
        }
    }
    for (size_t i = 0; i < blas.size(); ++i)
    {
        const HostBlas& bl = blas[i];
        max_blas_depth = std::max(max_blas_depth, bl.depth);
        blas_root_at[i] = blas_base[i];
        if (keep_blas) continue;
        if (!layout(bl.nodes, bl.root, blas_base[i], slot_of)) { if (err) *err = "internal: BLAS arena holds nodes outside the tree"; return -5; }
        for (size_t n = 0; n < bl.nodes.size(); ++n)
        {
            DNode& d = f.nodes[slot_of[n]];
            put_box(d, bl.nodes[n].box);
            if (bl.nodes[n].kind == NODE_BRANCH) { d.link = (NODE_BRANCH << NODE_KIND_SHIFT) | slot_of[bl.nodes[n].a]; d.aux = slot_of[bl.nodes[n].b]; }
            else { d.link = leaf_link(f.tri_base[i] + bl.nodes[n].a, bl.nodes[n].b); d.aux = bl.nodes[n].b; }
        }
        const size_t at = f.tri_orig.size();
        f.tri_isect.resize(at + bl.prim_ids.size());
        f.tri_shade.resize(at + bl.prim_ids.size());
        f.tri_pos.resize(at + bl.prim_ids.size());
        f.tri_orig.resize(at + bl.prim_ids.size());
        parallel_slices(bl.prim_ids.size(), [&](size_t lo, size_t hi) {
            for (size_t k = lo; k < hi; ++k)
            {
                const uint32_t id = bl.prim_ids[k];
                const HostTriangle& t = bl.tris[id];
                f.tri_isect[at + k] = DTriIsect{t.n0, t.n1, t.n2};
                f.tri_shade[at + k] = DTriVerts{f4{t.n[0].x, t.n[0].y, t.n[0].z, 0}, f4{t.n[1].x, t.n[1].y, t.n[1].z, 0}, f4{t.n[2].x, t.n[2].y, t.n[2].z, 0}};
                f.tri_pos[at + k] = DTriVerts{f4{t.p[0].x, t.p[0].y, t.p[0].z, 0}, f4{t.p[1].x, t.p[1].y, t.p[1].z, 0}, f4{t.p[2].x, t.p[2].y, t.p[2].z, 0}};
                f.tri_orig[at + k] = id;
            }
        });
        if (f.has_textures)
        {
            const std::vector<float>& uv = models[i].uvs;
            f.tri_uv.resize(at + bl.prim_ids.size(), DTriUV{{0.0f, 0.0f}, {0.0f, 0.0f}, {0.0f, 0.0f}});
            if (!uv.empty())
                for (size_t k = 0; k < bl.prim_ids.size(); ++k)
                {
                    const float* p = &uv[(size_t)bl.prim_ids[k] * 6];
                    f.tri_uv[at + k] = DTriUV{{p[0], p[1]}, {p[2], p[3]}, {p[4], p[5]}};
                }
        }
    }
    auto put_instances = [&](const HostTlas& t, uint32_t ident_bit) {
        bool all_identity = true;
        for (const HostInstance& hi : t.instances)
        {
            DInstance d;
            std::memset(&d, 0, sizeof(d));
            const xf34* src[2] = {&hi.inv, &hi.fwd};
            float* dst[2] = {d.inv, d.fwd};
            for (int k = 0; k < 2; ++k)
            {
                const xf34& x = *src[k];
                const float rows[12] = {x.m.c0.x, x.m.c1.x, x.m.c2.x, x.t.x, x.m.c0.y, x.m.c1.y, x.m.c2.y, x.t.y, x.m.c0.z, x.m.c1.z, x.m.c2.z, x.t.z};
                std::memcpy(dst[k], rows, sizeof(rows));
            }
            d.root = blas_root_at[hi.model];
            d.root_node = f.nodes[d.root];
            d.blas = hi.blas;
            d.material = blas_material[hi.model];
            switch (f.materials[d.material].kind)
            {
            case MAT_LAMBERTIAN: d.qclass = Q_LAMBERT; break;
            case MAT_SPECULAR: d.qclass = Q_SPECULAR; break;
            case MAT_DIELECTRIC: d.qclass = Q_DIELECTRIC; break;
            case MAT_GGX_METAL:
            case MAT_GGX_DIELECTRIC: d.qclass = Q_GGX; break;
            default: d.qclass = Q_TERMINAL; break;
            }
            if (f.has_volumes && f.materials[d.material].kind == MAT_EMISSIVE) d.qclass = Q_LAMBERT;
            {
                static const uint32_t ident[12] = {0x3f800000u, 0, 0, 0x80000000u, 0, 0x3f800000u, 0, 0x80000000u, 0, 0, 0x3f800000u, 0x80000000u};
                if (std::memcmp(d.inv, ident, sizeof(ident)) == 0) d.qclass |= INSTANCE_IDENTITY;
                else all_identity = false;
            }
            f.instances.push_back(d);
        }
        if (all_identity) f.ident_tlas |= ident_bit;
    };
    f.ident_tlas = 0u;
    put_instances(world, IDENT_TLAS_WORLD);
    put_instances(lights, IDENT_TLAS_LIGHTS);

    std::vector<std::vector<uint32_t>> where(blas.size());
    for (const uint32_t i : lights.models)
    {
        where[i].assign(blas[i].tris.size(), 0);
        for (size_t k = 0; k < blas[i].prim_ids.size(); ++k) where[i][blas[i].prim_ids[k]] = f.tri_base[i] + (uint32_t)k;
    }
    for (const HostLight& l : light_items)
    {
        const uint32_t mi = lights.models[l.blas];
        f.lights.push_back(DLight{where[mi][l.prim], (uint32_t)blas[mi].material, l.pdf, l.cdf});
    }
    f.light_weight_sum = light_weight_sum;

    uint32_t pb = 1;
    while ((1ull << pb) < (uint64_t)std::max<uint32_t>(tri_cursor, 2)) ++pb;
    f.prim_bits = pb;
    if ((uint64_t)f.instances.size() >= (1ull << (32 - pb)) - 1) { if (err) *err = "instance x triangle id does not fit 32 bits"; return -5; }
    const uint32_t tlas_depth = std::max(world.depth, lights.depth);
    f.stack_entries = std::max(tlas_depth, (tlas_depth > 0 ? tlas_depth - 1 : 0) + max_blas_depth);
    flat = std::move(f);
    flat_valid = true;
    flat_epoch = layout_epoch;
    return 0;
}

namespace {
struct quat { float x, y, z, w; };

quat quat_mul(quat l, quat r)
{
    return quat{(l.w * r.x + l.x * r.w) + (l.y * r.z + -(l.z * r.y)),
                (l.w * r.y + -(l.x * r.z)) + (l.y * r.w + l.z * r.x),
                (l.w * r.z + l.x * r.y) + (-(l.y * r.x) + l.z * r.w),
                (l.w * r.w + -(l.x * r.x)) + (-(l.y * r.y) + -(l.z * r.z))};
}

quat quat_from_axes(f3 ax, f3 ay, f3 az)
{
    const float m00 = ax.x, m01 = ax.y, m02 = ax.z, m10 = ay.x, m11 = ay.y, m12 = ay.z, m20 = az.x, m21 = az.y, m22 = az.z;
    if (m22 <= 0.0f)
    {
        const float dif10 = m11 - m00, omm22 = 1.0f - m22;
        if (dif10 <= 0.0f)
        {
            const float four_xsq = omm22 - dif10, inv4x = 0.5f / std::sqrt(four_xsq);
            return quat{four_xsq * inv4x, (m01 + m10) * inv4x, (m02 + m20) * inv4x, (m12 - m21) * inv4x};
        }
        const float four_ysq = omm22 + dif10, inv4y = 0.5f / std::sqrt(four_ysq);
        return quat{(m01 + m10) * inv4y, four_ysq * inv4y, (m12 + m21) * inv4y, (m20 - m02) * inv4y};
    }
    const float sum10 = m11 + m00, opm22 = 1.0f + m22;
    if (sum10 <= 0.0f)
    {
        const float four_zsq = opm22 - sum10, inv4z = 0.5f / std::sqrt(four_zsq);
        return quat{(m02 + m20) * inv4z, (m12 + m21) * inv4z, four_zsq * inv4z, (m01 - m10) * inv4z};
    }
    const float four_wsq = opm22 + sum10, inv4w = 0.5f / std::sqrt(four_wsq);
    return quat{(m12 - m21) * inv4w, (m20 - m02) * inv4w, (m01 - m10) * inv4w, four_wsq * inv4w};
}

void euler_yxz_of(quat q, float* first, float* second)
{
    *first = atan2_det(2.0f * (q.x * q.z + q.w * q.y), q.w * q.w - q.x * q.x - q.y * q.y + q.z * q.z);
    float v = -2.0f * (q.y * q.z - q.w * q.x);
    v = v < -1.0f ? -1.0f : v;
    v = v > 1.0f ? 1.0f : v;
    *second = asin_det(v);
}

m33 mat3_of_quat(quat q)
{
    const float x2 = q.x + q.x, y2 = q.y + q.y, z2 = q.z + q.z;
    const float xx = q.x * x2, xy = q.x * y2, xz = q.x * z2, yy = q.y * y2, yz = q.y * z2, zz = q.z * z2, wx = q.w * x2, wy = q.w * y2, wz = q.w * z2;
    return m33{f3{1.0f - (yy + zz), xy + wz, xz - wy}, f3{xy - wz, 1.0f - (xx + zz), yz + wx}, f3{xz + wy, yz - wx, 1.0f - (xx + yy)}};
}

}

void HostScene::set_camera(const float eye_[3], const float target_[3], float fov_deg, float aspect)
{
// ... 141 lines not shown
```

### path_tracer_amd/csrc/pt_scene.h

```cpp
#pragma once
#include <string>
#include <vector>

#include "pt_types.h"

namespace pt {

struct HostBox { f3 mn, mx; };

struct HostNode
{
    HostBox box;
    uint32_t kind;
    uint32_t a, b;
};

struct HostTriangle
{
    f3 p[3], n[3];
    f4 n0, n1, n2;
};

struct HostBlas
{
    std::vector<HostTriangle> tris;
    std::vector<HostNode> nodes;
    std::vector<uint32_t> prim_ids;
    uint32_t root = 0;
    uint32_t depth = 0;
    int material = 0;
};

struct HostInstance
{
    uint32_t blas;
    uint32_t model;
    xf34 fwd, inv;
};

struct HostTlas
{
    std::vector<HostNode> nodes;
    std::vector<HostInstance> instances;
    uint32_t root = MISS_ID;
    uint32_t depth = 0;
    std::vector<uint32_t> models;
};

struct HostModel
{
    std::vector<float> positions, normals;
    std::vector<float> uvs;
    uint32_t n_tris = 0;
    int material = 0;
    std::vector<xf34> matrices;
};

struct HostTexture
{
    uint32_t w = 0, h = 0;
    std::vector<float> rgb;
};

struct HostLight { uint32_t blas, prim; float pdf, cdf; };

struct HostCamera
{
    bool set = false;
    float yaw = 0, pitch = 0;
    xf34 matrix;
    float inv_proj[16];
    float ray_matrix[16];
    float aperture = 0, focus = 0;
    uint32_t proj_kind = PROJ_PERSPECTIVE;
    float span_x_deg = 0, span_y_deg = 0, ortho_height = 0;
    float aspect = 1;
};

struct FlatScene
{
    std::vector<DNode> nodes;
    std::vector<DTriIsect> tri_isect;
    std::vector<DTriVerts> tri_shade, tri_pos;
    std::vector<uint32_t> tri_orig;
    std::vector<DTriUV> tri_uv;
    std::vector<DTexture> tex_table;
    std::vector<f4> tex_texels;
    std::vector<DInstance> instances;
    std::vector<uint32_t> big_leaves;
    std::vector<DMaterial> materials;
    std::vector<DLight> lights;
    std::vector<uint32_t> tri_base;
    std::vector<uint32_t> inst_base;
    uint32_t world_root = MISS_ID, lights_root = MISS_ID;
    uint32_t prim_bits = 0;
    uint32_t stack_entries = 0;
    uint32_t ident_tlas = 0;
    float light_weight_sum = 0;
    bool has_volumes = false;
    bool has_textures = false;
    TexView tex_view() const { return TexView{tex_texels.data(), tex_table.data(), tri_uv.data()}; }
    size_t table_bytes() const
    {
        return nodes.size() * sizeof(DNode) + tri_isect.size() * sizeof(DTriIsect) + instances.size() * sizeof(DInstance) + (big_leaves.size() * 4 + 15) / 16 * 16 +
               (tri_shade.size() + tri_pos.size()) * sizeof(DTriVerts) + tri_orig.size() * 4 + materials.size() * sizeof(DMaterial) + lights.size() * sizeof(DLight) +
               tri_uv.size() * sizeof(DTriUV) + tex_table.size() * sizeof(DTexture) + tex_texels.size() * sizeof(f4);
    }
};

class HostScene
{
public:
    std::vector<DMaterial> materials;
    std::vector<HostModel> models;
    std::vector<HostTexture> textures;
    std::vector<HostBlas> blas;
    HostTlas world, lights;
    std::vector<HostLight> light_items;
    float light_weight_sum = 0;
    HostCamera camera;
    FlatScene flat;
    bool built = false;
    uint64_t layout_epoch = 0;
    uint64_t blas_builds = 0, tlas_builds = 0;
    bool tlas_valid = false;
    bool flat_valid = false;
    uint64_t flat_epoch = 0;

    int add_material(int kind, const float colour[3], float roughness, float ior, bool has_volume, const float vol_abs[3], float k, float c,
                     float g);
    int add_model(const float* positions, const float* normals, uint32_t n_tris, int material, const float* affines, uint32_t n_inst);
    int add_model(const float* positions, const float* normals, uint32_t n_tris, int material, const float* affines, uint32_t n_inst, std::vector<float>&& uvs);
    int add_model_obj(const char* path, int material, const float* affines, uint32_t n_inst, std::string* err);
    int set_instances(int model, const float* affines, uint32_t n_inst);
    enum : uint64_t { kMaxTextureSide = 16384u, kMaxTexels = 1ull << 28 };
    int add_texture(uint32_t w, uint32_t h, const float* rgb);
    int set_material_texture(int material, int texture);
    int set_model_uvs(int model, const float* uv, uint32_t n_tris);
    int build(std::string* err);
    void set_camera(const float eye[3], const float target[3], float fov_deg, float aspect);
    void create_ray(float s, float t, float o[3], float d[3]) const;
    CameraView camera_view() const;
    LensView lens_view() const;
    ProjView proj_view() const;
    CameraOptics optics_view() const { return CameraOptics{lens_view(), proj_view()}; }
    uint32_t primary_ray(uint32_t width, uint32_t height, uint32_t n_sobol, uint64_t seed, uint32_t pixel, uint32_t sample, float o[3], float d[3]) const;
    void inv_projection(float out16[16]) const;
    void camera_move(float dx, float dz, float dt);
    void camera_rotate(float dx, float dy, float dt);

private:
    void build_blas(HostBlas& out, const HostModel& m);
    void build_tlas(HostTlas& out, const std::vector<uint32_t>& model_ids);
    void build_lights();
    int flatten(std::string* err);
    void refresh_ray_matrix();
};

}
```

### path_tracer_amd/csrc/pt_types.h

```cpp
#pragma once
#include <stdint.h>
#include "pt_math.h"

namespace pt {

enum : uint32_t
{
    NODE_BRANCH = 0u,
    NODE_TRIS = 1u,
    NODE_INSTANCE = 2u,
    NODE_TRIS_BIG = 3u,
    NODE_KIND_SHIFT = 30u,
    NODE_PAYLOAD_MASK = 0x3fffffffu,
    LEAF_FIRST_BITS = 24u,
    LEAF_FIRST_MASK = 0x00ffffffu,
    LEAF_MAX_COUNT = 64u,
    MISS_ID = 0xffffffffu
};

struct alignas(16) DNode
{
    float mn[3];
    uint32_t link;
    float mx[3];
    uint32_t aux;
};
static_assert(sizeof(DNode) == 32, "node is two 16-byte words");

struct alignas(16) DTriIsect { f4 n0, n1, n2; };
static_assert(sizeof(DTriIsect) == 48, "");
struct alignas(16) DTriVerts { f4 a, b, c; };

struct alignas(16) DInstance
{
    float inv[12];
    uint32_t root;
    uint32_t blas;
    uint32_t material;
    uint32_t qclass;
    DNode root_node;
    float fwd[12];
};
static_assert(sizeof(DInstance) == 144, "");
enum : uint32_t { INST_WORDS = 9u, INST_META_WORD = 3u, INST_ROOT_WORD = 4u };

enum : uint32_t { MAT_LAMBERTIAN = 0, MAT_EMISSIVE = 1, MAT_SPECULAR = 2, MAT_GGX_METAL = 3, MAT_GGX_DIELECTRIC = 4, MAT_DIELECTRIC = 5 };

struct alignas(16) DMaterial
{
    float colour[3];
    uint32_t kind;
    float alpha;
    float ior;
    uint32_t has_volume;
    uint32_t vol_flags;
    float vol_abs[3];
    float vol_c;
    float vol_g;
    uint32_t texture;
    float pad[2];
};
static_assert(sizeof(DMaterial) == 64, "");

struct alignas(16) DTexture
{
    uint32_t offset;
    uint32_t w, h;
    uint32_t pad;
};
static_assert(sizeof(DTexture) == 16, "");
struct DTriUV { float a[2], b[2], c[2]; };
static_assert(sizeof(DTriUV) == 24, "");
struct TexView
{
    const f4* texels;
    const DTexture* table;
    const DTriUV* tri_uv;
};

struct alignas(16) DLight
{
    uint32_t tri;
    uint32_t material;
    float pdf;
    float cdf;
};

enum : uint32_t { Q_TERMINAL = 0, Q_LAMBERT = 1, Q_SPECULAR = 2, Q_DIELECTRIC = 3, Q_GGX = 4, Q_COUNT = 5 };
enum : uint32_t { ENTRY_DEAD = 0x80000000u };
enum : uint32_t { INSTANCE_IDENTITY = 0x100u };
enum : uint32_t { IDENT_TLAS_WORLD = 1u, IDENT_TLAS_LIGHTS = 2u };

struct Counters
{
    uint32_t n_closest;
    uint32_t overflow;
    uint32_t n_shadow;
    uint32_t vstack_full;
    uint32_t n_lchain;
    uint32_t spare1;
    uint32_t spare2, spare3;
    uint32_t n_shade[Q_COUNT];
    uint32_t spare4, spare5, spare6;
};
static_assert(sizeof(Counters) == 64, "");

struct SceneView
{
    const DNode* nodes;
    const DTriIsect* tri_isect;
    const DTriVerts* tri_shade;
    const DTriVerts* tri_pos;
    const uint32_t* tri_orig;
    const DInstance* instances;
    const DMaterial* materials;
    const DLight* lights;
    uint32_t n_nodes, n_tris, n_instances, n_materials, n_lights;
    uint32_t world_root, lights_root;
    uint32_t prim_bits;
    float light_weight_sum;
    uint32_t has_volumes;
    uint32_t blob_bytes;
    uint32_t stack_entries;
    uint32_t stack_lds;
    uint64_t* stack_spill;
};
struct CameraView
{
    float ray_matrix[16];
    float eye[3];
    float pad;
};
struct LensView
{
    float c0[3];
    float radius;
    float c1[3];
    float focus;
};
enum : uint32_t { PROJ_PERSPECTIVE = 0u, PROJ_PANORAMA = 1u, PROJ_ORTHOGRAPHIC = 2u };
struct ProjView
{
    float c0[3];
    uint32_t kind;
    float c1[3];
    float sx;
    float c2[3];
    float sy;
};
struct CameraOptics
{
    LensView lens;
    ProjView proj;
};

struct FastDiv
{
    uint32_t magic, shift, one, d;
};
inline FastDiv fastdiv_make(uint32_t d)
{
    FastDiv f{0u, 0u, d <= 1u ? 1u : 0u, d};
    if (d <= 1u) return f;
    uint32_t l = 31u;
    while (!((d >> l) & 1u)) --l;
    if ((d & (d - 1u)) == 0u) { f.magic = 0u; f.shift = l - 1u; return f; }
    const uint64_t num = (uint64_t)1 << (32u + l);
    uint64_t m = num / d;
    const uint64_t rem = num - m * d;
    m += m;
    const uint64_t twice_rem = rem + rem;
    if (twice_rem >= d) m += 1u;
    f.magic = (uint32_t)(m + 1u);
    f.shift = l;
    return f;
}

struct RenderParams
{
    uint32_t width, height;
    uint32_t local_rows, local_pixels;
    uint32_t rank, world_size, strip_rows;
    uint32_t first_sample;
    uint32_t batch_samples;
    uint32_t n_paths;
    uint32_t max_bounces, n_sobol, enable_nee;
    uint32_t keep_s_id;
    uint32_t keep_s_pos;
    uint32_t blk_log, n_blk, blk_last;
    uint32_t act_x0, act_w, act_ly0, act_rows, act_pixels;
    uint32_t ray_draws;
    uint64_t seed;
    FastDiv div_blk_paths, div_blk_last, div_act_w, div_width, div_strip_rows;
};

struct AdaptiveCrit
{
    float rel_error, abs_floor;
    uint32_t min_samples, max_samples;
};
enum : uint32_t { kSelectPerBlock = 1024u };

struct DPathRec
{
    f4 pw;
    f4 acc;
    f4 nee_e;
// ... 38 lines not shown
```

Measured before the change: 15320 Mray/s.

## Skip redundant BLAS root box test when TLAS leaf box equals it; quad-transpose via LDS

At scene build, instances with identity transforms whose TLAS leaf box matches the BLAS root box are flagged, and a walk flag lets closest, any-hit and inline shadow traversals jump straight to the BLAS root without re-running the slab test on the root box. Separately, the shade kernel's 4x4 quad transpose of path state is done through LDS stores and loads instead of cross-lane shuffles when LDS stack space allows. It also adds debug APIs for RNG stream draws and instance flags. The root skip removes one slab test and an instance-record load per instance entry, at the cost of an extra flag branch and an LDS round trip in shading.

```diff
diff --git a/include/pt_api.h b/include/pt_api.h
--- a/include/pt_api.h
+++ b/include/pt_api.h
@@ -65,7 +65,8 @@
     PT_FLAG_TIMING_ALL = 4u,
     PT_FLAG_NO_PRIMARY_CULL = 8u,
     PT_FLAG_GENERAL_WALK = 16u,
-    PT_FLAG_ADAPTIVE = 32u
+    PT_FLAG_ADAPTIVE = 32u,
+    PT_FLAG_RETEST_ROOT_BOX = 64u
 };
 
 pt_ctx* pt_create(const pt_config* cfg);
@@ -208,6 +209,7 @@
 int pt_trace_any(pt_ctx* ctx, int which, uint32_t n, const float* o_xyz, const float* d_xyz, const float* t_max, uint8_t* hit);
 int pt_ss_sobol(pt_ctx* ctx, uint32_t n_points, uint32_t n, const uint32_t* index, const uint32_t* seed, float* out_xy);
 int pt_math_batch(pt_ctx* ctx, int fn, uint32_t n, const float* a, const float* b, float* out0, float* out1);
+int pt_stream_draws(pt_ctx* ctx, uint32_t pixel, uint32_t sample, uint32_t first_draw, uint32_t n, uint32_t* out);
 int pt_material_eval(pt_ctx* ctx, int material, uint32_t n, const float* incoming_xyz, const float* normal_xyz, const uint8_t* front,
                      const uint32_t* pixel, const uint32_t* sample, uint32_t draws_consumed, float* out9);
 int pt_volume_eval(pt_ctx* ctx, int material, uint32_t n, const float* incoming_xyz, const float* t_max, const float* dist,
@@ -220,6 +222,7 @@
                  uint32_t cap_nodes);
 int pt_tlas_instances(pt_ctx* ctx, int which, uint32_t* n, float* matrix12, float* inv_matrix12, uint32_t cap);
 int pt_instance_materials(pt_ctx* ctx, int which, uint32_t* n, uint32_t* material, uint32_t* blas, uint32_t cap);
+int pt_instance_flags(pt_ctx* ctx, int which, uint32_t* n, uint32_t* flags, uint32_t cap);
 int pt_light_cdf(pt_ctx* ctx, uint32_t* n, float* pdf, float* cdf, uint32_t* blas, uint32_t* prim, float* max_weight, uint32_t cap);
 int pt_triangle_dump(pt_ctx* ctx, int blas, uint32_t prim, float out36[36]);
 
diff --git a/path_tracer_amd/api.py b/path_tracer_amd/api.py
--- a/path_tracer_amd/api.py
+++ b/path_tracer_amd/api.py
@@ -16,13 +16,14 @@
 FLAG_NO_PRIMARY_CULL = 8
 FLAG_GENERAL_WALK = 16
 FLAG_ADAPTIVE = 32
+FLAG_RETEST_ROOT_BOX = 64
 DEFAULT_SEED = 0x5EED5EED
 
 EXPORTS = [
     "pt_create", "pt_destroy", "pt_last_error", "pt_set_config", "pt_add_material", "pt_add_model", "pt_add_model_obj", "pt_model_vertices", "pt_build", "pt_set_camera",
     "pt_camera_matrices", "pt_set_environment", "pt_create_ray", "pt_set_lens", "pt_primary_ray", "pt_render", "pt_render_device", "pt_reset_accumulation", "pt_accum_device_ptr",
     "pt_read_accumulation", "pt_read_frame", "pt_write_accumulation", "pt_render_samples", "pt_render_adaptive", "pt_adaptive_mask", "pt_read_moments", "pt_write_moments", "pt_active_pixels", "pt_local_rows", "pt_set_stream", "pt_synchronize", "pt_camera_input", "pt_camera_angles", "pt_frame", "pt_inv_projection", "pt_present", "pt_post_velocity", "pt_post_reproject", "pt_post_tonemap", "pt_post_rgb8", "pt_present_rgb8", "pt_write_image", "pt_trace_closest", "pt_trace_any",
-    "pt_ss_sobol", "pt_math_batch", "pt_material_eval", "pt_volume_eval", "pt_blas_count", "pt_blas_dump", "pt_tlas_dump", "pt_tlas_instances", "pt_instance_materials", "pt_light_cdf",
+    "pt_ss_sobol", "pt_math_batch", "pt_stream_draws", "pt_material_eval", "pt_volume_eval", "pt_blas_count", "pt_blas_dump", "pt_tlas_dump", "pt_tlas_instances", "pt_instance_materials", "pt_instance_flags", "pt_light_cdf",
     "pt_triangle_dump", "pt_get_stats", "pt_reset_stats", "pt_last_batch_counters", "pt_last_batch_shade_pids", "pt_last_batch_step_stats",
     "pt_multi_create", "pt_multi_destroy", "pt_multi_last_error", "pt_multi_ctx", "pt_multi_render", "pt_multi_framebuffer_device_ptr",
     "pt_multi_reset_accumulation", "pt_multi_get_stats", "pt_multi_used_rccl", "pt_multi_write_image",
@@ -189,6 +190,7 @@
         L.pt_tlas_dump.argtypes = [vp, C.c_int] + [vp] * 6 + [u32]
         L.pt_tlas_instances.argtypes = [vp, C.c_int, vp, vp, vp, u32]
         L.pt_instance_materials.argtypes = [vp, C.c_int, vp, vp, vp, u32]
+        L.pt_instance_flags.argtypes = [vp, C.c_int, vp, vp, u32]
         L.pt_light_cdf.argtypes = [vp] + [vp] * 6 + [u32]
         L.pt_triangle_dump.argtypes = [vp, C.c_int, u32, vp]
         L.pt_get_stats.argtypes = [vp, C.POINTER(Stats)]
@@ -204,6 +206,7 @@
         L.pt_integrate_rays_device.argtypes = [vp, C.c_uint64, vp, vp, vp, vp, C.POINTER(RaysParams), vp, vp, vp]
         L.pt_bake_probes.argtypes = [vp, u32, vp, C.POINTER(ProbeParams), vp]
         L.pt_probe_ray.argtypes = [vp, u32, u32, vp, vp]
+        L.pt_stream_draws.argtypes = [vp, u32, u32, u32, u32, vp]
         L.pt_set_instances.argtypes = [vp, C.c_int, f32p, u32]
         L.pt_get_scene_info.argtypes = [vp, C.POINTER(SceneInfo)]
         L.pt_read_guide_instances.argtypes = [vp, vp]
@@ -750,6 +753,11 @@
         self._chk(self.L.pt_math_batch(self.ctx, fn, a.size, _p(a), _p(b), _p(o0), _p(o1)))
         return o0, o1
 
+    def stream_draws(self, pixel: int, sample: int, first_draw: int, n: int):
+        out = np.zeros(n, np.uint32)
+        self._chk(self.L.pt_stream_draws(self.ctx, pixel, sample, first_draw, n, _p(out)))
+        return out
+
     def material_eval(self, material, incoming, normal, front, pixel, sample, draws_consumed=0):
         i = np.ascontiguousarray(incoming, np.float32); n = np.ascontiguousarray(normal, np.float32)
         f = np.ascontiguousarray(front, np.uint8); px = np.ascontiguousarray(pixel, np.uint32); sm = np.ascontiguousarray(sample, np.uint32)
@@ -801,6 +809,12 @@
         mat = np.zeros(cap, np.uint32); bl = np.zeros(cap, np.uint32)
         self._chk(self.L.pt_instance_materials(self.ctx, which, C.byref(n), _p(mat), _p(bl), cap))
         return dict(material=mat[:n.value].copy(), blas=bl[:n.value].copy())
+
+    def instance_flags(self, which=0, cap=1 << 16):
+        n = C.c_uint32()
+        fl = np.zeros(cap, np.uint32)
+        self._chk(self.L.pt_instance_flags(self.ctx, which, C.byref(n), _p(fl), cap))
+        return fl[:n.value].copy()
 
     def light_cdf(self, cap=1 << 20):
         n = C.c_uint32(); mx = C.c_float()
diff --git a/path_tracer_amd/csrc/pt_api.cpp b/path_tracer_amd/csrc/pt_api.cpp
--- a/path_tracer_amd/csrc/pt_api.cpp
+++ b/path_tracer_amd/csrc/pt_api.cpp
@@ -130,6 +130,7 @@
     SceneView sv{};
     bool lds_scene = false;
     uint32_t ident_tlas = 0;
+    bool root_boxes_same = false;
     uint32_t block_threads = 256, trace_blocks = 1024;
     bool class_present[Q_COUNT] = {true, false, false, false, false};
     bool resident_valid = false;
@@ -306,6 +307,8 @@
     sv.stack_entries = f.stack_entries;
     sv.has_volumes = f.has_volumes ? 1u : 0u;
     c->ident_tlas = f.ident_tlas;
+    c->root_boxes_same = f.root_boxes_same;
+    sv.walk_flags = 0u;
 
     c->lds_scene = blob_bytes <= 48 * 1024 && !(c->cfg.flags & PT_FLAG_NO_LDS_SCENE);
     uint32_t threads = 256;
@@ -422,6 +425,7 @@
     tl.blob = c->d_blob.p;
     tl.lds_scene = c->lds_scene;
     tl.ident_tlas = (c->cfg.flags & PT_FLAG_GENERAL_WALK) ? 0u : c->ident_tlas;
+    tl.scene.walk_flags = c->root_boxes_same && !(c->cfg.flags & PT_FLAG_RETEST_ROOT_BOX) ? (uint32_t)WALK_SKIP_ROOT_BOX : 0u;
     tl.grid_blocks = c->trace_blocks;
     tl.n_cus = (uint32_t)c->n_cus;
     tl.block_threads = c->block_threads;
@@ -2644,6 +2648,15 @@
     return o1 ? t.download(o1, d1, (size_t)n * 4) : PT_OK;
 }
 
+int pt_stream_draws(pt_ctx* c, uint32_t pixel, uint32_t sample, uint32_t first_draw, uint32_t n, uint32_t* out)
+{
+    if (!c || (n && !out)) return PT_ERR_ARG;
+    std::lock_guard<std::mutex> lk(c->mu);
+    Stream rng{stream_key(c->cfg.seed, pixel, sample), first_draw};
+    for (uint32_t j = 0; j < n; ++j) out[j] = rng.u32();
+    return PT_OK;
+}
+
 int pt_material_eval(pt_ctx* c, int material, uint32_t n, const float* incoming, const float* normal, const uint8_t* front, const uint32_t* pixel,
                      const uint32_t* sample, uint32_t draws, float* out9)
 {
@@ -2743,6 +2756,18 @@
     *n = e - b;
     if (e - b > cap || !material || !blas) return PT_ERR_ARG;
     for (uint32_t i = b; i < e; ++i) { material[i - b] = f.instances[i].material; blas[i - b] = f.instances[i].blas; }
+    return PT_OK;
+}
+
+int pt_instance_flags(pt_ctx* c, int which, uint32_t* n, uint32_t* flags, uint32_t cap)
+{
+    if (!c || !c->scene.built || !n) return PT_ERR_STATE;
+    const FlatScene& f = c->scene.flat;
+    const uint32_t b = f.inst_base[which ? 1 : 0], e = which ? (uint32_t)f.instances.size() : f.inst_base[1];
+    *n = e - b;
+    if (e - b > cap || !flags) return PT_ERR_ARG;
+    for (uint32_t i = b; i < e; ++i)
+        flags[i - b] = ((f.instances[i].qclass & INSTANCE_IDENTITY) ? 1u : 0u) | ((f.instances[i].qclass & INSTANCE_ROOT_BOX_SAME) ? 2u : 0u);
     return PT_OK;
 }
 
diff --git a/path_tracer_amd/csrc/pt_kernels.hip b/path_tracer_amd/csrc/pt_kernels.hip
--- a/path_tracer_amd/csrc/pt_kernels.hip
+++ b/path_tracer_amd/csrc/pt_kernels.hip
@@ -111,6 +111,12 @@
 #endif
 #ifndef PT_SHADE_WAVES_INLINE
 #define PT_SHADE_WAVES_INLINE 5
+#endif
+#ifndef PT_SKIP_ROOT_BOX
+#define PT_SKIP_ROOT_BOX 1
+#endif
+#ifndef PT_QUAD_LDS
+#define PT_QUAD_LDS 1
 #endif
 #ifndef PT_SHADE_THREADS
 #define PT_SHADE_THREADS 256
@@ -551,6 +557,9 @@
               asf((asu(v.z) & 0x7fffffffu) | (((bits >> 2) & 1u) << 31))};
 }
 
+__device__ __forceinline__ bool walk_skips_root_box(const SceneView& sv) { return PT_SKIP_ROOT_BOX && (sv.walk_flags & WALK_SKIP_ROOT_BOX) != 0u; }
+__device__ __forceinline__ uint32_t root_link(const Blob& bl, uint32_t inst) { return reinterpret_cast<const uint32_t*>(bl.inst + INST_WORDS * inst + INST_ROOT_WORD)[3]; }
+
 __device__ __forceinline__ Blob blob_at(const SceneView& sv, const uint4* base)
 {
     Blob b;
@@ -765,6 +774,7 @@
     if (blockIdx.x >= plan.blocks) return;
     const Stack8<SPILL> stk = Stack8<SPILL>::make(smem, blob_words, sv);
     const uint32_t prim_bits = sv.prim_bits;
+    [[maybe_unused]] const bool skip_root_box = IDENT && MODE == CLOSEST_LIGHTS && walk_skips_root_box(sv);
 
     bool active = false, pending = false, ray_finite = false;
     uint32_t ray_idx = 0, pid = 0;
@@ -980,6 +990,9 @@
                 if ((link >> NODE_KIND_SHIFT) == NODE_INSTANCE)
                 {
                     uint4 r0, r1;
+                    if (IDENT && skip_root_box) link = root_link(bl, link & NODE_PAYLOAD_MASK);
+                    else
+                    {
                     if (IDENT)
                     {
                         const uint4* ip = bl.inst + INST_WORDS * (link & NODE_PAYLOAD_MASK) + INST_ROOT_WORD;
@@ -993,6 +1006,7 @@
                     }
                     if (!slab(r0, r1, ob.o, ob.inv, t_max, t_enter)) continue;
                     link = r0.w;
+                    }
                 }
                 const uint32_t kkind = link >> NODE_KIND_SHIFT, kpay = link & NODE_PAYLOAD_MASK;
                 if (kkind == NODE_BRANCH)
@@ -1156,6 +1170,7 @@
     const FetchPlan plan = fetch_plan(min(*n_ptr, cap_in), LDS_SCENE ? (uint32_t)PT_CHUNK_DIV : (uint32_t)PT_CHUNK_DIV_GLOBAL_BVH, (uint32_t)PT_TAPER_ANY);
     if (blockIdx.x >= plan.blocks) return;
     const Stack8<SPILL> stk = Stack8<SPILL>::make(smem, blob_words, sv);
+    const bool skip_root_box = IDENT && walk_skips_root_box(sv);
 
     bool active = false, ray_finite = false;
     uint32_t out_idx = 0, valid_rays = 0;
@@ -1240,6 +1255,9 @@
             if ((link >> NODE_KIND_SHIFT) == NODE_INSTANCE)
             {
                 uint4 r0, r1;
+                if (IDENT && skip_root_box) link = root_link(bl, link & NODE_PAYLOAD_MASK);
+                else
+                {
                 if (IDENT)
                 {
                     const uint4* ip = bl.inst + INST_WORDS * (link & NODE_PAYLOAD_MASK) + INST_ROOT_WORD;
@@ -1253,6 +1271,7 @@
                 }
                 if (!slab(r0, r1, ob.o, ob.inv, t_max, t_enter)) continue;
                 link = r0.w;
+                }
             }
             uint32_t kind = link >> NODE_KIND_SHIFT, payload = link & NODE_PAYLOAD_MASK;
             ss.section(StepStats::BRANCH, kind == NODE_BRANCH);
@@ -1606,7 +1625,8 @@
 }
 
 template <bool IDENT>
-__device__ __forceinline__ bool inline_any(const Blob& bl, const Stack8<false>& stk, const uint32_t root, const f4 ra, const f4 rb, const bool want)
+__device__ __forceinline__ bool inline_any(const Blob& bl, const Stack8<false>& stk, const uint32_t root, const f4 ra, const f4 rb, const bool want,
+                                           const bool skip_root_box)
 {
     bool active = false, blocked = false, in_blas = false, ray_finite = false;
     LaneRay w{}, ob{};
@@ -1640,6 +1660,9 @@
         if ((link >> NODE_KIND_SHIFT) == NODE_INSTANCE)
         {
             uint4 r0, r1;
+            if (IDENT && skip_root_box) link = root_link(bl, link & NODE_PAYLOAD_MASK);
+            else
+            {
             if (IDENT)
             {
                 const uint4* ip = bl.inst + INST_WORDS * (link & NODE_PAYLOAD_MASK) + INST_ROOT_WORD;
@@ -1653,6 +1676,7 @@
             }
             if (!slab(r0, r1, ob.o, ob.inv, t_max, t_enter)) continue;
             link = r0.w;
+            }
         }
         uint32_t kind = link >> NODE_KIND_SHIFT, payload = link & NODE_PAYLOAD_MASK;
 #pragma unroll 1
@@ -2021,6 +2045,24 @@
         {
             float m[4][4] = {{pw.x, pw.y, pw.z, asf(draws)}, {acc.x, acc.y, acc.z, asf(flags)}, {nee_e.x, nee_e.y, nee_e.z, nee_e.w}, {nee_pw.x, nee_pw.y, nee_pw.z, nee_pw.w}};
             const uint32_t q = threadIdx.x & 3u;
+            bool by_lds = false;
+            if (PT_QUAD_LDS && INLINE) by_lds = shade_args().sv.stack_lds >= 8u;
+            if (by_lds)
+            {
+                typedef float v4_t __attribute__((ext_vector_type(4)));
+                uint32_t tid = threadIdx.x;
+                asm volatile("" : "+v"(tid));
+                const uint32_t lane = tid & 63u;
+                char* const wave_base = reinterpret_cast<char*>(smem_dyn) + shade_args().sv.blob_bytes + (lane >> 3) * (blockDim.x * 8u) + (tid >> 6) * 512u;
+                typedef __attribute__((address_space(3))) v4_t lds_v4_t;
+                lds_v4_t* const mine = (lds_v4_t*)(wave_base + (lane & 7u) * 64u);
+#pragma unroll
+                for (int w = 0; w < 4; ++w) mine[w] = v4_t{m[w][0], m[w][1], m[w][2], m[w][3]};
+                const lds_v4_t* const quad = (const lds_v4_t*)(wave_base + (lane & 4u) * 64u + q * 16u);
+#pragma unroll
+                for (int k = 0; k < 4; ++k) { const v4_t v = quad[4 * k]; m[k][0] = v.x; m[k][1] = v.y; m[k][2] = v.z; m[k][3] = v.w; }
+            }
+            else
 #pragma unroll
             for (int c = 0; c < 4; ++c)
             {
@@ -2051,7 +2093,7 @@
             const Stack8<false> stk{reinterpret_cast<char*>(smem_dyn), blob_words * 16u + tid * 8u, blockDim.x * 8u};
             traced += (uint32_t)__popcll(__ballot(want_shadow));
             culled += (uint32_t)__popcll(__ballot(cull_now));
-            const bool blocked = inline_any<IDENT>(bl, stk, ka2.world_root, sh_a, sh_b, want_shadow);
+            const bool blocked = inline_any<IDENT>(bl, stk, ka2.world_root, sh_a, sh_b, want_shadow, IDENT && walk_skips_root_box(ka2.sv));
             if (want_shadow) apply_shadow(shade_args().io.st.rec + pid, ends_with_shadow, blocked, [&]() -> f4& { return shade_args().io.st.radiance[pid]; });
             a_next = (idx + stride) < n ? nt_load(shade_args().io.q_in.a + idx + stride) : hole_a;
         }
@@ -2397,6 +2439,15 @@
         Stream r{stream_key(seed, asu(a[i]), asu(b[i])), 0u};
         o0[i] = asf(r.u32());
         o1[i] = r.f32();
+        break;
+    }
+    case 10:
+    {
+        Stream r{stream_key(seed, asu(a[i]), 0u), asu(b[i])};
+        uint32_t v = 0u;
+        for (uint32_t j = 0; j <= (i & 63u); ++j) v = r.u32();
+        o0[i] = asf(v);
+        o1[i] = asf(r.k);
         break;
     }
     }
@@ -2789,7 +2840,8 @@
     const bool inl = tl && shade_traces_shadow(*tl);
     if (list && qclass != Q_TERMINAL) io.list = list;
     if (ray_keys && qclass != Q_TERMINAL) io.list = ray_keys;
-    const ShadeKArgs ka{sv, rp, io, b, inl ? (const uint4*)tl->blob : nullptr, inl ? tl->scene.world_root : 0u};
+    ShadeKArgs ka{sv, rp, io, b, inl ? (const uint4*)tl->blob : nullptr, inl ? tl->scene.world_root : 0u};
+    if (inl) ka.sv.walk_flags = tl->scene.walk_flags;
     const size_t lds = inl ? trace_lds_bytes(*tl) : 0;
     ShadeKArgsTex kat{};
     static_cast<ShadeKArgs&>(kat) = ka;
diff --git a/path_tracer_amd/csrc/pt_scene.cpp b/path_tracer_amd/csrc/pt_scene.cpp
--- a/path_tracer_amd/csrc/pt_scene.cpp
+++ b/path_tracer_amd/csrc/pt_scene.cpp
@@ -882,8 +882,9 @@
     }
     auto put_instances = [&](const HostTlas& t, uint32_t ident_bit) {
         bool all_identity = true;
-        for (const HostInstance& hi : t.instances)
-        {
+        for (size_t k = 0; k < t.instances.size(); ++k)
+        {
+            const HostInstance& hi = t.instances[k];
             DInstance d;
             std::memset(&d, 0, sizeof(d));
             const xf34* src[2] = {&hi.inv, &hi.fwd};
@@ -913,11 +914,20 @@
                 if (std::memcmp(d.inv, ident, sizeof(ident)) == 0) d.qclass |= INSTANCE_IDENTITY;
                 else all_identity = false;
             }
+            {
+                DNode leaf;
+                put_box(leaf, t.nodes[k].box);
+                if ((d.qclass & INSTANCE_IDENTITY) != 0u && t.nodes[k].kind == NODE_INSTANCE && t.nodes[k].a == k && std::memcmp(leaf.mn, d.root_node.mn, sizeof(leaf.mn)) == 0 &&
+                    std::memcmp(leaf.mx, d.root_node.mx, sizeof(leaf.mx)) == 0)
+                    d.qclass |= INSTANCE_ROOT_BOX_SAME;
+                else f.root_boxes_same = false;
+            }
             f.instances.push_back(d);
         }
         if (all_identity) f.ident_tlas |= ident_bit;
     };
     f.ident_tlas = 0u;
+    f.root_boxes_same = true;
     put_instances(world, IDENT_TLAS_WORLD);
     put_instances(lights, IDENT_TLAS_LIGHTS);
 
diff --git a/path_tracer_amd/csrc/pt_scene.h b/path_tracer_amd/csrc/pt_scene.h
--- a/path_tracer_amd/csrc/pt_scene.h
+++ b/path_tracer_amd/csrc/pt_scene.h
@@ -96,6 +96,7 @@
     uint32_t prim_bits = 0;
     uint32_t stack_entries = 0;
     uint32_t ident_tlas = 0;
+    bool root_boxes_same = false;
     float light_weight_sum = 0;
     bool has_volumes = false;
     bool has_textures = false;
diff --git a/path_tracer_amd/csrc/pt_types.h b/path_tracer_amd/csrc/pt_types.h
--- a/path_tracer_amd/csrc/pt_types.h
+++ b/path_tracer_amd/csrc/pt_types.h
@@ -90,6 +90,8 @@
 enum : uint32_t { ENTRY_DEAD = 0x80000000u };
 enum : uint32_t { INSTANCE_IDENTITY = 0x100u };
 enum : uint32_t { IDENT_TLAS_WORLD = 1u, IDENT_TLAS_LIGHTS = 2u };
+enum : uint32_t { INSTANCE_ROOT_BOX_SAME = 0x200u };
+enum : uint32_t { WALK_SKIP_ROOT_BOX = 1u };
 
 struct Counters
 {
@@ -123,6 +125,7 @@
     uint32_t blob_bytes;
     uint32_t stack_entries;
     uint32_t stack_lds;
+    uint32_t walk_flags;
     uint64_t* stack_spill;
 };
 struct CameraView
```

Measured after the change: 15370 Mray/s (median of 6 runs). Within noise of the previous version (+0.4%).
